# ferdean/lsa-fw

Measured on AMD Instinct MI355X. Metric: converged eigenpairs/sec (k=20, shift-invert), higher is better.
Workload: dtype c128

## Files before the change

### include/lsa_hip.h

```cpp
#ifndef LSA_HIP_H
#define LSA_HIP_H

#include <stdint.h>

#ifdef __cplusplus
extern "C" {
#endif

typedef enum { LSA_F64 = 0, LSA_C128 = 1 } lsa_dtype;

typedef enum {
    LSA_OK = 0,
    LSA_ERR_ARG = -1,
    LSA_ERR_HIP = -2,
    LSA_ERR_ZERO_PIVOT = -3,
    LSA_ERR_DIVERGED = -4,
    LSA_ERR_NONFINITE = -5,
    LSA_ERR_TIMEOUT = -6,
    LSA_ERR_COMM = -7,
    LSA_ERR_OOM = -8
} lsa_status;

typedef struct lsa_ctx lsa_ctx;
typedef struct lsa_mat lsa_mat;
typedef struct lsa_vec lsa_vec;
typedef struct lsa_ilu lsa_ilu;
typedef struct lsa_op lsa_op;
typedef struct lsa_krylov lsa_krylov;

typedef struct {
    int64_t op_applies;
    int64_t gmres_iters;
    int64_t spmv_calls;
    int64_t sptrsv_calls;
    double last_rel_res;
    double max_rel_res;
    double seconds_factor;
    double seconds_solve;
    int32_t stagnated_solves;
    int32_t pc_fallback;
    int32_t backward_accepted;
    int32_t analysis_reused;
    int32_t refined_solves;
    int32_t reserved0;
} lsa_stats;

int lsa_ctx_create(int device, lsa_ctx **out);
void lsa_ctx_destroy(lsa_ctx *ctx);
const char *lsa_last_error(const lsa_ctx *ctx);
int lsa_ctx_synchronize(lsa_ctx *ctx);
const char *lsa_ctx_arch(const lsa_ctx *ctx);

int lsa_vec_create(lsa_ctx *ctx, int64_t n, int dtype, lsa_vec **out);
void lsa_vec_destroy(lsa_vec *v);
int lsa_vec_upload(lsa_ctx *ctx, lsa_vec *v, const void *host);
int lsa_vec_download(lsa_ctx *ctx, const lsa_vec *v, void *host);

int lsa_csr_upload(lsa_ctx *ctx, int32_t n, int64_t nnz, const int32_t *rowptr, const int32_t *col,
                   const void *val, int dtype, lsa_mat **out);
void lsa_mat_destroy(lsa_mat *m);
int lsa_mat_download_values(lsa_ctx *ctx, const lsa_mat *m, void *host_val);
int lsa_csr_axpby(lsa_ctx *ctx, const lsa_mat *A, const lsa_mat *B, const double alpha[2], const double beta[2],
                  int out_dtype, lsa_mat **out);
int lsa_spmv(lsa_ctx *ctx, const lsa_mat *A, const lsa_vec *x, lsa_vec *y);
int lsa_spmv_transpose(lsa_ctx *ctx, const lsa_mat *A, int conj, const lsa_vec *x, lsa_vec *y);
int lsa_spmv_info(lsa_ctx *ctx, const lsa_mat *A, int xdtype, char *kernel, int32_t kernel_len, int64_t *bytes_moved);
int lsa_spmv_time(lsa_ctx *ctx, const lsa_mat *A, const lsa_vec *x, lsa_vec *y, int iters, double *avg_ms);

int lsa_ilu_create(lsa_ctx *ctx, const lsa_mat *C, int levels, double shift_tol, lsa_ilu **out);
void lsa_ilu_destroy(lsa_ilu *pc);
int lsa_ilu_set_algorithm(lsa_ctx *ctx, lsa_ilu *pc, int algo, int32_t block_size);
int lsa_ilu_solve(lsa_ctx *ctx, lsa_ilu *pc, int which, const lsa_vec *b, lsa_vec *x);
int lsa_ilu_solve_time(lsa_ctx *ctx, lsa_ilu *pc, int which, const lsa_vec *b, lsa_vec *x, int iters, double *avg_ms);
int lsa_ilu_info(const lsa_ilu *pc, int64_t *nnz, int32_t *levels_lower, int32_t *levels_upper, int32_t *nshift);
int lsa_ilu_download(lsa_ctx *ctx, const lsa_ilu *pc, int32_t *rowptr, int32_t *col, void *val);

typedef struct lsa_nd_sym lsa_nd_sym;
typedef struct lsa_ndlu lsa_ndlu;
int lsa_nd_analyse(int32_t n, const int32_t *rowptr, const int32_t *col, int32_t leaf_size, const int8_t *constraint, lsa_nd_sym **out);
int lsa_nd_order(int32_t n, const int32_t *rowptr, const int32_t *col, int32_t leaf_size, const int8_t *constraint, lsa_nd_sym **out);
int lsa_nd_analyse_tree(int32_t n, const int32_t *rowptr, const int32_t *col, int32_t ntree, const int32_t *first, const int32_t *size,
                        const int32_t *parent, const int32_t *owner, int32_t rank, int32_t nranks, lsa_nd_sym **out);
const char *lsa_nd_sym_error(const lsa_nd_sym *h);
void lsa_nd_sym_destroy(lsa_nd_sym *h);
int lsa_nd_sym_info(const lsa_nd_sym *h, int32_t *ntree, int32_t *nlevels, int32_t *max_front, int64_t *index_entries,
                    int64_t *factor_entries, int64_t *front_entries, double *flops);
int lsa_nd_sym_memory(const lsa_nd_sym *h, int32_t scalar_bytes, int64_t work_budget_bytes, int64_t *out, int64_t *upd_off, int64_t *work_off,
                      int32_t *chunk_of);
int lsa_nd_sym_export(const lsa_nd_sym *h, int32_t *perm, int32_t *node_start, int32_t *parent, int32_t *level, int32_t *front_size,
                      int32_t *idx);
int lsa_nd_sym_export_tables(const lsa_nd_sym *h, int32_t *cmap, int32_t *gptr, int32_t *gidx, int64_t *asm_dst, int32_t *lvl_ptr,
                             int32_t *lvl_nodes);
int lsa_nd_sym_export_dist(const lsa_nd_sym *h, int32_t *kind, int64_t *front_off, int64_t *u_off, int32_t *asm_src, int32_t *children_ptr,
                           int32_t *children_idx, int64_t *scalars);
int lsa_nd_sym_export_top(const lsa_nd_sym *h, int32_t *owner, int32_t *rows, int64_t *exch, int64_t *totals);
int lsa_ndlu_create(lsa_ctx *ctx, const lsa_mat *C, int32_t leaf_size, lsa_ndlu **out);
int lsa_ndlu_prepare(lsa_ctx *ctx, const lsa_mat *P, int dtype, int32_t leaf_size, const int8_t *constraint);
int lsa_ndlu_prepare_tree(lsa_ctx *ctx, const lsa_mat *P, int dtype, int32_t ntree, const int32_t *first, const int32_t *size,
                          const int32_t *parent);
int lsa_ndlu_create_tree(lsa_ctx *ctx, const lsa_mat *C, int32_t ntree, const int32_t *first, const int32_t *size, const int32_t *parent,
                         const int32_t *owner, lsa_ndlu **out);
int lsa_ndlu_refactor(lsa_ctx *ctx, lsa_ndlu *f, const lsa_mat *C);
void lsa_ndlu_destroy(lsa_ndlu *f);
int lsa_ndlu_solve(lsa_ctx *ctx, lsa_ndlu *f, const lsa_vec *b, lsa_vec *x);
int lsa_ndlu_solve_batch(lsa_ctx *ctx, int32_t J, lsa_ndlu *const *f, const lsa_vec *const *b, lsa_vec *const *x);
int lsa_ndlu_solve_adjoint(lsa_ctx *ctx, lsa_ndlu *f, int conj, const lsa_vec *b, lsa_vec *x);
int lsa_ndlu_solve_time(lsa_ctx *ctx, lsa_ndlu *f, const lsa_vec *b, lsa_vec *x, int iters, double *avg_ms);
int lsa_ndlu_inertia(lsa_ctx *ctx, lsa_ndlu *f, int64_t *negative, int64_t *zero, int64_t *positive);
int lsa_ndlu_info(const lsa_ndlu *f, int32_t *ntree, int32_t *nlevels, int32_t *max_front, int64_t *factor_entries,
                  int64_t *front_entries, int64_t *apply_bytes, int32_t *apply_launches, double *seconds_analyse,
                  double *seconds_numeric);

int lsa_gmres(lsa_ctx *ctx, const lsa_mat *C, lsa_ilu *pc, const lsa_vec *b, lsa_vec *x, int use_x0, double rtol,
              int restart, int maxit, int32_t *iters, double *rel_res);

typedef struct {
    int32_t ilu_levels;
    double ilu_shift;
    double ksp_rtol;
    int32_t ksp_restart;
    int32_t ksp_maxit;
    int32_t pc_type;
    double antishift[2];
} lsa_op_options;

int lsa_op_create(lsa_ctx *ctx, const lsa_mat *A, const lsa_mat *M, const double sigma[2], int mode,
                  const lsa_op_options *opts, lsa_op **out);
void lsa_op_destroy(lsa_op *op);
int lsa_op_apply(lsa_ctx *ctx, lsa_op *op, const lsa_vec *x, lsa_vec *y);
int lsa_op_stats(const lsa_op *op, lsa_stats *out);
int lsa_op_set_adjoint(lsa_ctx *ctx, lsa_op *op, int on);
int lsa_op_set_projection(lsa_ctx *ctx, lsa_op *op, const double *keep);

int lsa_krylov_create(lsa_ctx *ctx, lsa_op *op, int32_t ncv, lsa_krylov **out);
// ... 94 lines not shown
```

### lsa-fw_amd/csrc/core.hip

```cpp
#include "lsa_internal.h"

int lsa_set_error(lsa_ctx* ctx, int code, const char* fmt, ...) {
    char buf[1024];
    va_list ap;
    va_start(ap, fmt);
    vsnprintf(buf, sizeof buf, fmt, ap);
    va_end(ap);
    if (ctx) ctx->err = buf;
    return code;
}

int lsa_ensure_scratch(lsa_ctx* ctx, size_t dbytes, size_t hbytes) {
    if (dbytes > ctx->dscratch_bytes) {
        LSA_HIP_CHECK(ctx, hipStreamSynchronize(ctx->stream));
        if (ctx->dscratch) (void)hipFree(ctx->dscratch);
        ctx->dscratch = nullptr;
        ctx->dscratch_bytes = 0;
        size_t want = dbytes * 2;
        LSA_HIP_CHECK(ctx, hipMalloc(&ctx->dscratch, want));
        ctx->dscratch_bytes = want;
    }
    if (hbytes > ctx->pinned_bytes) {
        LSA_HIP_CHECK(ctx, hipStreamSynchronize(ctx->stream));
        if (ctx->pinned) (void)hipHostFree(ctx->pinned);
        ctx->pinned = nullptr;
        ctx->pinned_bytes = 0;
        size_t want = hbytes * 2;
        LSA_HIP_CHECK(ctx, hipHostMalloc(&ctx->pinned, want, hipHostMallocDefault));
        ctx->pinned_bytes = want;
    }
    return LSA_OK;
}

lsa_mat* mat_row_view(const lsa_mat* full, int32_t r0, int32_t r1) {
    lsa_mat* v = new lsa_mat();
    v->ctx = full->ctx;
    v->n = r1 - r0;
    v->ncols = full->ncols;
    v->row0 = r0;
    v->nnz = (int64_t)full->h_rp[(size_t)r1] - full->h_rp[(size_t)r0];
    v->dtype = full->dtype;
    v->rp = full->rp + r0;
    v->ci = full->ci;
    v->val = full->val;
    v->owns_index = false;
    v->owns_values = false;
    v->ci16_state = -1;
    return v;
}

extern "C" {

int lsa_ctx_create(int device, lsa_ctx** out) {
    if (!out) return LSA_ERR_ARG;
    *out = nullptr;
    int ndev = 0;
    if (hipGetDeviceCount(&ndev) != hipSuccess || ndev <= 0) return LSA_ERR_HIP;
    if (device < 0 || device >= ndev) return LSA_ERR_ARG;
    if (hipSetDevice(device) != hipSuccess) return LSA_ERR_HIP;
    lsa_ctx* ctx = new lsa_ctx();
    ctx->device = device;
    hipDeviceProp_t prop;
    if (hipGetDeviceProperties(&prop, device) != hipSuccess) {
        delete ctx;
        return LSA_ERR_HIP;
    }
    ctx->arch = prop.gcnArchName;
    ctx->num_cu = prop.multiProcessorCount > 0 ? prop.multiProcessorCount : 256;
    if (hipStreamCreateWithFlags(&ctx->stream, hipStreamNonBlocking) != hipSuccess ||
        hipEventCreate(&ctx->ev0) != hipSuccess || hipEventCreate(&ctx->ev1) != hipSuccess) {
        delete ctx;
        return LSA_ERR_HIP;
    }
    if (lsa_ensure_scratch(ctx, 1 << 20, 1 << 16) != LSA_OK) {
        delete ctx;
        return LSA_ERR_HIP;
    }
    *out = ctx;
    return LSA_OK;
}

void lsa_ctx_destroy(lsa_ctx* ctx) {
    if (!ctx) return;
    (void)hipSetDevice(ctx->device);
    if (ctx->stream) (void)hipStreamSynchronize(ctx->stream);
    lsa_ndlu_drop_cache(ctx);
    lsa_krylov_drop_cache(ctx);
    comm_release(ctx);
    if (ctx->dscratch) (void)hipFree(ctx->dscratch);
    if (ctx->pinned) (void)hipHostFree(ctx->pinned);
    if (ctx->ev0) (void)hipEventDestroy(ctx->ev0);
    if (ctx->ev1) (void)hipEventDestroy(ctx->ev1);
    if (ctx->stream) (void)hipStreamDestroy(ctx->stream);
    delete ctx;
}

const char* lsa_last_error(const lsa_ctx* ctx) { return ctx ? ctx->err.c_str() : "null context"; }
const char* lsa_ctx_arch(const lsa_ctx* ctx) { return ctx ? ctx->arch.c_str() : ""; }

int lsa_ctx_synchronize(lsa_ctx* ctx) {
    if (!ctx) return LSA_ERR_ARG;
    LSA_HIP_CHECK(ctx, hipStreamSynchronize(ctx->stream));
    return LSA_OK;
}

static size_t dtype_size(int dtype) { return dtype == LSA_C128 ? 16 : 8; }

int lsa_vec_create(lsa_ctx* ctx, int64_t n, int dtype, lsa_vec** out) {
    if (!ctx || !out || n < 0 || (dtype != LSA_F64 && dtype != LSA_C128))
        return lsa_set_error(ctx, LSA_ERR_ARG, "lsa_vec_create: bad argument");
    lsa_vec* v = new lsa_vec{ctx, n, dtype, nullptr};
    hipError_t e = hipMalloc(&v->d, (size_t)(n > 0 ? n : 1) * dtype_size(dtype));
    if (e != hipSuccess) {
        delete v;
        return lsa_set_error(ctx, LSA_ERR_HIP, "hipMalloc(vector of %lld) failed: %s", (long long)n, hipGetErrorString(e));
    }
    e = hipMemsetAsync(v->d, 0, (size_t)(n > 0 ? n : 1) * dtype_size(dtype), ctx->stream);
    if (e != hipSuccess) {
        (void)hipFree(v->d);
        delete v;
        return lsa_set_error(ctx, LSA_ERR_HIP, "hipMemsetAsync failed: %s", hipGetErrorString(e));
    }
    *out = v;
    return LSA_OK;
}

void lsa_vec_destroy(lsa_vec* v) {
    if (!v) return;
    if (v->ctx && v->ctx->stream) (void)hipStreamSynchronize(v->ctx->stream);
    if (v->d) (void)hipFree(v->d);
    delete v;
}

int lsa_vec_upload(lsa_ctx* ctx, lsa_vec* v, const void* host) {
    if (!ctx || !v || !host) return lsa_set_error(ctx, LSA_ERR_ARG, "lsa_vec_upload: null argument");
    LSA_HIP_CHECK(ctx, hipMemcpyAsync(v->d, host, (size_t)v->n * dtype_size(v->dtype), hipMemcpyHostToDevice, ctx->stream));
    LSA_HIP_CHECK(ctx, hipStreamSynchronize(ctx->stream));
    return LSA_OK;
}

int lsa_vec_download(lsa_ctx* ctx, const lsa_vec* v, void* host) {
    if (!ctx || !v || !host) return lsa_set_error(ctx, LSA_ERR_ARG, "lsa_vec_download: null argument");
    LSA_HIP_CHECK(ctx, hipMemcpyAsync(host, v->d, (size_t)v->n * dtype_size(v->dtype), hipMemcpyDeviceToHost, ctx->stream));
    LSA_HIP_CHECK(ctx, hipStreamSynchronize(ctx->stream));
    return LSA_OK;
}

static int validate_csr(lsa_ctx* ctx, int32_t n, int32_t ncols, int64_t nnz, const int32_t* rp, const int32_t* ci) {
    if (rp[0] != 0 || rp[n] != nnz) return lsa_set_error(ctx, LSA_ERR_ARG, "CSR: rowptr[0] must be 0 and rowptr[n] == nnz");
    for (int32_t i = 0; i < n; ++i) {
        if (rp[i + 1] < rp[i]) return lsa_set_error(ctx, LSA_ERR_ARG, "CSR: rowptr not monotone at row %d", i);
        for (int32_t p = rp[i]; p < rp[i + 1]; ++p) {
            if (ci[p] < 0 || ci[p] >= ncols) return lsa_set_error(ctx, LSA_ERR_ARG, "CSR: column %d out of range in row %d", ci[p], i);
            if (p > rp[i] && ci[p] <= ci[p - 1]) return lsa_set_error(ctx, LSA_ERR_ARG, "CSR: columns of row %d are not strictly increasing", i);
        }
    }
    return LSA_OK;
}

static int csr_upload_impl(lsa_ctx* ctx, int32_t n_local, int32_t ncols, int32_t row0, int64_t nnz, const int32_t* rowptr,
                           const int32_t* col, const void* val, int dtype, lsa_mat** out) {
    if (!ctx || !out || !rowptr || (nnz > 0 && (!col || !val)) || n_local < 0 || nnz < 0 ||
        (dtype != LSA_F64 && dtype != LSA_C128))
        return lsa_set_error(ctx, LSA_ERR_ARG, "lsa_csr_upload: bad argument");
    if (nnz >= (int64_t)INT32_MAX) return lsa_set_error(ctx, LSA_ERR_ARG, "lsa_csr_upload: nnz >= 2^31 needs 64-bit row pointers");
    LSA_CHECK(validate_csr(ctx, n_local, ncols, nnz, rowptr, col));
    lsa_mat* m = new lsa_mat();
    m->ctx = ctx;
    m->n = n_local;
    m->ncols = ncols;
    m->row0 = row0;
    m->nnz = nnz;
    m->dtype = dtype;
// ... 3 lines not shown
    m->val = nullptr;
    m->h_rp.assign(rowptr, rowptr + n_local + 1);
    m->h_ci.assign(col, col + nnz);
    size_t vb = (size_t)(nnz > 0 ? nnz : 1) * dtype_size(dtype);
    hipError_t e1 = hipMalloc(&m->rp, sizeof(int32_t) * (size_t)(n_local + 1));
    hipError_t e2 = hipMalloc(&m->ci, sizeof(int32_t) * (size_t)(nnz > 0 ? nnz : 1));
    hipError_t e3 = hipMalloc(&m->val, vb);
    if (e1 != hipSuccess || e2 != hipSuccess || e3 != hipSuccess) {
        lsa_mat_destroy(m);
        return lsa_set_error(ctx, LSA_ERR_HIP, "hipMalloc(CSR n=%d nnz=%lld) failed", n_local, (long long)nnz);
    }
    hipError_t e = hipMemcpyAsync(m->rp, rowptr, sizeof(int32_t) * (size_t)(n_local + 1), hipMemcpyHostToDevice, ctx->stream);
    if (e == hipSuccess && nnz > 0) e = hipMemcpyAsync(m->ci, col, sizeof(int32_t) * (size_t)nnz, hipMemcpyHostToDevice, ctx->stream);
    if (e == hipSuccess && nnz > 0) e = hipMemcpyAsync(m->val, val, (size_t)nnz * dtype_size(dtype), hipMemcpyHostToDevice, ctx->stream);
    if (e == hipSuccess) e = hipStreamSynchronize(ctx->stream);
    if (e != hipSuccess) {
        lsa_mat_destroy(m);
        return lsa_set_error(ctx, LSA_ERR_HIP, "CSR upload failed: %s", hipGetErrorString(e));
    }
    *out = m;
    return LSA_OK;
}

int lsa_csr_upload(lsa_ctx* ctx, int32_t n, int64_t nnz, const int32_t* rowptr, const int32_t* col, const void* val,
                   int dtype, lsa_mat** out) {
    return csr_upload_impl(ctx, n, n, 0, nnz, rowptr, col, val, dtype, out);
}

int lsa_csr_upload_shard(lsa_ctx* ctx, int32_t n_global, int32_t row0, int32_t row1, int64_t nnz_local,
                         const int32_t* rowptr_local, const int32_t* col, const void* val, int dtype, lsa_mat** out) {
    if (row0 < 0 || row1 < row0 || row1 > n_global) return lsa_set_error(ctx, LSA_ERR_ARG, "lsa_csr_upload_shard: bad row range");
    return csr_upload_impl(ctx, row1 - row0, n_global, row0, nnz_local, rowptr_local, col, val, dtype, out);
}

int64_t lsa_mat_rows(const lsa_mat* m) { return m ? (int64_t)m->n : 0; }

void lsa_mat_destroy(lsa_mat* m) {
    if (!m) return;
    if (m->ctx && m->ctx->stream) (void)hipStreamSynchronize(m->ctx->stream);
    if (m->owns_index) {
        if (m->rp) (void)hipFree(m->rp);
        if (m->ci) (void)hipFree(m->ci);
    }
    if (m->val && m->owns_values) (void)hipFree(m->val);
    if (!m->owns_extras) m->ci16 = nullptr, m->cbase = nullptr, m->grp_start = nullptr;
    if (m->grp_start) (void)hipFree(m->grp_start);
    if (m->ci16) (void)hipFree(m->ci16);
    if (m->cbase) (void)hipFree(m->cbase);
    delete m;
}

int lsa_mat_download_values(lsa_ctx* ctx, const lsa_mat* m, void* host_val) {
    if (!ctx || !m || !host_val) return lsa_set_error(ctx, LSA_ERR_ARG, "lsa_mat_download_values: null argument");
    LSA_HIP_CHECK(ctx, hipMemcpyAsync(host_val, m->val, (size_t)m->nnz * dtype_size(m->dtype), hipMemcpyDeviceToHost, ctx->stream));
    LSA_HIP_CHECK(ctx, hipStreamSynchronize(ctx->stream));
    return LSA_OK;
}

}

template <typename TA, typename TB, typename TC>
__global__ void axpby_kernel(int64_t nnz, const TA* __restrict__ a, const TB* __restrict__ b, cplx alpha, cplx beta,
                             TC* __restrict__ c) {
    int64_t stride = (int64_t)gridDim.x * blockDim.x;
    for (int64_t p = (int64_t)blockIdx.x * blockDim.x + threadIdx.x; p < nnz; p += stride) {
        cplx acc{0.0, 0.0};
        fma_acc(acc, alpha, to_cplx(a[p]));
        fma_acc(acc, beta, to_cplx(b[p]));
        s_from(c[p], acc.re, acc.im);
    }
}

template <typename TA, typename TB, typename TC>
static void launch_axpby(lsa_ctx* ctx, int64_t nnz, const void* a, const void* b, cplx alpha, cplx beta, void* c) {
    int threads = 256;
    int64_t want = (nnz + threads - 1) / threads;
    int blocks = (int)(want < 1 ? 1 : (want > 4096 ? 4096 : want));
    hipLaunchKernelGGL((axpby_kernel<TA, TB, TC>), dim3(blocks), dim3(threads), 0, ctx->stream, nnz, (const TA*)a, (const TB*)b,
                       alpha, beta, (TC*)c);
}

extern "C" int lsa_csr_axpby(lsa_ctx* ctx, const lsa_mat* A, const lsa_mat* B, const double alpha[2], const double beta[2],
                             int out_dtype, lsa_mat** out) {
    if (!ctx || !A || !B || !alpha || !beta || !out) return lsa_set_error(ctx, LSA_ERR_ARG, "lsa_csr_axpby: null argument");
    if (A->n != B->n || A->nnz != B->nnz || A->ncols != B->ncols || A->row0 != B->row0)
        return lsa_set_error(ctx, LSA_ERR_ARG, "lsa_csr_axpby: operands must share one sparsity pattern (n %d vs %d, nnz %lld vs %lld)",
                             A->n, B->n, (long long)A->nnz, (long long)B->nnz);
    if (!A->h_rp.same_object(B->h_rp) || !A->h_ci.same_object(B->h_ci)) {
        if (A->h_rp != B->h_rp || A->h_ci != B->h_ci)
            return lsa_set_error(ctx, LSA_ERR_ARG, "lsa_csr_axpby: operands must share one sparsity pattern (index arrays differ)");
        B->h_rp = A->h_rp;
        B->h_ci = A->h_ci;
        if (!A->h_hash) A->h_hash = B->h_hash ? B->h_hash : std::make_shared<uint64_t>(0);
        B->h_hash = A->h_hash;
        if (!A->h_shared) A->h_shared = B->h_shared ? B->h_shared : std::make_shared<PatternShared>();
        B->h_shared = A->h_shared;
    }
    if (out_dtype == LSA_F64 && (A->dtype != LSA_F64 || B->dtype != LSA_F64 || alpha[1] != 0.0 || beta[1] != 0.0))
        return lsa_set_error(ctx, LSA_ERR_ARG, "lsa_csr_axpby: a real result needs real operands and real coefficients");
    lsa_mat* C = new lsa_mat();
    C->ctx = ctx;
    C->n = A->n;
    C->ncols = A->ncols;
    C->row0 = A->row0;
    C->nnz = A->nnz;
    C->dtype = out_dtype;
    C->rp = A->rp;
    C->ci = A->ci;
    C->owns_index = false;
    C->h_rp = A->h_rp;
    C->h_ci = A->h_ci;
    if (!A->h_hash) A->h_hash = std::make_shared<uint64_t>(0);
    C->h_hash = A->h_hash;
    if (!A->h_shared) A->h_shared = std::make_shared<PatternShared>();
    C->h_shared = A->h_shared;
    C->val = nullptr;
    hipError_t e = hipMalloc(&C->val, (size_t)(C->nnz > 0 ? C->nnz : 1) * dtype_size(out_dtype));
    if (e != hipSuccess) {
        delete C;
        return lsa_set_error(ctx, LSA_ERR_HIP, "hipMalloc(axpby result) failed: %s", hipGetErrorString(e));
    }
    cplx al{alpha[0], alpha[1]}, be{beta[0], beta[1]};
    const bool ca = A->dtype == LSA_C128, cb = B->dtype == LSA_C128;
    if (out_dtype == LSA_F64) launch_axpby<double, double, double>(ctx, C->nnz, A->val, B->val, al, be, C->val);
    else if (!ca && !cb) launch_axpby<double, double, cplx>(ctx, C->nnz, A->val, B->val, al, be, C->val);
    else if (ca && !cb) launch_axpby<cplx, double, cplx>(ctx, C->nnz, A->val, B->val, al, be, C->val);
    else if (!ca && cb) launch_axpby<double, cplx, cplx>(ctx, C->nnz, A->val, B->val, al, be, C->val);
    else launch_axpby<cplx, cplx, cplx>(ctx, C->nnz, A->val, B->val, al, be, C->val);
    hipError_t le = hipGetLastError();
    if (le != hipSuccess) {
        lsa_mat_destroy(C);
        return lsa_set_error(ctx, LSA_ERR_HIP, "axpby launch failed: %s", hipGetErrorString(le));
    }
    *out = C;
    return LSA_OK;
}
```

### lsa-fw_amd/csrc/dense.hip

```cpp
#include <algorithm>
#include <chrono>
#include <cmath>
#include <cstdint>
#include <cstring>
#include <vector>

#include "lsa_internal.h"

namespace {

struct Z {
    double re, im;
};
inline Z operator+(Z a, Z b) { return {a.re + b.re, a.im + b.im}; }
inline Z operator-(Z a, Z b) { return {a.re - b.re, a.im - b.im}; }
inline Z operator-(Z a) { return {-a.re, -a.im}; }
inline Z operator*(Z a, Z b) { return {a.re * b.re - a.im * b.im, a.re * b.im + a.im * b.re}; }
inline Z operator*(double a, Z b) { return {a * b.re, a * b.im}; }
inline Z conj(Z a) { return {a.re, -a.im}; }
inline double abs1(Z a) { return std::fabs(a.re) + std::fabs(a.im); }
inline double abs2(Z a) { return a.re * a.re + a.im * a.im; }
inline double zabs(Z a) { return std::hypot(a.re, a.im); }
inline Z zdiv(Z a, Z b) {
    if (std::fabs(b.re) >= std::fabs(b.im)) {
// ... 667 lines not shown
        }
    auto W = [&](int i, int j) -> double& { return w[(size_t)j * n + i]; };
    auto swap_sym = [&](int p, int q) {
        if (p == q) return;
        for (int j = 0; j < n; ++j) std::swap(W(p, j), W(q, j));
        for (int i = 0; i < n; ++i) std::swap(W(i, p), W(i, q));
    };
    const double alpha = (1.0 + std::sqrt(17.0)) / 8.0, tiny = std::max(tol_rel, 0.0) * amax;
    int k = 0;
    while (k < n) {
        const double absakk = std::fabs(W(k, k));
        int imax = k;
        double colmax = 0.0;
        for (int i = k + 1; i < n; ++i)
            if (std::fabs(W(i, k)) > colmax) colmax = std::fabs(W(i, k)), imax = i;
        int step = 1;
        if (std::max(absakk, colmax) <= tiny) {
            ++*zero;
            ++k;
            continue;
        }
        if (absakk < alpha * colmax) {
            double rowmax = 0.0;
            for (int j = k; j < n; ++j)
                if (j != imax) rowmax = std::max(rowmax, std::fabs(W(imax, j)));
            if (absakk >= alpha * colmax * (colmax / rowmax)) {
            } else if (std::fabs(W(imax, imax)) >= alpha * rowmax) {
                swap_sym(k, imax);
            } else {
                swap_sym(k + 1, imax);
                step = 2;
            }
        }
        if (step == 1) {
            const double d = W(k, k);
            if (std::fabs(d) <= tiny) ++*zero;
            else if (d < 0.0) ++*negative;
            else ++*positive;
            if (std::fabs(d) > tiny) {
                const double dinv = 1.0 / d;
                for (int j = k + 1; j < n; ++j) {
                    const double f = W(k, j) * dinv;
                    if (f == 0.0) continue;
                    for (int i = k + 1; i < n; ++i) W(i, j) -= W(i, k) * f;
                }
            }
        } else {
            const double a = W(k, k), b = W(k + 1, k), c = W(k + 1, k + 1), det = a * c - b * b;
            if (std::fabs(det) <= tiny * tiny) {
                *zero += 2;
            } else {
                if (det < 0.0) {
                    ++*negative;
                    ++*positive;
                } else if (a + c < 0.0) *negative += 2;
                else *positive += 2;
                for (int j = k + 2; j < n; ++j) {
                    const double u = W(k, j), v = W(k + 1, j);
                    const double f0 = (c * u - b * v) / det, f1 = (a * v - b * u) / det;
                    if (f0 == 0.0 && f1 == 0.0) continue;
                    for (int i = k + 2; i < n; ++i) W(i, j) -= W(i, k) * f0 + W(i, k + 1) * f1;
                }
            }
        }
        k += step;
    }
    return LSA_OK;
}

static_assert(sizeof(lsa_ks_result) == 56 && sizeof(lsa_ks_options) == 88, "lsa_ks_options layout is part of the C-ABI (tests/test_abi.py)");

int lsa_krylov_solve(lsa_ctx* ctx, lsa_krylov* k, const lsa_ks_options* o, const void* v0, const double* mask, int32_t max_out, void* theta_out,
                     void* lambda_out, void* X_out, double* est_out, lsa_ks_result* result) {
    if (!ctx || !k || !o || !result) return lsa_set_error(ctx, LSA_ERR_ARG, "lsa_krylov_solve: null argument");
    int32_t m = 0;
    int64_t n = 0;
    LSA_CHECK(lsa_krylov_shape(k, &n, &m));
    if (m > n) return lsa_set_error(ctx, LSA_ERR_ARG, "ncv = %d exceeds the problem size %lld", m, (long long)n);
    LSA_CHECK(ks_check_options(ctx, "lsa_krylov_solve", o, max_out, theta_out, lambda_out));
    const int nev = std::min<int>(o->nev, m);
    const double keep_fraction = ks_keep_fraction(o);
    const Selector sel{o->which, o->transform, {o->sigma[0], o->sigma[1]}, {o->antishift[0], o->antishift[1]}, {o->target[0], o->target[1]}};
    Rng rng = ks_rng(o);
    std::vector<Z> vec((size_t)n);
    auto random_vector = [&]() {
        for (int64_t i = 0; i < n; ++i) {
            rng.normal_pair(vec[(size_t)i].re, vec[(size_t)i].im);
            if (mask && mask[i] == 0.0) vec[(size_t)i] = {0.0, 0.0};
        }
    };
    if (v0) {
        memcpy(vec.data(), v0, (size_t)n * sizeof(Z));
        if (mask)
            for (int64_t i = 0; i < n; ++i)
                if (mask[i] == 0.0) vec[(size_t)i] = {0.0, 0.0};
    } else {
        random_vector();
    }
    LSA_CHECK(lsa_krylov_inject(ctx, k, 0, vec.data()));
    const int ldh = m + 1;
    std::vector<Z> H((size_t)ldh * m, Z{0.0, 0.0}), T((size_t)m * m), Q((size_t)m * m), S((size_t)m * m), b((size_t)m), bq((size_t)m), w((size_t)m);
    std::vector<double> est((size_t)m), rel((size_t)m), keys((size_t)m);
    std::vector<int> rank((size_t)m);
    std::vector<char> select((size_t)m);
    const Mat Hm{H.data(), ldh}, Tm{T.data(), m}, Qm{Q.data(), m}, Sm{S.data(), m};
    int kept = 0, restarts = 0;
    int64_t applies = 0;
    memset(result, 0, sizeof *result);
    KsClock clk;
    auto extend = [&](int j, int32_t* bd) {
        LSA_CHECK(lsa_krylov_extend(ctx, k, j, m, H.data(), ldh, bd));
        if (*bd >= 0) Hm(*bd + 1, *bd) = {0.0, 0.0};
        return (int)LSA_OK;
    };
    auto inject_random = [&](int j) {
        random_vector();
        return lsa_krylov_inject(ctx, k, j, vec.data());
    };
    while (true) {
        clk.start();
        LSA_CHECK(ks_expand(kept, m, &applies, extend, inject_random));
        clk.lap(clk.expand);
        for (int c = 0; c < m; ++c) {
            b[(size_t)c] = Hm(m, c);
            for (int r = 0; r < m; ++r) Tm(r, c) = Hm(r, c);
        }
        if (!schur(m, Tm, Qm)) return lsa_set_error(ctx, LSA_ERR_DIVERGED, "Krylov-Schur: the QR algorithm on the projected matrix did not converge");
        tri_eigenvectors(m, Tm, Sm);
        for (int c = 0; c < m; ++c) {
            Z acc = {0.0, 0.0};
            for (int r = 0; r < m; ++r) acc = acc + b[(size_t)r] * Qm(r, c);
            bq[(size_t)c] = acc;
        }
        for (int c = 0; c < m; ++c) {
            Z acc = {0.0, 0.0};
            for (int r = 0; r <= c; ++r) acc = acc + bq[(size_t)r] * Sm(r, c);
            est[(size_t)c] = zabs(acc);
            w[(size_t)c] = Tm(c, c);
            keys[(size_t)c] = sel.key(w[(size_t)c]);
            rel[(size_t)c] = est[(size_t)c] / std::max(zabs(w[(size_t)c]), 2.2250738585072014e-308);
        }
        const int nconv = ks_rank_converged(m, keys, rel, o->tol, rank);
        if (nconv >= nev || nconv >= m || restarts >= o->max_restarts) {
            const int nout = std::min<int>(nconv, max_out);
            if (nout > 0) {
                std::vector<Z> Y((size_t)m * nout);
                for (int c = 0; c < nout; ++c) {
                    const int src = rank[(size_t)c];
                    for (int r = 0; r < m; ++r) {
                        Z acc = {0.0, 0.0};
                        for (int q = 0; q <= src; ++q) acc = acc + Qm(r, q) * Sm(q, src);
                        Y[(size_t)c * m + r] = acc;
                    }
                    ((Z*)theta_out)[c] = w[(size_t)src];
                    ((Z*)lambda_out)[c] = sel.back(w[(size_t)src]);
                    if (est_out) est_out[c] = rel[(size_t)src];
                }
                clk.lap(clk.dense);
                if (X_out) LSA_CHECK(lsa_krylov_ritz_vectors(ctx, k, m, nout, Y.data(), m, 3, X_out));
                clk.lap(clk.restart);
            }
            clk.lap(clk.dense);
            ks_fill_result(result, clk, nconv, nout, restarts, applies, nconv < m ? rel[(size_t)rank[(size_t)nconv]] : 0.0);
            return k_agree_in_step(ctx, "lsa_krylov_solve");
        }
        int knew = ks_keep_count(m, nconv, keep_fraction);
        {
            std::vector<double> sorted(keys);
            std::sort(sorted.begin(), sorted.end());
            const double thr = sorted[(size_t)knew] > sorted[(size_t)knew - 1] ? 0.5 * (sorted[(size_t)knew - 1] + sorted[(size_t)knew]) : sorted[(size_t)knew - 1];
            for (int c = 0; c < m; ++c) select[(size_t)c] = keys[(size_t)c] <= thr;
            const int sdim = schur_reorder(m, Tm, Qm, select);
            knew = std::max(std::min(sdim, m - 1), 1);
        }
        clk.lap(clk.dense);
        LSA_CHECK(lsa_krylov_restart(ctx, k, m, knew, Q.data(), m));
        clk.lap(clk.restart);
        std::fill(H.begin(), H.end(), Z{0.0, 0.0});
        for (int c = 0; c < knew; ++c) {
            for (int r = 0; r <= c; ++r) Hm(r, c) = Tm(r, c);
            Z acc = {0.0, 0.0};
            for (int r = 0; r < m; ++r) acc = acc + b[(size_t)r] * Qm(r, c);
            Hm(knew, c) = acc;
        }
        kept = knew;
        ++restarts;
    }
}

int lsa_eigs_sinvert(lsa_ctx* ctx, const lsa_mat* A, const lsa_mat* M, const double sigma[2], int32_t nev, int32_t ncv, double tol, int32_t max_restarts,
                     const lsa_op_options* opts, const void* v0, const int32_t* row_perm, int32_t max_out, void* lambda_out, void* X_out, double* est_out,
                     lsa_ks_result* result, lsa_stats* stats) {
    if (!ctx || !A || !sigma || !opts || !result) return lsa_set_error(ctx, LSA_ERR_ARG, "lsa_eigs_sinvert: null argument");
    if (ncv <= 0) ncv = std::max(2 * nev, nev + 15);
    ncv = (int32_t)std::min<int64_t>(ncv, lsa_mat_rows(A));
    lsa_op* op = nullptr;
    lsa_krylov* kr = nullptr;
    int rc = lsa_op_create(ctx, A, M, sigma, 0, opts, &op);
    if (rc == LSA_OK) rc = lsa_krylov_create(ctx, op, ncv, &kr);
    if (rc == LSA_OK && row_perm) rc = lsa_krylov_set_row_permutation(ctx, kr, row_perm);
    if (rc == LSA_OK) {
        lsa_ks_options o;
        memset(&o, 0, sizeof o);
        o.nev = nev;
        o.max_restarts = max_restarts;
        o.tol = tol;
        o.which = LSA_WHICH_TARGET_MAGNITUDE;
        o.transform = 0;
        o.sigma[0] = o.target[0] = sigma[0];
// ... 114 lines not shown
```

### lsa-fw_amd/csrc/lsa_internal.h

```cpp
#pragma once

#include <hip/hip_runtime.h>

#include <cstdarg>
#include <cstdint>
#include <cstdio>
#include <cstdlib>
#include <cstring>
#include <memory>
#include <string>
#include <vector>

#include "../../include/lsa_hip.h"

struct cplx {
    double re, im;
};
static_assert(sizeof(cplx) == 16, "complex128 layout");

__host__ __device__ inline cplx make_cplx(double r, double i) { return cplx{r, i}; }

template <typename T>
struct scalar_traits;
template <>
struct scalar_traits<double> {
    static constexpr int dtype = LSA_F64;
    __host__ __device__ static double zero() { return 0.0; }
};
template <>
struct scalar_traits<cplx> {
    static constexpr int dtype = LSA_C128;
    __host__ __device__ static cplx zero() { return cplx{0.0, 0.0}; }
};

__host__ __device__ inline void fma_acc(double& acc, double a, double b) { acc = fma(a, b, acc); }
__host__ __device__ inline void fma_acc(cplx& acc, double a, cplx b) {
    acc.re = fma(a, b.re, acc.re);
    acc.im = fma(a, b.im, acc.im);
}
__host__ __device__ inline void fma_acc(cplx& acc, cplx a, cplx b) {
    acc.re = fma(a.re, b.re, acc.re);
    acc.re = fma(-a.im, b.im, acc.re);
    acc.im = fma(a.re, b.im, acc.im);
    acc.im = fma(a.im, b.re, acc.im);
}
__host__ __device__ inline void fma_conj_acc(double& acc, double a, double b) { acc = fma(a, b, acc); }
__host__ __device__ inline void fma_conj_acc(cplx& acc, cplx a, cplx b) {
    acc.re = fma(a.re, b.re, acc.re);
    acc.re = fma(a.im, b.im, acc.re);
    acc.im = fma(a.re, b.im, acc.im);
    acc.im = fma(-a.im, b.re, acc.im);
}
__host__ __device__ inline double s_mul(double a, double b) { return a * b; }
__host__ __device__ inline cplx s_mul(double a, cplx b) { return cplx{a * b.re, a * b.im}; }
__host__ __device__ inline cplx s_mul(cplx a, cplx b) { return cplx{a.re * b.re - a.im * b.im, a.re * b.im + a.im * b.re}; }
__host__ __device__ inline double s_add(double a, double b) { return a + b; }
__host__ __device__ inline cplx s_add(cplx a, cplx b) { return cplx{a.re + b.re, a.im + b.im}; }
__host__ __device__ inline double s_sub(double a, double b) { return a - b; }
__host__ __device__ inline cplx s_sub(cplx a, cplx b) { return cplx{a.re - b.re, a.im - b.im}; }
__host__ __device__ inline double s_conj(double a) { return a; }
__host__ __device__ inline cplx s_conj(cplx a) { return cplx{a.re, -a.im}; }
__host__ __device__ inline double s_abs2(double a) { return a * a; }
__host__ __device__ inline double s_abs2(cplx a) { return a.re * a.re + a.im * a.im; }
__host__ __device__ inline double s_inv(double a) { return 1.0 / a; }
__host__ __device__ inline cplx s_inv(cplx a) {
    if (fabs(a.re) >= fabs(a.im)) {
        double r = a.im / a.re, d = a.re + a.im * r;
        return cplx{1.0 / d, -r / d};
    }
    double r = a.re / a.im, d = a.re * r + a.im;
    return cplx{r / d, -1.0 / d};
}
__host__ __device__ inline cplx to_cplx(double a) { return cplx{a, 0.0}; }
__host__ __device__ inline cplx to_cplx(cplx a) { return a; }
__host__ __device__ inline void s_from(double& out, double re, double) { out = re; }
__host__ __device__ inline void s_from(cplx& out, double re, double im) { out = cplx{re, im}; }

struct lsa_ctx {
    int device = 0;
    hipStream_t stream = nullptr;
    hipEvent_t ev0 = nullptr, ev1 = nullptr;
    std::string err;
    std::string arch;
    int num_cu = 256;
    void* pinned = nullptr;
    size_t pinned_bytes = 0;
    void* dscratch = nullptr;
    size_t dscratch_bytes = 0;
    void* comm = nullptr;
    int nranks = 1, rank = 0;
    lsa_host_allgather_fn host_gather = nullptr;
    void* host_gather_user = nullptr;
    void* comm_stage = nullptr;
    size_t comm_stage_bytes = 0;
    int64_t comm_calls = 0, comm_bytes = 0;
    struct lsa_ndlu* nd_cache = nullptr;
    struct lsa_krylov* krylov_cache = nullptr;
};
extern "C" void lsa_ndlu_drop_cache(lsa_ctx* ctx);
extern "C" void lsa_krylov_drop_cache(lsa_ctx* ctx);

struct lsa_vec {
    lsa_ctx* ctx;
    int64_t n;
    int dtype;
    void* d;
};

struct SharedInts {
    std::shared_ptr<const std::vector<int32_t>> p;
    const int32_t* data() const { return p ? p->data() : nullptr; }
    size_t size() const { return p ? p->size() : 0; }
    const int32_t& operator[](size_t i) const { return (*p)[i]; }
    const std::vector<int32_t>& vec() const {
        static const std::vector<int32_t> none;
        return p ? *p : none;
    }
    void assign(const int32_t* b, const int32_t* e) { p = std::make_shared<const std::vector<int32_t>>(b, e); }
    bool same_object(const SharedInts& o) const { return p == o.p; }
    bool operator==(const SharedInts& o) const { return p == o.p || vec() == o.vec(); }
    bool operator!=(const SharedInts& o) const { return !(*this == o); }
};

struct TransposeIndex {
    int32_t *rp = nullptr, *ci = nullptr, *src = nullptr;
    int32_t ncols = 0;
    int64_t nnz = 0;
    ~TransposeIndex() {
        for (void* p : {(void*)rp, (void*)ci, (void*)src})
            if (p) (void)hipFree(p);
    }
};

struct PatternShared {
    std::shared_ptr<TransposeIndex> tr;
};

struct lsa_mat {
    lsa_ctx* ctx;
    int32_t n;
    int32_t ncols;
    int32_t row0;
    int64_t nnz;
    int dtype;
    int32_t* rp;
    int32_t* ci;
    void* val;
    bool owns_index;
    bool owns_values = true;
    mutable SharedInts h_rp, h_ci;
    mutable std::shared_ptr<uint64_t> h_hash;
    mutable std::shared_ptr<PatternShared> h_shared;
    mutable uint16_t* ci16 = nullptr;
    mutable int32_t* cbase = nullptr;
    mutable int ci16_state = 0;
    mutable int32_t* grp_start = nullptr;
    mutable int32_t ngroups = 0;
    mutable int grp_state = 0;
    bool owns_extras = true;
};

int lsa_set_error(lsa_ctx* ctx, int code, const char* fmt, ...);
lsa_mat* mat_row_view(const lsa_mat* full, int32_t r0, int32_t r1);
void comm_release(lsa_ctx* ctx);
int k_agree_status(lsa_ctx* ctx, int rc);
int k_agree_min_i64(lsa_ctx* ctx, int64_t* value);
int k_agree_in_step(lsa_ctx* ctx, const char* where);
int lsa_ensure_scratch(lsa_ctx* ctx, size_t dbytes, size_t hbytes);
inline bool env_flag(const char* name, bool dflt) {
    const char* e = getenv(name);
    return e ? atoi(e) != 0 : dflt;
}

#define LSA_HIP_CHECK(ctx, expr)                                                                         \
    do {                                                                                                 \
        hipError_t _e = (expr);                                                                          \
        if (_e != hipSuccess)                                                                            \
            return lsa_set_error((ctx), LSA_ERR_HIP, "%s failed: %s (%s:%d)", #expr, hipGetErrorString(_e), \
                                 __FILE__, __LINE__);                                                    \
    } while (0)

#define LSA_HIP_ALLOC(ctx, expr)                                                                                    \
    do {                                                                                                            \
        hipError_t _e = (expr);                                                                                     \
        if (_e != hipSuccess) {                                                                                     \
            (void)hipGetLastError();                                                                                \
            return lsa_set_error((ctx), _e == hipErrorOutOfMemory ? LSA_ERR_OOM : LSA_ERR_HIP, "%s failed: %s (%s:%d)", #expr, \
                                 hipGetErrorString(_e), __FILE__, __LINE__);                                        \
        }                                                                                                           \
    } while (0)

#define LSA_CHECK(expr)            \
    do {                           \
        int _rc = (expr);          \
        if (_rc != LSA_OK) return _rc; \
    } while (0)


int k_spmv(lsa_ctx* ctx, const lsa_mat* A, int xdtype, const void* x, void* y);
int k_spmv_transpose(lsa_ctx* ctx, const lsa_mat* A, int conj, int xdtype, const void* x, void* y);

int k_copy(lsa_ctx* ctx, int dtype, int64_t n, const void* x, void* y);
int k_set_zero(lsa_ctx* ctx, int dtype, int64_t n, void* x);
int k_axpy(lsa_ctx* ctx, int dtype, int64_t n, const double alpha[2], const void* x, void* y);
int k_multi_dot(lsa_ctx* ctx, int dtype, int64_t n, int j, const void* V, int64_t ldv, const void* w, void* h_dev);
int k_multi_axpy_dot(lsa_ctx* ctx, int dtype, int64_t n, int j, const void* V, int64_t ldv, const void* h1_dev, void* w, void* h2_dev);
int k_multi_axpy(lsa_ctx* ctx, int dtype, int64_t n, int j, const void* V, int64_t ldv, const void* h_dev, void* w,
                 double* nrm2_dev);
int k_columns_canonical(lsa_ctx* ctx, int64_t n, int ncols, void* X, int64_t ldx, int unit, double* imag2_dev);
int k_nrm2(lsa_ctx* ctx, int dtype, int64_t n, const void* x, double* nrm2_dev);
int k_mask(lsa_ctx* ctx, int dtype, int64_t n, const double* keep_dev, void* y);
int k_residual_norms(lsa_ctx* ctx, int dtype, int64_t n, const void* b, const void* z, void* w, double* nrm2_dev);
int k_scale_by_inv_norm(lsa_ctx* ctx, int dtype, int64_t n, const void* x, const double* nrm2_dev, void* y);
int k_hess_column(lsa_ctx* ctx, int dtype, int j, const void* h1, const void* h2, const double* nrm2_dev, void* hout);
size_t k_cgs2_fused_work_bytes(lsa_ctx* ctx, int64_t n, int jmax);
int k_cgs2_fused(lsa_ctx* ctx, int dtype, int64_t n, int j, const void* V, int64_t ldv, void* w, void* vnext, void* hcol_dev, void* work,
                 const void* chk_b, const void* chk_z, double* chk_out);
bool k_cgs2_tail_fits(lsa_ctx* ctx, int64_t n, int jmax, const lsa_mat* M, const lsa_mat* C);
int k_cgs2_tail_parts(int64_t n);
int k_cgs2_fused_tail(lsa_ctx* ctx, int64_t n, int j, const void* V, int64_t ldv, const void* y, void* w, void* vnext, void* hcol_dev, void* work,
                      const lsa_mat* M, const lsa_mat* C, void* t, double* tail_part);
int k_cgs2_tail_checks(lsa_ctx* ctx, int nslots, int nparts, const double* tail_parts, double* checks);
bool k_dcgs2_fits(int64_t n, int ncv);
int k_dcgs2_step(lsa_ctx* ctx, int64_t n, int j, void* V, int64_t ldv, const void* y, int first, void* slot, int lds, void* work,
                 const void* chk_b, const void* chk_z, double* chk_out);
int k_dcgs2_norm(lsa_ctx* ctx, int64_t n, void* work, void* slot, int lds);
int k_dcgs2_tail(lsa_ctx* ctx, int64_t n, int j, const void* V, int64_t ldv, const void* y, void* work, const lsa_mat* M, const lsa_mat* C, void* t,
                 double* tail_part, void* slot, int lds);
int k_spmv_plain_subwave_lanes(const lsa_mat* A);
int k_basis_gemm(lsa_ctx* ctx, int dtype, int64_t n, int m, int k, const void* V, int64_t ldv, const void* Q, int ldq,
                 void* Out, int64_t ldo);
int k_scatter_rows(lsa_ctx* ctx, int dtype, int64_t n, int ncols, const int32_t* perm, const void* In, void* Out);

int basis_upload_row_permutation(lsa_ctx* ctx, const char* who, int64_t n, const int32_t* perm, int32_t** row_perm);
int basis_times_host_matrix(lsa_ctx* ctx, int dtype, int64_t n, int m, int k, const void* V, const void* Q, int ldq, void* qdev, void* Out,
                            size_t pinned_extra);
int direct_solve_enqueue(lsa_ctx* ctx, lsa_op* op, int dtype, const void* rhs, void* y, void* z, void* r, bool refine, double* norms);
void stats_book_direct_solve(lsa_stats* st, int products, bool refine, double res, double bnorm);

struct lsa_ndlu;
struct lsa_op_parts {
    int64_t n;
    const lsa_mat *Kmul, *Kfac;
    lsa_ndlu* nd;
    bool plain;
    double ksp_rtol;
    double normF;
    bool* refine;
    lsa_stats* st;
};
int lsa_op_get_parts(lsa_op* op, lsa_op_parts* out);
int lanczos_shape(const lsa_lanczos* l, int64_t* n, int32_t* ncv);
int lanczos_inject(lsa_ctx* ctx, lsa_lanczos* l, int32_t j, const double* host_v);
int lanczos_restart(lsa_ctx* ctx, lsa_lanczos* l, int32_t m, int32_t knew, const double* Y, int32_t ldy);
int lanczos_ritz_vectors(lsa_ctx* ctx, lsa_lanczos* l, int32_t m, int32_t nvec, const double* Y, int32_t ldy, double* X);

struct lsa_ilu {
    lsa_ctx* ctx;
    int32_t n;
    int64_t nnz;
    int dtype;
    int32_t *rp, *ci, *diag;
    void* val;
    void* dinv;
    int32_t *order_l, *order_u;
    std::vector<int32_t> lvl_ptr_l, lvl_ptr_u;
    std::vector<int32_t> h_rp, h_ci, h_diag;
    int32_t nshift;
    int32_t* flag;
    int sptrsv_blocks_l, sptrsv_blocks_u;
    int algo;
    void* tmp;
    int tmp_dtype;
    int32_t blk_B = 0, blk_nb = 0;
    int32_t *lsplit = nullptr, *usplit = nullptr;
    void *linv = nullptr, *uinv = nullptr;
    void *blk_t[2] = {nullptr, nullptr}, *blk_y[2] = {nullptr, nullptr};
    void *blk_in[2] = {nullptr, nullptr}, *blk_out[2] = {nullptr, nullptr};
    void* blk_graph[2] = {nullptr, nullptr};
};

int ilu_solve_dev(lsa_ctx* ctx, lsa_ilu* pc, int which, int vdtype, const void* b, void* x);
int blk_setup(lsa_ctx* ctx, lsa_ilu* pc, int32_t B);
int blk_solve(lsa_ctx* ctx, lsa_ilu* pc, int which, int vdtype, const void* b, void* x);
void blk_release(lsa_ilu* pc);

struct lsa_ndlu;
int ndlu_solve_dev(lsa_ctx* ctx, lsa_ndlu* f, int vdtype, const void* b, void* x);
int ndlu_solve_adjoint_dev(lsa_ctx* ctx, lsa_ndlu* f, int conj, int vdtype, const void* b, void* x);
```

### lsa-fw_amd/csrc/ndlu.hip

```cpp
#include <algorithm>
#include <chrono>
#include <cmath>
#include <cstdlib>
#include <functional>
#include <new>
#include <string>

#include "lsa_internal.h"
#include "nd_internal.h"

int k_allgather_inplace(lsa_ctx* ctx, void* vec, size_t bytes_per_rank);

namespace {

constexpr int kRT = 32;
constexpr int kCH = 1024;
constexpr int kGT = 64;

inline double now_s() { return std::chrono::duration<double>(std::chrono::steady_clock::now().time_since_epoch()).count(); }
inline size_t esize(int dtype) { return dtype == LSA_C128 ? 16 : 8; }

struct NdNodeDev {
    int64_t front_off;
    int64_t lfac_off;
// ... 2067 lines not shown
        if (L.exchange_before && f->xupd_slot > 0) {
            LSA_CHECK(k_allgather_inplace(ctx, f->d_upd, (size_t)f->xupd_slot * sizeof(T)));
            exchanged = true;
        }
        LSA_HIP_CHECK(ctx, hipMemsetAsync(f->d_work, 0, (size_t)L.work_entries * sizeof(T), st));
        if (L.asm_count > 0) {
            const int blocks = (int)std::min<int64_t>((L.asm_count + 255) / 256, (int64_t)ctx->num_cu * 16);
            hipLaunchKernelGGL((nd_assemble_kernel<T>), dim3(blocks), dim3(256), 0, st, L.asm_count, (const T*)C->val, f->d_asm_src + L.asm_begin,
                               f->d_asm_dst + L.asm_begin, front);
        }
        for (const TileList& e : L.ext)
            if (e.count > 0)
                hipLaunchKernelGGL((nd_extend_add_kernel<T>), dim3(e.count), dim3(256), 0, st, tl + 2 * e.off, f->d_nodes, f->d_cmap, front, (const T*)upd);
        for (const auto& step : L.xsteps) {
            T* stage = (T*)f->d_xstage;
            int64_t stride = 0;
            for (int r = 0; r < S.nranks; ++r) {
                const NdChunk::XPiece& pc = step[(size_t)r];
                if (pc.nrows > 0) stride = std::max(stride, (int64_t)pc.nrows * (S.f[(size_t)pc.child] - S.m[(size_t)pc.child]));
            }
            if (stride == 0) continue;
            const NdChunk::XPiece& mine = step[(size_t)S.rank];
            if (mine.nrows > 0) {
                const int32_t bc = S.f[(size_t)mine.child] - S.m[(size_t)mine.child];
                const int64_t src_off = f->chunk_node_upd_off(mine.child) + (int64_t)(mine.row0 - S.brow0[(size_t)mine.child]) * bc;
                LSA_HIP_CHECK(ctx, hipMemcpyAsync(stage + (size_t)S.rank * (size_t)stride, upd + src_off, (size_t)mine.nrows * (size_t)bc * sizeof(T),
                                                  hipMemcpyDeviceToDevice, st));
            }
            LSA_CHECK(k_allgather_inplace(ctx, stage, (size_t)stride * sizeof(T)));
            for (int r = 0; r < S.nranks; ++r) {
                const NdChunk::XPiece& pc = step[(size_t)r];
                if (pc.nrows <= 0) continue;
                hipLaunchKernelGGL((nd_extend_add_staged_kernel<T>), dim3((pc.nrows + 15) / 16), dim3(256), 0, st, f->d_nodes, f->d_cmap, front,
                                   (const T*)(stage + (size_t)r * (size_t)stride), pc.child, pc.row0, pc.nrows);
            }
        }
        if (L.max_m >= f->tp_min) LSA_CHECK(launch_level_tp<T>(ctx, f, L, tiny2));
        for (int32_t kb = 0; kb < L.max_m && L.max_m < f->tp_min; kb += kNB) {
            if (L.max_m <= 64) launch_block<T, 64, 1, 8>(ctx, f, L, kb, tiny2);
            else if (L.max_m <= 128) launch_block<T, 128, 1, 8>(ctx, f, L, kb, tiny2);
            else if (L.max_m <= 256) launch_block<T, 256, 1, 8>(ctx, f, L, kb, tiny2);
            else if (L.max_m <= 512) launch_block<T, 512, 1, 8>(ctx, f, L, kb, tiny2);
            else if (L.max_m <= 1024) launch_block<T, 1024, 1, 8>(ctx, f, L, kb, tiny2);
            else if (L.max_m <= 2048) launch_block<T, 1024, 2, 8>(ctx, f, L, kb, tiny2);
            else if (L.max_m <= 4096) launch_block<T, 1024, 4, 4>(ctx, f, L, kb, tiny2);
            else if (L.max_m <= 8192) launch_block<T, 1024, 8, 2>(ctx, f, L, kb, tiny2);
            else launch_block<T, 1024, 16, 1>(ctx, f, L, kb, tiny2);
        }
        if (L.unperm.count > 0)
            hipLaunchKernelGGL((nd_unperm_kernel<T>), dim3(L.unperm.count), dim3(256), 0, st, tl + 2 * L.unperm.off, f->d_nodes, front, f->d_ipiv,
                               f->d_rowq, lfac);
        auto product = [&](auto kind) {
            constexpr int KIND = decltype(kind)::value;
            if (L.gemm[KIND].count == 0) return;
            hipLaunchKernelGGL((nd_gemm_mfma_kernel<T, KIND>), dim3(L.gemm[KIND].count), dim3(256), 0, st, tl + 2 * L.gemm[KIND].off, f->d_nodes, front, lfac, ufac);
        };
        product(std::integral_constant<int, 0>{});
        product(std::integral_constant<int, 1>{});
        product(std::integral_constant<int, 2>{});
        if (L.save.count > 0)
            hipLaunchKernelGGL((nd_save_update_kernel<T>), dim3(L.save.count), dim3(256), 0, st, tl + 2 * L.save.off, f->d_nodes, (const T*)front, upd);
    }
    if (f->top.s > 0)
        for (int q = 0, t0 = 0; q < 2; t0 += f->top_tiles[q++])
            if (f->top_tiles[q] > 0)
                hipLaunchKernelGGL((nd_top_gemm_kernel<T>), dim3(f->top_tiles[q]), dim3(256), 0, st, f->d_top_tiles + 2 * t0, f->d_top_jobs, f->d_cmap,
                                   (const T*)lfac, (const T*)ufac, (T*)f->d_top, f->top.s);
    if (!exchanged && S.nranks > 1 && f->xupd_slot > 0)
        LSA_CHECK(k_allgather_inplace(ctx, f->d_upd, (size_t)f->xupd_slot * sizeof(T)));
    int32_t hflag[4] = {0, 0, 0, 0};
    if (S.nranks > 1) {
        LSA_HIP_CHECK(ctx, hipMemcpyAsync(f->d_xflag + 4 * S.rank, f->d_flag, 4 * sizeof(int32_t), hipMemcpyDeviceToDevice, st));
        LSA_CHECK(k_allgather_inplace(ctx, f->d_xflag, 4 * sizeof(int32_t)));
        std::vector<int32_t> all((size_t)4 * S.nranks, 0);
        LSA_HIP_CHECK(ctx, hipMemcpyAsync(all.data(), f->d_xflag, all.size() * sizeof(int32_t), hipMemcpyDeviceToHost, st));
        LSA_HIP_CHECK(ctx, hipStreamSynchronize(st));
        for (int r = 0; r < S.nranks; ++r)
            if (all[(size_t)4 * r + 1] != 0) {
                memcpy(hflag, &all[(size_t)4 * r], sizeof hflag);
                if (r != S.rank) hflag[1] = -(r + 1);
                break;
            }
    } else {
        LSA_HIP_CHECK(ctx, hipMemcpyAsync(hflag, f->d_flag, sizeof hflag, hipMemcpyDeviceToHost, st));
        LSA_HIP_CHECK(ctx, hipStreamSynchronize(st));
    }
    LSA_HIP_CHECK(ctx, hipGetLastError());
    if (hflag[1] < 0)
        return lsa_set_error(ctx, LSA_ERR_ZERO_PIVOT, "lsa_ndlu: a pivot block on rank %d is singular to 1e-15 * max|C| (column %d of its node)", -hflag[1] - 1,
                             hflag[2]);
    if (hflag[1] != 0) {
        const int32_t t = hflag[1] - 1;
        const unsigned long long hi = (unsigned long long)(uint32_t)hflag[3] << 32;
        double mag2;
        memcpy(&mag2, &hi, sizeof mag2);
        return lsa_set_error(ctx, LSA_ERR_ZERO_PIVOT,
                             "lsa_ndlu: the pivot block of tree node %d (%d unknowns, front %d, level %d) is singular at its column %d: largest "
                             "candidate pivot %.3e against max|C| = %.3e (threshold 1e-15 max|C|); the matrix is singular, or needs pivoting "
                             "across fronts",
                             t, S.m[(size_t)t], S.f[(size_t)t], S.level[(size_t)t], hflag[2], std::sqrt(mag2), std::sqrt(max2));
    }
    if (const char* pe = getenv("LSA_ND_TEST_PERTURB")) {
        const double eps = atof(pe);
        if (eps != 0.0 && f->ufac_entries > 0) {
            const int blocks = (int)std::min<int64_t>((f->ufac_entries + 255) / 256, (int64_t)ctx->num_cu * 16);
            hipLaunchKernelGGL((nd_scale_kernel<T>), dim3(blocks), dim3(256), 0, st, f->ufac_entries, ufac, 1.0 + eps);
            LSA_HIP_CHECK(ctx, hipStreamSynchronize(st));
        }
    }
    return LSA_OK;
}

template <typename MT, typename VT, bool ORDERED>
int nd_apply_ordered(lsa_ctx* ctx, lsa_ndlu* f, const VT* b, VT* x) {
    hipStream_t st = ctx->stream;
    const MT* lfac = (const MT*)f->d_lfac;
    const MT* ufac = (const MT*)f->d_ufac;
    const NdSymbolic& S = f->S;
    VT *ubuf = (VT*)f->d_ubuf, *acc = (VT*)f->d_acc, *xb = (VT*)f->d_xb;
    const bool top = f->top.s > 0;
    if (f->acc_vbytes != (int)sizeof(VT)) {
        LSA_HIP_CHECK(ctx, hipMemsetAsync(f->d_acc, 0, (size_t)std::max<int64_t>(f->acc_entries, 1) * 16, st));
        f->acc_vbytes = (int)sizeof(VT);
    }
    for (size_t li = 0; li <= f->levels.size(); ++li) {
        if ((int32_t)li == S.phase_b_level && S.nranks > 1 && S.xu_slot > 0) LSA_CHECK(k_allgather_inplace(ctx, f->d_ubuf, (size_t)S.xu_slot * sizeof(VT)));
        if (li == f->levels.size()) break;
        const NdLevel& L = f->levels[li];
        if (ORDERED && top && (int32_t)li + 1 == f->top_level) continue;
        if (ORDERED && top && (int32_t)li == f->top_level) {
            hipLaunchKernelGGL((nd_top_kernel<MT, VT>), dim3((f->top.s + 7) / 8), dim3(256), 0, st, f->top, (const MT*)f->d_top, f->d_top_icmap, f->d_gell, b, x,
                               (const VT*)acc, xb);
        } else if (L.fwd_tiles > 0) {
            const dim3 grid(L.node_count, L.fwd_tiles);
            const NdSweepNode* ln = f->d_lnodes + L.node_begin;
            if (L.sweep_rows == 8)
                hipLaunchKernelGGL((nd_fwd_kernel<MT, VT, 64, ORDERED>), grid, dim3(256), 0, st, ln, lfac, f->d_idx, f->d_gell, f->d_cmap, b, x, ubuf, acc, xb);
            else if (L.sweep_rows == 128)
                hipLaunchKernelGGL((nd_fwd_kernel<MT, VT, 4, ORDERED>), grid, dim3(256), 0, st, ln, lfac, f->d_idx, f->d_gell, f->d_cmap, b, x, ubuf, acc, xb);
            else
                hipLaunchKernelGGL((nd_fwd_kernel<MT, VT, 16, ORDERED>), grid, dim3(256), 0, st, ln, lfac, f->d_idx, f->d_gell, f->d_cmap, b, x, ubuf, acc, xb);
        }
        if (L.dist_count > 0 && L.ux_slot > 0) LSA_CHECK(k_allgather_inplace(ctx, ubuf + L.ux_base, (size_t)L.ux_slot * sizeof(VT)));
    }
    for (size_t l = f->levels.size(); l-- > 0;) {
        const NdLevel& L = f->levels[l];
        if (L.bwd_tiles > 0 && !(ORDERED && top && (int32_t)l + 1 == f->top_level)) {
            const dim3 grid(L.node_count, L.bwd_tiles);
            const NdSweepNode* ln = f->d_lnodes_bwd + L.node_begin;
            if (L.sweep_rows == 8) hipLaunchKernelGGL((nd_bwd_kernel<MT, VT, 64, ORDERED>), grid, dim3(256), 0, st, ln, ufac, f->d_idx, f->d_gell, x, xb);
            else hipLaunchKernelGGL((nd_bwd_kernel<MT, VT, 16, ORDERED>), grid, dim3(256), 0, st, ln, ufac, f->d_idx, f->d_gell, x, xb);
        }
        if (L.dist_count > 0) {
            const int32_t* dn = f->d_dist_nodes + L.dist_begin;
            VT* xg = (VT*)f->d_xg;
            if (L.xg_slot > 0) {
                hipLaunchKernelGGL((nd_dist_pack_kernel<VT, ORDERED>), dim3(L.dist_count, (L.dist_rows + 255) / 256), dim3(256), 0, st, dn, f->d_nodes, f->d_idx, S.rank,
                                   (const VT*)x, xg);
                LSA_CHECK(k_allgather_inplace(ctx, xg + L.xg_base, (size_t)L.xg_slot * sizeof(VT)));
            }
            hipLaunchKernelGGL((nd_dist_unpack_kernel<VT, ORDERED>), dim3(L.dist_count, 1 + L.dist_children, (L.dist_rows + 255) / 256), dim3(256), 0, st, dn, f->d_nodes,
                               f->d_child_ptr, f->d_child_idx, f->d_cmap, f->d_idx, S.nranks, x, (const VT*)xg, xb);
        }
    }
    LSA_HIP_CHECK(ctx, hipGetLastError());
    return LSA_OK;
// ... 544 lines not shown
```

### lsa-fw_amd/csrc/solver.hip

```cpp
#include <algorithm>
#include <chrono>
#include <cmath>
#include <complex>

#include "lsa_internal.h"

int ilu_check_abort(lsa_ctx* ctx, lsa_ilu* pc);
int k_allgather_inplace(lsa_ctx* ctx, void* vec, size_t bytes_per_rank);

namespace {

using zc = std::complex<double>;
inline size_t esize(int dtype) { return dtype == LSA_C128 ? 16 : 8; }
inline double now_s() {
    return std::chrono::duration<double>(std::chrono::steady_clock::now().time_since_epoch()).count();
}

struct KrylovSwitches {
    bool fused;
    bool four_passes;
    bool tail;
    bool delayed;
    bool timing;
};
const KrylovSwitches& krylov_switches() {
    static const KrylovSwitches sw = [] {
        const char* passes = getenv("LSA_KRYLOV_PASSES");
        return KrylovSwitches{env_flag("LSA_KRYLOV_FUSED", true), passes && atoi(passes) == 4, env_flag("LSA_KRYLOV_TAIL", true),
                              env_flag("LSA_KRYLOV_DELAYED", true), getenv("LSA_KRYLOV_TIMING") != nullptr};
    }();
    return sw;
}

struct OrthWork {
    void *h1 = nullptr, *h2 = nullptr, *hcol = nullptr;
    double* nrm2 = nullptr;
    void* fused = nullptr;
    int cap = 0;
    int ensure_fused(lsa_ctx* ctx, int64_t n) {
        if (fused) return LSA_OK;
        LSA_HIP_ALLOC(ctx, hipMalloc(&fused, k_cgs2_fused_work_bytes(ctx, n, cap)));
        return LSA_OK;
    }
    int alloc(lsa_ctx* ctx, int cap_, int dtype) {
        cap = cap_;
        const size_t b = (size_t)(cap + 2) * esize(dtype);
        LSA_HIP_CHECK(ctx, hipMalloc(&h1, b));
        LSA_HIP_CHECK(ctx, hipMalloc(&h2, b));
        LSA_HIP_CHECK(ctx, hipMalloc(&hcol, b));
        LSA_HIP_CHECK(ctx, hipMalloc((void**)&nrm2, 4 * sizeof(double)));
        return LSA_OK;
    }
    void release() {
        for (void* p : {h1, h2, hcol, (void*)nrm2, fused})
            if (p) (void)hipFree(p);
        h1 = h2 = hcol = fused = nullptr;
        nrm2 = nullptr;
    }
};

struct SolveCheck {
    const void *b, *z;
    void* r;
    double* out;
};

int orthonormalize_enqueue(lsa_ctx* ctx, int dtype, int64_t n, const void* V, int64_t ldv, int j, void* w, void* vnext, OrthWork& ow,
                           void* hcol_dev, const SolveCheck* chk = nullptr) {
    const KrylovSwitches& sw = krylov_switches();
    if (sw.fused) {
        LSA_CHECK(ow.ensure_fused(ctx, n));
        const int frc = k_cgs2_fused(ctx, dtype, n, j, V, ldv, w, vnext, hcol_dev, ow.fused, chk ? chk->b : nullptr, chk ? chk->z : nullptr,
                                     chk ? chk->out : nullptr);
        if (frc <= 0) return frc;
    }
    if (chk) LSA_CHECK(k_residual_norms(ctx, dtype, n, chk->b, chk->z, chk->r, chk->out));
    LSA_CHECK(k_multi_dot(ctx, dtype, n, j, V, ldv, w, ow.h1));
    const int arc = sw.four_passes ? 1 : k_multi_axpy_dot(ctx, dtype, n, j, V, ldv, ow.h1, w, ow.h2);
    if (arc < 0) return arc;
    if (arc > 0) {
        LSA_CHECK(k_multi_axpy(ctx, dtype, n, j, V, ldv, ow.h1, w, nullptr));
        LSA_CHECK(k_multi_dot(ctx, dtype, n, j, V, ldv, w, ow.h2));
    }
    LSA_CHECK(k_multi_axpy(ctx, dtype, n, j, V, ldv, ow.h2, w, ow.nrm2));
    LSA_CHECK(k_hess_column(ctx, dtype, j, ow.h1, ow.h2, ow.nrm2, hcol_dev));
    LSA_CHECK(k_scale_by_inv_norm(ctx, dtype, n, w, ow.nrm2, vnext));
    return LSA_OK;
}

int orthonormalize(lsa_ctx* ctx, int dtype, int64_t n, const void* V, int64_t ldv, int j, void* w, void* vnext,
                   OrthWork& ow, zc* h_host) {
    LSA_CHECK(orthonormalize_enqueue(ctx, dtype, n, V, ldv, j, w, vnext, ow, ow.hcol));
    const size_t bytes = (size_t)(j + 1) * esize(dtype);
    LSA_CHECK(lsa_ensure_scratch(ctx, 0, bytes));
    LSA_HIP_CHECK(ctx, hipMemcpyAsync(ctx->pinned, ow.hcol, bytes, hipMemcpyDeviceToHost, ctx->stream));
    LSA_HIP_CHECK(ctx, hipStreamSynchronize(ctx->stream));
    if (dtype == LSA_C128) {
        const cplx* p = (const cplx*)ctx->pinned;
        for (int c = 0; c <= j; ++c) h_host[c] = zc(p[c].re, p[c].im);
    } else {
        const double* p = (const double*)ctx->pinned;
        for (int c = 0; c <= j; ++c) h_host[c] = zc(p[c], 0.0);
    }
    return LSA_OK;
}

int device_norm(lsa_ctx* ctx, int dtype, int64_t n, const void* x, double* nrm2_dev, double* out) {
    LSA_CHECK(k_nrm2(ctx, dtype, n, x, nrm2_dev));
    LSA_CHECK(lsa_ensure_scratch(ctx, 0, sizeof(double)));
    LSA_HIP_CHECK(ctx, hipMemcpyAsync(ctx->pinned, nrm2_dev, sizeof(double), hipMemcpyDeviceToHost, ctx->stream));
    LSA_HIP_CHECK(ctx, hipStreamSynchronize(ctx->stream));
    *out = std::sqrt(*(const double*)ctx->pinned);
    return LSA_OK;
}

int upload_small(lsa_ctx* ctx, int dtype, const zc* src, size_t count, void* dst) {
    LSA_CHECK(lsa_ensure_scratch(ctx, 0, count * 16));
    if (dtype == LSA_C128) {
        cplx* p = (cplx*)ctx->pinned;
        for (size_t i = 0; i < count; ++i) p[i] = cplx{src[i].real(), src[i].imag()};
    } else {
        double* p = (double*)ctx->pinned;
        for (size_t i = 0; i < count; ++i) p[i] = src[i].real();
    }
    LSA_HIP_CHECK(ctx, hipMemcpyAsync(dst, ctx->pinned, count * esize(dtype), hipMemcpyHostToDevice, ctx->stream));
    LSA_HIP_CHECK(ctx, hipStreamSynchronize(ctx->stream));
    return LSA_OK;
}

int spmv_global(lsa_ctx* ctx, const lsa_mat* A, int dtype, const void* x, void* y, bool adjoint = false) {
    if (adjoint) return k_spmv_transpose(ctx, A, 1, dtype, x, y);
    const size_t es = esize(dtype);
    LSA_CHECK(k_spmv(ctx, A, dtype, x, (char*)y + (size_t)A->row0 * es));
    if (ctx->nranks > 1 && A->n != A->ncols) LSA_CHECK(k_allgather_inplace(ctx, y, (size_t)(A->ncols / ctx->nranks) * es));
    return LSA_OK;
}

struct PcRef {
    lsa_ilu* ilu = nullptr;
    lsa_ndlu* nd = nullptr;
    bool nd_dist = false;
    bool adjoint = false;
    double normF = 0.0;
    explicit operator bool() const { return ilu || nd; }
    bool exact() const { return nd != nullptr; }
};

int pc_global(lsa_ctx* ctx, PcRef pc, int32_t row0, int64_t nglobal, int dtype, const void* b, void* x) {
    const size_t es = esize(dtype);
    const char* bl = (const char*)b + (size_t)row0 * es;
    char* xl = (char*)x + (size_t)row0 * es;
    if (pc.nd && pc.adjoint) LSA_CHECK(ndlu_solve_adjoint_dev(ctx, pc.nd, 1, dtype, pc.nd_dist ? b : bl, pc.nd_dist ? x : xl));
    else if (pc.nd && pc.nd_dist) LSA_CHECK(ndlu_solve_dev(ctx, pc.nd, dtype, b, x));
    else if (pc.nd) LSA_CHECK(ndlu_solve_dev(ctx, pc.nd, dtype, bl, xl));
    else LSA_CHECK(ilu_solve_dev(ctx, pc.ilu, 2, dtype, bl, xl));
    if (ctx->nranks > 1) LSA_CHECK(k_allgather_inplace(ctx, x, (size_t)(nglobal / ctx->nranks) * es));
    return LSA_OK;
}

struct GmresWork {
    int dtype = LSA_C128;
    int64_t n = 0;
    int restart = 0;
    void *V = nullptr, *w = nullptr, *z = nullptr, *ydev = nullptr;
    OrthWork ow;
    std::vector<zc> H, cs, sn, g, y, hcol;
    int alloc(lsa_ctx* ctx, int64_t n_, int restart_, int dtype_) {
        n = n_;
        restart = restart_;
        dtype = dtype_;
        const size_t vb = (size_t)std::max<int64_t>(n, 1) * esize(dtype);
        LSA_HIP_CHECK(ctx, hipMalloc(&w, vb));
        LSA_HIP_CHECK(ctx, hipMalloc(&z, vb));
        LSA_HIP_CHECK(ctx, hipMemsetAsync(w, 0, vb, ctx->stream));
        LSA_HIP_CHECK(ctx, hipMemsetAsync(z, 0, vb, ctx->stream));
        LSA_HIP_CHECK(ctx, hipMalloc(&ydev, (size_t)(restart + 2) * esize(dtype)));
        LSA_CHECK(ow.alloc(ctx, restart + 1, dtype));
        H.assign((size_t)(restart + 1) * restart, zc(0));
        cs.assign(restart + 1, zc(0));
        sn.assign(restart + 1, zc(0));
        g.assign(restart + 2, zc(0));
        y.assign(restart + 1, zc(0));
        hcol.assign(restart + 2, zc(0));
        return LSA_OK;
    }
    int ensure_basis(lsa_ctx* ctx) {
        if (V) return LSA_OK;
        const size_t vb = (size_t)std::max<int64_t>(n, 1) * esize(dtype);
        LSA_HIP_ALLOC(ctx, hipMalloc(&V, vb * (size_t)(restart + 1)));
        return LSA_OK;
    }
    void release() {
        for (void* p : {V, w, z, ydev})
            if (p) (void)hipFree(p);
        V = w = z = ydev = nullptr;
        ow.release();
    }
};

int gmres_run(lsa_ctx* ctx, const lsa_mat* C, PcRef pc, int dtype, const void* b, void* x, bool use_x0, double rtol,
              int maxit, GmresWork& W, int32_t* iters_out, double* relres_out, lsa_stats* st) {
    const int64_t n = W.n;
    const int m = W.restart;
    const size_t vb = (size_t)n * esize(dtype);
    auto col = [&](int j) { return (void*)((char*)W.V + (size_t)j * vb); };
    double bnorm = 0.0;
    double beta0 = -1.0;
    int total = 0;
    double relres = 0.0;
    if (pc.exact() && !use_x0) {
        LSA_CHECK(pc_global(ctx, pc, C->row0, n, dtype, b, x));
        if (st) st->sptrsv_calls += 2;
        LSA_CHECK(spmv_global(ctx, C, dtype, x, W.z, pc.adjoint));
        if (st) ++st->spmv_calls;
        LSA_CHECK(k_residual_norms(ctx, dtype, n, b, W.z, W.w, W.ow.nrm2));
        LSA_CHECK(lsa_ensure_scratch(ctx, 0, 2 * sizeof(double)));
        LSA_HIP_CHECK(ctx, hipMemcpyAsync(ctx->pinned, W.ow.nrm2, 2 * sizeof(double), hipMemcpyDeviceToHost, ctx->stream));
        LSA_HIP_CHECK(ctx, hipStreamSynchronize(ctx->stream));
        beta0 = std::sqrt(((const double*)ctx->pinned)[0]);
        bnorm = std::sqrt(((const double*)ctx->pinned)[1]);
        use_x0 = true;
        for (int pass = 0; pass < 2 && beta0 > rtol * bnorm && std::isfinite(beta0) && bnorm > 0.0; ++pass) {
            LSA_CHECK(pc_global(ctx, pc, C->row0, n, dtype, W.w, W.z));
            const double one[2] = {1.0, 0.0};
            LSA_CHECK(k_axpy(ctx, dtype, n, one, W.z, x));
            LSA_CHECK(spmv_global(ctx, C, dtype, x, W.z, pc.adjoint));
            LSA_CHECK(k_residual_norms(ctx, dtype, n, b, W.z, W.w, W.ow.nrm2));
            LSA_HIP_CHECK(ctx, hipMemcpyAsync(ctx->pinned, W.ow.nrm2, 2 * sizeof(double), hipMemcpyDeviceToHost, ctx->stream));
            LSA_HIP_CHECK(ctx, hipStreamSynchronize(ctx->stream));
            const double before = beta0;
            beta0 = std::sqrt(((const double*)ctx->pinned)[0]);
            if (st) {
                st->sptrsv_calls += 2;
                ++st->spmv_calls;
                if (pass == 0) ++st->refined_solves;
            }
            if (!(beta0 < 0.5 * before)) break;
        }
        if (beta0 > rtol * bnorm && pc.normF > 0.0 && std::isfinite(beta0)) {
            double xnorm = 0.0;
            LSA_CHECK(device_norm(ctx, dtype, n, x, W.ow.nrm2, &xnorm));
            if (beta0 <= 1e-12 * pc.normF * xnorm) {
                if (st) {
                    ++st->backward_accepted;
                    st->last_rel_res = beta0 / bnorm;
                    st->max_rel_res = std::max(st->max_rel_res, beta0 / bnorm);
                }
                if (iters_out) *iters_out = 0;
                if (relres_out) *relres_out = beta0 / bnorm;
                return LSA_OK;
            }
        }
    } else {
        LSA_CHECK(device_norm(ctx, dtype, n, b, W.ow.nrm2, &bnorm));
    }
    if (!std::isfinite(bnorm)) return lsa_set_error(ctx, LSA_ERR_NONFINITE, "GMRES: right-hand side is not finite");
    if (!use_x0) LSA_CHECK(k_set_zero(ctx, dtype, n, x));
    if (bnorm == 0.0) {
        LSA_CHECK(k_set_zero(ctx, dtype, n, x));
        if (iters_out) *iters_out = 0;
        if (relres_out) *relres_out = 0.0;
        return LSA_OK;
    }
    bool converged = false;
    bool first_cycle = true;
    int verified_cycles = 0;
    bool pending = false;
    double last_verified = 1e300;
    while (!converged && (total < maxit || pending)) {
        if (beta0 >= 0.0) {
        } else if (first_cycle && !use_x0) {
            LSA_CHECK(k_copy(ctx, dtype, n, b, W.w));
        } else {
            LSA_CHECK(spmv_global(ctx, C, dtype, x, W.z, pc.adjoint));
            if (st) ++st->spmv_calls;
            LSA_CHECK(k_copy(ctx, dtype, n, b, W.w));
            const double minus1[2] = {-1.0, 0.0};
            LSA_CHECK(k_axpy(ctx, dtype, n, minus1, W.z, W.w));
        }
        first_cycle = false;
        double beta = beta0;
// ... 84 lines not shown
    if (relres_out) *relres_out = relres;
    if (st) {
        st->gmres_iters += total;
        st->last_rel_res = relres;
        st->max_rel_res = std::max(st->max_rel_res, relres);
    }
    if (!converged)
        return lsa_set_error(ctx, LSA_ERR_DIVERGED, "GMRES did not reach rtol %.1e in %d iterations (relative residual %.3e)", rtol,
                             total, relres);
    return LSA_OK;
}

template <typename T>
__global__ void shift_diag_kernel(int32_t n, int32_t row0, const int32_t* __restrict__ rp, const int32_t* __restrict__ ci,
                                  T* __restrict__ val, cplx shift, int32_t* __restrict__ missing) {
    const int64_t stride = (int64_t)gridDim.x * blockDim.x;
    for (int64_t i = (int64_t)blockIdx.x * blockDim.x + threadIdx.x; i < n; i += stride) {
        const int32_t target = (int32_t)i + row0;
        int32_t lo = rp[i], hi = rp[i + 1];
        while (lo < hi) {
            const int32_t mid = (lo + hi) >> 1;
            if (ci[mid] < target) lo = mid + 1;
            else hi = mid;
        }
        if (lo < rp[i + 1] && ci[lo] == target) {
            cplx v = to_cplx(val[lo]);
            s_from(val[lo], v.re - shift.re, v.im - shift.im);
        } else {
            atomicAdd(missing, 1);
        }
    }
}

}

static_assert(sizeof(lsa_op_options) == 56, "lsa_op_options layout is part of the C-ABI (tests/test_abi.py)");

struct TreeArg {
    int32_t nt;
    const int32_t *first, *size, *parent, *owner;
    int32_t row0, row1;
};

struct lsa_op {
    lsa_ctx* ctx;
    int64_t n;
    const lsa_mat* Kmul;
    const lsa_mat* Kfac;
    lsa_mat* owned;
    lsa_mat* owned_mul = nullptr;
    lsa_mat* owned_diag;
    lsa_ilu* pc;
    lsa_ndlu* nd = nullptr;
    bool nd_dist = false;
    bool adjoint = false;
    double normF = 0.0;
    lsa_mat *view_fac = nullptr, *view_mul = nullptr;
    const lsa_mat* M_whole = nullptr;
    lsa_op_options opts;
    GmresWork gw;
    bool gw_ready;
    void* t;
    double* keep = nullptr;
    bool refine = false;
    lsa_stats st;
};

static PcRef pc_of(const lsa_op* op) {
    PcRef pc;
    pc.ilu = op->pc;
    pc.nd = op->nd;
    pc.nd_dist = op->nd_dist;
    pc.adjoint = op->adjoint;
    pc.normF = op->normF;
    return pc;
}

struct lsa_krylov {
    lsa_ctx* ctx;
    lsa_op* op;
    int64_t n;
    int32_t ncv;
    int32_t* row_perm = nullptr;
    void *V, *V2, *w, *qdev;
    OrthWork ow;
    std::vector<zc> hcol;
    double* imag2 = nullptr;
    void* xtmp = nullptr;
    std::vector<double> imag_norms;
    void* Hdev = nullptr;
    double* checks = nullptr;
    int32_t batch = 0;
    bool pipeline = false;
    void* w2 = nullptr;
    double* tail_parts = nullptr;
    int32_t tail_nparts = 0;
    int32_t t_for = -1;
};

static size_t krylov_slot_bytes(int32_t ncv) { return (size_t)(2 * ncv + 4) * 16; }

static void krylov_free(lsa_krylov* k) {
    for (void* p : {k->V, k->V2, k->w, k->qdev, k->Hdev, (void*)k->checks, (void*)k->imag2, k->xtmp, (void*)k->row_perm, k->w2, (void*)k->tail_parts})
        if (p) (void)hipFree(p);
    k->ow.release();
    delete k;
}

extern "C" {

int lsa_gmres(lsa_ctx* ctx, const lsa_mat* C, lsa_ilu* pc, const lsa_vec* b, lsa_vec* x, int use_x0, double rtol, int restart,
              int maxit, int32_t* iters, double* rel_res) {
    if (!ctx || !C || !b || !x) return lsa_set_error(ctx, LSA_ERR_ARG, "lsa_gmres: null argument");
    if (C->n != C->ncols || b->n != C->n || x->n != C->n || b->dtype != x->dtype)
        return lsa_set_error(ctx, LSA_ERR_ARG, "lsa_gmres: shape/dtype mismatch");
    if (C->dtype == LSA_C128 && b->dtype != LSA_C128) return lsa_set_error(ctx, LSA_ERR_ARG, "lsa_gmres: complex matrix needs complex vectors");
    if (restart < 1 || maxit < 1 || !(rtol > 0.0)) return lsa_set_error(ctx, LSA_ERR_ARG, "lsa_gmres: restart, maxit, rtol must be positive");
    restart = std::min(restart, maxit);
    GmresWork W;
    int rc = W.alloc(ctx, C->n, restart, b->dtype);
    PcRef pcr;
    pcr.ilu = pc;
    if (rc == LSA_OK) rc = gmres_run(ctx, C, pcr, b->dtype, b->d, x->d, use_x0 != 0, rtol, maxit, W, iters, rel_res, nullptr);
    (void)hipStreamSynchronize(ctx->stream);
    W.release();
    return rc;
}

static int build_shifted(lsa_ctx* ctx, const lsa_mat* A, const lsa_mat* M, const double sigma[2], bool cdt, lsa_mat** out) {
    const bool zshift = sigma[0] == 0.0 && sigma[1] == 0.0;
    const double one[2] = {1.0, 0.0}, ms[2] = {-sigma[0], -sigma[1]}, zero[2] = {0.0, 0.0};
    lsa_mat* C = nullptr;
    int rc;
    if (M) rc = lsa_csr_axpby(ctx, A, M, one, ms, cdt ? LSA_C128 : LSA_F64, &C);
    else {
        rc = lsa_csr_axpby(ctx, A, A, one, zero, cdt ? LSA_C128 : LSA_F64, &C);
        if (rc == LSA_OK && !zshift) {
            int32_t* miss = (int32_t*)ctx->dscratch;
            (void)hipMemsetAsync(miss, 0, sizeof(int32_t), ctx->stream);
            const int blocks = std::max(1, std::min((int)((C->n + 255) / 256), ctx->num_cu * 8));
            if (cdt) hipLaunchKernelGGL((shift_diag_kernel<cplx>), dim3(blocks), dim3(256), 0, ctx->stream, C->n, C->row0, C->rp, C->ci, (cplx*)C->val, cplx{sigma[0], sigma[1]}, miss);
            else hipLaunchKernelGGL((shift_diag_kernel<double>), dim3(blocks), dim3(256), 0, ctx->stream, C->n, C->row0, C->rp, C->ci, (double*)C->val, cplx{sigma[0], sigma[1]}, miss);
            int32_t hm = 0;
            (void)hipMemcpyAsync(&hm, miss, sizeof hm, hipMemcpyDeviceToHost, ctx->stream);
            if (hipStreamSynchronize(ctx->stream) != hipSuccess) rc = lsa_set_error(ctx, LSA_ERR_HIP, "diagonal shift failed");
            else if (hm != 0) rc = lsa_set_error(ctx, LSA_ERR_ARG, "A - sigma*I needs a structurally present diagonal (%d rows have none)", hm);
        }
    }
    if (rc != LSA_OK) {
        if (C) lsa_mat_destroy(C);
        return rc;
    }
    *out = C;
    return LSA_OK;
}

static int op_build(lsa_ctx* ctx, const lsa_mat* A, const lsa_mat* M, const lsa_mat* Ad, const lsa_mat* Md, const double sigma[2],
                    int mode, const lsa_op_options* opts, lsa_op** out, const TreeArg* tree = nullptr) {
    if (!ctx || !A || !sigma || !opts || !out) return lsa_set_error(ctx, LSA_ERR_ARG, "lsa_op_create: null argument");
    const bool sharded = Ad != nullptr;
    if (tree) {
        const int nr = std::max(1, ctx->nranks);
        if (sharded || A->n != A->ncols || A->row0 != 0 || (mode != 0 && mode != 2) || opts->pc_type != 2)
            return lsa_set_error(ctx, LSA_ERR_ARG, "lsa_op_create_dist: needs the whole square matrices, a factorising mode (0 or 2) and pc_type 2");
        if (A->ncols % nr != 0 || tree->row0 != (int64_t)ctx->rank * (A->ncols / nr) || tree->row1 < tree->row0 || tree->row1 > tree->row0 + A->ncols / nr)
            return lsa_set_error(ctx, LSA_ERR_ARG, "lsa_op_create_dist: this rank's rows do not sit on its block of the padded layout");
    }
    if (!sharded && A->n != A->ncols) return lsa_set_error(ctx, LSA_ERR_ARG, "lsa_op_create: A must be square (got %d x %d)", A->n, A->ncols);
    if (M && (M->n != A->n || M->ncols != A->ncols || M->row0 != A->row0)) return lsa_set_error(ctx, LSA_ERR_ARG, "lsa_op_create: M does not match A's shape");
    if (mode < 0 || mode > 2) return lsa_set_error(ctx, LSA_ERR_ARG, "lsa_op_create: mode must be 0 (sinvert), 1 (shift) or 2 (Cayley)");
    if (sharded) {
        if (Ad->n != Ad->ncols || Ad->n != A->n || (Md && (Md->n != Ad->n || Md->ncols != Ad->ncols)) || (M != nullptr) != (Md != nullptr))
            return lsa_set_error(ctx, LSA_ERR_ARG, "lsa_op_create_sharded: diagonal blocks must be square with the shard's row count");
        if (A->ncols % std::max(1, ctx->nranks) != 0 || A->row0 != (int64_t)ctx->rank * (A->ncols / std::max(1, ctx->nranks)))
            return lsa_set_error(ctx, LSA_ERR_ARG, "lsa_op_create_sharded: shard does not sit on this rank's block of the padded layout");
        if (A->n > A->ncols / std::max(1, ctx->nranks)) return lsa_set_error(ctx, LSA_ERR_ARG, "lsa_op_create_sharded: shard larger than its padded block");
    }
    const double t0 = now_s();
    lsa_op* op = new lsa_op();
    op->ctx = ctx;
    op->n = A->ncols;
    op->Kmul = op->Kfac = nullptr;
    op->owned = op->owned_diag = nullptr;
    op->pc = nullptr;
    op->opts = *opts;
    op->gw_ready = false;
    op->t = nullptr;
    memset(&op->st, 0, sizeof op->st);
    const bool zshift = sigma[0] == 0.0 && sigma[1] == 0.0;
    const bool cdt = sigma[1] != 0.0 || A->dtype == LSA_C128 || (M && M->dtype == LSA_C128);
    int rc = LSA_OK;
    lsa_mat* C = nullptr;
    if (!(mode == 1 && zshift)) {
        rc = build_shifted(ctx, A, M, sigma, cdt, &C);
        if (rc != LSA_OK) {
            delete op;
            return rc;
        }
        op->owned = C;
    }
    const lsa_mat* fac_src = nullptr;
    if (mode == 0 || mode == 2) {
        op->Kfac = C;
        op->Kmul = M;
        op->M_whole = M;
        bool shard_rows = false;
        if (tree) {
            const char* e = getenv("LSA_DIST_SPMV");
            shard_rows = (e && *e) ? (e[0] == 's') : (C->nnz > 60 * (int64_t)C->n);
        }
        if (tree && shard_rows) {
            op->view_fac = mat_row_view(C, tree->row0, tree->row1);
            op->Kfac = op->view_fac;
            if (M) {
                op->view_mul = mat_row_view(M, tree->row0, tree->row1);
                op->Kmul = op->view_mul;
            }
        }
        if (mode == 2) {
            const double mnu[2] = {-opts->antishift[0], -opts->antishift[1]};
            const bool cmul = cdt || opts->antishift[1] != 0.0;
            rc = build_shifted(ctx, A, M, mnu, cmul, &op->owned_mul);
            if (rc != LSA_OK) {
                lsa_op_destroy(op);
                return rc;
            }
            if (tree && shard_rows) {
                if (op->view_mul) lsa_mat_destroy(op->view_mul);
                op->view_mul = mat_row_view(op->owned_mul, tree->row0, tree->row1);
                op->Kmul = op->view_mul;
            } else op->Kmul = op->owned_mul;
        }
        if (sharded) {
            rc = build_shifted(ctx, Ad, Md, sigma, cdt, &op->owned_diag);
            if (rc != LSA_OK) {
                lsa_op_destroy(op);
                return rc;
            }
            fac_src = op->owned_diag;
        } else fac_src = C;
    } else {
        op->Kmul = C ? C : A;
        op->Kfac = M;
        fac_src = sharded ? Md : M;
    }
    bool lu_fell_back = false;
    if (opts->pc_type == 3) {
        lsa_op_destroy(op);
        return lsa_set_error(ctx, LSA_ERR_ARG, "lsa_op_create: pc_type 3 (the banded block LU of round 1) left the product library; it lives on as a "
                                               "cross-check library for the tests (tests/xcheck).  Use pc_type 2, the nested-dissection LU");
    }
    if (op->Kfac && fac_src && opts->pc_type == 2) {
        if (tree) {
            rc = lsa_ndlu_create_tree(ctx, fac_src, tree->nt, tree->first, tree->size, tree->parent, tree->owner, &op->nd);
            op->nd_dist = rc == LSA_OK;
            if (rc == LSA_ERR_OOM) {
                lsa_op_destroy(op);
                return rc;
            }
        } else
            rc = lsa_ndlu_create(ctx, fac_src, 0, &op->nd);
        if (rc == LSA_OK && op->nd) {
            double sa = 1.0;
            (void)lsa_ndlu_info(op->nd, nullptr, nullptr, nullptr, nullptr, nullptr, nullptr, nullptr, &sa, nullptr);
            op->st.analysis_reused = sa == 0.0 ? 1 : 0;
        }
        if (rc == LSA_ERR_OOM) {
            fprintf(stderr, "[lsa_hip] exact LU does not fit the device memory (%s): falling back to ILU(%d) + GMRES\n", ctx->err.c_str(),
                    opts->ilu_levels);
            lu_fell_back = true;
            op->st.pc_fallback = 1;
        } else if (rc != LSA_OK) {
            lsa_op_destroy(op);
            return rc;
        }
    }
    if (op->Kfac && fac_src && (opts->pc_type == 1 || lu_fell_back)) {
        rc = lsa_ilu_create(ctx, fac_src, opts->ilu_levels, opts->ilu_shift, &op->pc);
        if (rc != LSA_OK) {
            lsa_op_destroy(op);
            return rc;
        }
    }
    const size_t tb = (size_t)std::max<int64_t>(op->n, 1) * 16;
    if (hipMalloc(&op->t, tb) != hipSuccess || hipMemsetAsync(op->t, 0, tb, ctx->stream) != hipSuccess) {
        lsa_op_destroy(op);
        return lsa_set_error(ctx, LSA_ERR_HIP, "lsa_op_create: out of device memory");
    }
    if (op->Kfac && op->nd && fac_src && fac_src->nnz > 0) {
        double* nr = (double*)op->t;
        double v2 = 0.0;
        if (k_nrm2(ctx, fac_src->dtype, fac_src->nnz, fac_src->val, nr) == LSA_OK &&
            hipMemcpyAsync(&v2, nr, sizeof v2, hipMemcpyDeviceToHost, ctx->stream) == hipSuccess && hipStreamSynchronize(ctx->stream) == hipSuccess &&
            std::isfinite(v2))
            op->normF = std::sqrt(v2);
        (void)hipMemsetAsync(op->t, 0, sizeof(double), ctx->stream);
    }
    op->st.seconds_factor = now_s() - t0;
    *out = op;
    return LSA_OK;
}

int lsa_op_create(lsa_ctx* ctx, const lsa_mat* A, const lsa_mat* M, const double sigma[2], int mode, const lsa_op_options* opts,
                  lsa_op** out) {
    return op_build(ctx, A, M, nullptr, nullptr, sigma, mode, opts, out);
}

int lsa_op_create_sharded(lsa_ctx* ctx, const lsa_mat* A_rows, const lsa_mat* M_rows, const lsa_mat* A_diag, const lsa_mat* M_diag,
                          const double sigma[2], int mode, const lsa_op_options* opts, lsa_op** out) {
    if (!A_diag) return lsa_set_error(ctx, LSA_ERR_ARG, "lsa_op_create_sharded: the diagonal block of A is required");
    return op_build(ctx, A_rows, M_rows, A_diag, M_diag, sigma, mode, opts, out);
}

int lsa_op_create_dist(lsa_ctx* ctx, const lsa_mat* A, const lsa_mat* M, int32_t row0, int32_t row1, int32_t ntree, const int32_t* first,
                       const int32_t* size, const int32_t* parent, const int32_t* owner, const double sigma[2], int mode, const lsa_op_options* opts,
                       lsa_op** out) {
    if (!first || !size || !parent || !owner || ntree < 1) return lsa_set_error(ctx, LSA_ERR_ARG, "lsa_op_create_dist: the forest is required");
    const TreeArg tree{ntree, first, size, parent, owner, row0, row1};
    return op_build(ctx, A, M, nullptr, nullptr, sigma, mode, opts, out, &tree);
}

void lsa_op_destroy(lsa_op* op) {
    if (!op) return;
    if (op->ctx && op->ctx->stream) (void)hipStreamSynchronize(op->ctx->stream);
    if (op->pc) lsa_ilu_destroy(op->pc);
    if (op->nd) lsa_ndlu_destroy(op->nd);
    if (op->view_fac) lsa_mat_destroy(op->view_fac);
    if (op->view_mul) lsa_mat_destroy(op->view_mul);
    if (op->owned) lsa_mat_destroy(op->owned);
    if (op->owned_mul) lsa_mat_destroy(op->owned_mul);
    if (op->owned_diag) lsa_mat_destroy(op->owned_diag);
    if (op->gw_ready) op->gw.release();
    if (op->t) (void)hipFree(op->t);
    if (op->keep) (void)hipFree(op->keep);
    delete op;
}

static int op_apply_dev(lsa_ctx* ctx, lsa_op* op, const void* x, void* y) {
    const int dtype = LSA_C128;
    ++op->st.op_applies;
    const void* rhs = x;
    if (op->Kmul) {
        void* dst = op->Kfac ? op->t : y;
        LSA_CHECK(spmv_global(ctx, op->Kmul, dtype, x, dst, op->adjoint));
        ++op->st.spmv_calls;
        rhs = dst;
    }
    if (!op->Kfac) {
        if (!op->Kmul) LSA_CHECK(k_copy(ctx, dtype, op->n, x, y));
        if (op->keep) LSA_CHECK(k_mask(ctx, dtype, op->n, op->keep, y));
        return LSA_OK;
    }
    if (!op->gw_ready) {
        int restart = std::max(1, std::min(op->opts.ksp_restart, op->opts.ksp_maxit));
        if (op->nd && (ctx->nranks == 1 || op->nd_dist)) restart = std::min(restart, 40);
        LSA_CHECK(op->gw.alloc(ctx, op->n, restart, dtype));
        op->gw_ready = true;
    }
    LSA_CHECK(gmres_run(ctx, op->Kfac, pc_of(op), dtype, rhs, y, false, op->opts.ksp_rtol, op->opts.ksp_maxit, op->gw, nullptr, nullptr, &op->st));
    if (op->keep) LSA_CHECK(k_mask(ctx, dtype, op->n, op->keep, y));
    return LSA_OK;
}

int lsa_op_set_adjoint(lsa_ctx* ctx, lsa_op* op, int on) {
    if (!ctx || !op) return lsa_set_error(ctx, LSA_ERR_ARG, "lsa_op_set_adjoint: null argument");
    if (on && (!op->nd || !op->Kfac || (ctx->nranks != 1 && !op->nd_dist)))
        return lsa_set_error(ctx, LSA_ERR_ARG, "lsa_op_set_adjoint: needs the nested-dissection LU (pc_type 2) of a factorising mode, on one rank or in the "
                                                "subtree-parallel layout");
    if (op->nd_dist) {
        op->Kfac = (on || !op->view_fac) ? op->owned : op->view_fac;
        op->Kmul = (on || !op->view_mul) ? (op->owned_mul ? op->owned_mul : op->M_whole) : op->view_mul;
    }
    op->adjoint = on != 0;
    return LSA_OK;
}

int lsa_op_set_projection(lsa_ctx* ctx, lsa_op* op, const double* keep) {
    if (!ctx || !op) return lsa_set_error(ctx, LSA_ERR_ARG, "lsa_op_set_projection: null argument");
    LSA_HIP_CHECK(ctx, hipStreamSynchronize(ctx->stream));
    if (!keep) {
        if (op->keep) (void)hipFree(op->keep);
        op->keep = nullptr;
        return LSA_OK;
    }
    for (int64_t i = 0; i < op->n; ++i)
        if (keep[i] != 0.0 && keep[i] != 1.0) return lsa_set_error(ctx, LSA_ERR_ARG, "lsa_op_set_projection: keep[%lld] is neither 0 nor 1", (long long)i);
    const size_t bytes = sizeof(double) * (size_t)std::max<int64_t>(op->n, 1);
    if (!op->keep) LSA_HIP_CHECK(ctx, hipMalloc((void**)&op->keep, bytes));
    LSA_HIP_CHECK(ctx, hipMemcpy(op->keep, keep, sizeof(double) * (size_t)op->n, hipMemcpyHostToDevice));
    return LSA_OK;
}

int lsa_op_apply(lsa_ctx* ctx, lsa_op* op, const lsa_vec* x, lsa_vec* y) {
    if (!ctx || !op || !x || !y) return lsa_set_error(ctx, LSA_ERR_ARG, "lsa_op_apply: null argument");
    if (x->n != op->n || y->n != op->n || x->dtype != LSA_C128 || y->dtype != LSA_C128 || x->d == y->d)
        return lsa_set_error(ctx, LSA_ERR_ARG, "lsa_op_apply: x and y must be distinct complex vectors of length n");
    const double t0 = now_s();
    int rc = op_apply_dev(ctx, op, x->d, y->d);
    if (rc == LSA_OK) LSA_HIP_CHECK(ctx, hipStreamSynchronize(ctx->stream));
    op->st.seconds_solve += now_s() - t0;
    return rc;
}

}

int lsa_op_get_parts(lsa_op* op, lsa_op_parts* out) {
    if (!op || !out) return LSA_ERR_ARG;
    out->n = op->n;
    out->Kmul = op->Kmul;
    out->Kfac = op->Kfac;
    out->nd = op->nd;
    out->plain = op->Kfac && op->Kfac == op->owned && op->Kmul == op->M_whole && !op->owned_mul && !op->adjoint && !op->keep && !op->nd_dist &&
                 op->ctx->nranks == 1;
    out->ksp_rtol = op->opts.ksp_rtol;
    out->normF = op->normF;
    out->refine = &op->refine;
    out->st = &op->st;
    return LSA_OK;
}

int direct_solve_enqueue(lsa_ctx* ctx, lsa_op* op, int dtype, const void* rhs, void* y, void* z, void* r, bool refine, double* norms) {
    const PcRef pc = pc_of(op);
    const lsa_mat* C = op->Kfac;
    LSA_CHECK(pc_global(ctx, pc, C->row0, op->n, dtype, rhs, y));
    LSA_CHECK(spmv_global(ctx, C, dtype, y, z, op->adjoint));
    if (refine) {
        LSA_CHECK(k_residual_norms(ctx, dtype, op->n, rhs, z, r, norms));
        LSA_CHECK(pc_global(ctx, pc, C->row0, op->n, dtype, r, z));
        const double one[2] = {1.0, 0.0};
        LSA_CHECK(k_axpy(ctx, dtype, op->n, one, z, y));
        LSA_CHECK(spmv_global(ctx, C, dtype, y, z, op->adjoint));
    }
    return LSA_OK;
}

void stats_book_direct_solve(lsa_stats* st, int products, bool refine, double res, double bnorm) {
    ++st->op_applies;
    st->spmv_calls += products + (refine ? 1 : 0);
    st->sptrsv_calls += refine ? 4 : 2;
    if (refine) ++st->refined_solves;
    st->last_rel_res = bnorm > 0.0 ? res / bnorm : 0.0;
    st->max_rel_res = std::max(st->max_rel_res, st->last_rel_res);
}

int basis_upload_row_permutation(lsa_ctx* ctx, const char* who, int64_t n, const int32_t* perm, int32_t** row_perm) {
    LSA_HIP_CHECK(ctx, hipStreamSynchronize(ctx->stream));
    if (*row_perm) (void)hipFree(*row_perm);
    *row_perm = nullptr;
    if (!perm) return LSA_OK;
    std::vector<char> seen((size_t)n, 0);
    for (int64_t i = 0; i < n; ++i) {
        if (perm[i] < 0 || perm[i] >= n || seen[(size_t)perm[i]]) return lsa_set_error(ctx, LSA_ERR_ARG, "%s: not a permutation of 0..n-1", who);
        seen[(size_t)perm[i]] = 1;
    }
    LSA_HIP_ALLOC(ctx, hipMalloc((void**)row_perm, sizeof(int32_t) * (size_t)std::max<int64_t>(n, 1)));
    LSA_HIP_CHECK(ctx, hipMemcpy(*row_perm, perm, sizeof(int32_t) * (size_t)n, hipMemcpyHostToDevice));
    return LSA_OK;
}

int basis_times_host_matrix(lsa_ctx* ctx, int dtype, int64_t n, int m, int k, const void* V, const void* Q, int ldq, void* qdev, void* Out,
                            size_t pinned_extra) {
    const size_t es = esize(dtype), qbytes = (size_t)m * k * es;
    LSA_CHECK(lsa_ensure_scratch(ctx, 0, qbytes + pinned_extra));
    for (int c = 0; c < k; ++c) memcpy((char*)ctx->pinned + (size_t)c * m * es, (const char*)Q + (size_t)c * ldq * es, (size_t)m * es);
    LSA_HIP_CHECK(ctx, hipMemcpyAsync(qdev, ctx->pinned, qbytes, hipMemcpyHostToDevice, ctx->stream));
    return k_basis_gemm(ctx, dtype, n, m, k, V, n, qdev, m, Out, n);
}

extern "C" {

int lsa_op_stats(const lsa_op* op, lsa_stats* out) {
    if (!op || !out) return LSA_ERR_ARG;
    *out = op->st;
    return LSA_OK;
}

int lsa_krylov_create(lsa_ctx* ctx, lsa_op* op, int32_t ncv, lsa_krylov** out) {
    if (!ctx || !op || !out || ncv < 1) return lsa_set_error(ctx, LSA_ERR_ARG, "lsa_krylov_create: bad argument");
    const size_t vb = (size_t)std::max<int64_t>(op->n, 1) * 16;
    const char* be = getenv("LSA_KRYLOV_BATCH");
    const int32_t batch = be && *be ? std::max(0, std::min(atoi(be), 256)) : 16;
    if (lsa_krylov* c = ctx->krylov_cache) {
        ctx->krylov_cache = nullptr;
        if (c->n == op->n && c->ncv == ncv && c->batch == batch) {
            c->op = op;
            c->pipeline = true;
            c->imag_norms.clear();
            (void)hipMemsetAsync(c->w, 0, vb, ctx->stream);
            *out = c;
            return LSA_OK;
        }
        krylov_free(c);
    }
    lsa_krylov* k = new lsa_krylov();
    k->ctx = ctx;
    k->op = op;
    k->n = op->n;
    k->ncv = ncv;
    k->V = k->V2 = k->w = k->qdev = nullptr;
    bool ok = hipMalloc(&k->V, vb * (size_t)(ncv + 1)) == hipSuccess && hipMalloc(&k->V2, vb * (size_t)(ncv + 1)) == hipSuccess &&
              hipMalloc(&k->w, vb) == hipSuccess && hipMalloc(&k->qdev, (size_t)(ncv + 1) * (size_t)(ncv + 1) * 16) == hipSuccess;
    if (!ok || k->ow.alloc(ctx, ncv + 1, LSA_C128) != LSA_OK) {
        lsa_krylov_destroy(k);
        return lsa_set_error(ctx, LSA_ERR_HIP, "lsa_krylov_create: out of device memory (n=%lld, ncv=%d)", (long long)op->n, ncv);
    }
    (void)hipMemsetAsync(k->w, 0, vb, ctx->stream);
    k->hcol.assign((size_t)ncv + 2, zc(0));
    k->batch = batch;
    const size_t slots = (size_t)std::max(batch, 1);
    if (hipMalloc(&k->Hdev, slots * krylov_slot_bytes(ncv)) != hipSuccess || hipMalloc((void**)&k->checks, slots * 2 * sizeof(double)) != hipSuccess) {
        lsa_krylov_destroy(k);
        return lsa_set_error(ctx, LSA_ERR_HIP, "lsa_krylov_create: out of device memory (pipeline buffers)");
    }
    k->pipeline = true;
    *out = k;
    return LSA_OK;
}

void lsa_krylov_destroy(lsa_krylov* k) {
    if (!k) return;
    lsa_ctx* ctx = k->ctx;
    if (ctx && ctx->stream) (void)hipStreamSynchronize(ctx->stream);
    if (k->row_perm) (void)hipFree(k->row_perm);
    k->row_perm = nullptr;
    k->op = nullptr;
    if (ctx && k->V && k->V2 && k->w && k->qdev && k->ow.h1 && !getenv("LSA_KRYLOV_NO_CACHE")) {
        if (ctx->krylov_cache) krylov_free(ctx->krylov_cache);
        ctx->krylov_cache = k;
        return;
    }
    krylov_free(k);
}

void lsa_krylov_drop_cache(lsa_ctx* ctx) {
    if (ctx && ctx->krylov_cache) {
        krylov_free(ctx->krylov_cache);
        ctx->krylov_cache = nullptr;
    }
}

int lsa_krylov_shape(const lsa_krylov* k, int64_t* n, int32_t* ncv) {
    if (!k) return LSA_ERR_ARG;
    if (n) *n = k->n;
    if (ncv) *ncv = k->ncv;
    return LSA_OK;
}

int lsa_krylov_set_row_permutation(lsa_ctx* ctx, lsa_krylov* k, const int32_t* perm) {
    if (!ctx || !k) return lsa_set_error(ctx, LSA_ERR_ARG, "lsa_krylov_set_row_permutation: null argument");
    return basis_upload_row_permutation(ctx, "lsa_krylov_set_row_permutation", k->n, perm, &k->row_perm);
}

int lsa_krylov_set_start(lsa_ctx* ctx, lsa_krylov* k, const void* host_v) {
    if (!ctx || !k || !host_v) return lsa_set_error(ctx, LSA_ERR_ARG, "lsa_krylov_set_start: null argument");
    LSA_HIP_CHECK(ctx, hipMemcpyAsync(k->w, host_v, (size_t)k->n * 16, hipMemcpyHostToDevice, ctx->stream));
    double nrm = 0.0;
    LSA_CHECK(device_norm(ctx, LSA_C128, k->n, k->w, k->ow.nrm2, &nrm));
    if (!(nrm > 0.0) || !std::isfinite(nrm)) return lsa_set_error(ctx, LSA_ERR_ARG, "lsa_krylov_set_start: start vector is zero or not finite");
    LSA_CHECK(k_scale_by_inv_norm(ctx, LSA_C128, k->n, k->w, k->ow.nrm2, k->V));
    LSA_HIP_CHECK(ctx, hipStreamSynchronize(ctx->stream));
    return LSA_OK;
}

int lsa_krylov_inject(lsa_ctx* ctx, lsa_krylov* k, int32_t j, const void* host_v) {
    if (!ctx || !k || !host_v) return lsa_set_error(ctx, LSA_ERR_ARG, "lsa_krylov_inject: null argument");
    if (j < 0 || j > k->ncv) return lsa_set_error(ctx, LSA_ERR_ARG, "lsa_krylov_inject: index %d out of range", j);
    if (j == 0) return lsa_krylov_set_start(ctx, k, host_v);
    const size_t vb = (size_t)k->n * 16;
    LSA_HIP_CHECK(ctx, hipMemcpyAsync(k->w, host_v, vb, hipMemcpyHostToDevice, ctx->stream));
    LSA_CHECK(orthonormalize(ctx, LSA_C128, k->n, k->V, k->n, j, k->w, (char*)k->V + (size_t)j * vb, k->ow, k->hcol.data()));
    const double beta = k->hcol[j].real();
    if (!(beta > 0.0) || !std::isfinite(beta)) return lsa_set_error(ctx, LSA_ERR_ARG, "lsa_krylov_inject: vector lies in the span of the basis");
    return LSA_OK;
}

enum class Orth {
    cgs2_fused,
    cgs2_staged,
    dcgs2,
};
struct StepPlan {
    bool pipelined = false;
    Orth orth = Orth::cgs2_fused;
    bool tail = false;
};

static StepPlan step_plan(lsa_ctx* ctx, const lsa_krylov* k) {
    const KrylovSwitches& sw = krylov_switches();
    const lsa_op* op = k->op;
    StepPlan p;
    if (!sw.fused) p.orth = Orth::cgs2_staged;
    else if (sw.delayed && ctx->nranks == 1 && !op->adjoint && op->n == k->n && k_dcgs2_fits(k->n, k->ncv)) p.orth = Orth::dcgs2;
    p.pipelined = k->pipeline && (k->batch > 1 || p.orth == Orth::dcgs2) && op->Kfac && op->nd && !op->pc &&
                  !(ctx->nranks > 1 && (!op->nd_dist || ctx->host_gather));
    p.tail = p.pipelined && sw.tail && sw.fused && op->Kmul && !op->adjoint && !op->keep && !op->refine && op->n == k->n &&
             k_cgs2_tail_fits(ctx, k->n, k->ncv, op->Kmul, op->Kfac);
    return p;
}

static int krylov_enqueue_step(lsa_ctx* ctx, lsa_krylov* k, const StepPlan& plan, int32_t j, int32_t slot, bool first) {
    lsa_op* op = k->op;
    const int dtype = LSA_C128;
    const size_t vb = (size_t)k->n * 16;
    const void* vj = (char*)k->V + (size_t)j * vb;
    void* vn = (char*)k->V + (size_t)(j + 1) * vb;
    void* sl = (char*)k->Hdev + (size_t)slot * krylov_slot_bytes(k->ncv);
    double* chk = k->checks + 2 * (size_t)slot;
    const bool dcgs2 = plan.orth == Orth::dcgs2;
    if (plan.orth != Orth::cgs2_staged) LSA_CHECK(k->ow.ensure_fused(ctx, k->n));
    if (plan.tail) {
        if (k->t_for != j) LSA_CHECK(spmv_global(ctx, op->Kmul, dtype, vj, op->t, false));
        k->t_for = -1;
        LSA_CHECK(pc_global(ctx, pc_of(op), op->Kfac->row0, op->n, dtype, op->t, k->w));
        double* parts = k->tail_parts + (size_t)slot * 2 * (size_t)k->tail_nparts;
        if (dcgs2) {
            LSA_CHECK(k_dcgs2_step(ctx, k->n, j, k->V, k->n, k->w, first ? 1 : 0, sl, k->ncv, k->ow.fused, nullptr, nullptr, nullptr));
            LSA_CHECK(k_dcgs2_tail(ctx, k->n, j, k->V, k->n, k->w, k->ow.fused, op->Kmul, op->Kfac, op->t, parts, sl, k->ncv));
        } else {
            LSA_CHECK(k_cgs2_fused_tail(ctx, k->n, j + 1, k->V, k->n, k->w, k->w2, vn, sl, k->ow.fused, op->Kmul, op->Kfac, op->t, parts));
        }
        k->t_for = j + 1;
        return LSA_OK;
    }
    k->t_for = -1;
    const void* rhs = vj;
    if (op->Kmul) {
        LSA_CHECK(spmv_global(ctx, op->Kmul, dtype, vj, op->t, op->adjoint));
        rhs = op->t;
    }
    LSA_CHECK(direct_solve_enqueue(ctx, op, dtype, rhs, k->w, op->gw.z, op->gw.w, op->refine, chk));
    const SolveCheck check{rhs, op->gw.z, op->gw.w, chk};
    const bool rides = plan.orth != Orth::cgs2_staged;
    if (!rides) LSA_CHECK(k_residual_norms(ctx, dtype, op->n, check.b, check.z, check.r, check.out));
    if (op->keep) LSA_CHECK(k_mask(ctx, dtype, op->n, op->keep, k->w));
    if (dcgs2) {
        LSA_CHECK(k_dcgs2_step(ctx, k->n, j, k->V, k->n, k->w, first ? 1 : 0, sl, k->ncv, k->ow.fused, check.b, check.z, check.out));
        return k_dcgs2_norm(ctx, k->n, k->ow.fused, sl, k->ncv);
    }
    return orthonormalize_enqueue(ctx, dtype, k->n, k->V, k->n, j + 1, k->w, vn, k->ow, sl, rides ? &check : nullptr);
}

struct HessView {
    cplx* Hh;
    int32_t ldh, j0, ncv;
    cplx* col(int32_t j) const { return Hh + (size_t)j * ldh; }
};

static int judge_norm(double beta, const cplx* col, int32_t rows) {
    if (!std::isfinite(beta)) return -1;
    double colmax = 0.0;
    for (int32_t i = 0; i < rows; ++i) colmax = std::max(colmax, std::hypot(col[i].re, col[i].im));
    return beta <= 1e-14 * std::max(colmax, 1e-300) ? 1 : 0;
}

static int take_column(const HessView& H, int32_t j, const cplx* h) {
    cplx* Hj = H.col(j);
    for (int32_t i = 0; i < H.ldh; ++i) Hj[i] = i <= j + 1 ? h[i] : cplx{0.0, 0.0};
    return judge_norm(h[j + 1].re, h, j + 1);
}

static int finish_column(const HessView& H, int32_t jc, const cplx* sl) {
    cplx* Hp = H.col(jc - 1);
    const double nu = sl[2 * H.ncv].re;
    for (int32_t i = 0; i < jc; ++i) Hp[i] = cplx{Hp[i].re + sl[i].re, Hp[i].im + sl[i].im};
    Hp[jc] = cplx{nu, 0.0};
    return judge_norm(nu, Hp, jc);
}

static int provisional_column(const HessView& H, int32_t jc, const cplx* sl, bool first, cplx* h) {
    const int32_t ncv = H.ncv;
    const double inv = 1.0 / sl[2 * ncv].re;
    for (int32_t i = 0; i < jc; ++i) h[i] = sl[ncv + i];
    h[jc] = sl[2 * ncv + 1];
    if (!first) {
        for (int32_t c = 0; c < jc; ++c) {
            const cplx a = sl[c];
            const cplx* Hc = H.col(c);
            const int32_t rows = std::min(jc, std::max(H.j0, c + 1));
            for (int32_t i = 0; i <= rows; ++i) {
                h[i].re -= Hc[i].re * a.re - Hc[i].im * a.im;
                h[i].im -= Hc[i].re * a.im + Hc[i].im * a.re;
            }
        }
        for (int32_t i = 0; i <= jc; ++i) h[i] = cplx{h[i].re * inv, h[i].im * inv};
    }
    h[jc + 1] = cplx{sl[2 * ncv + 2].re, 0.0};
    return take_column(H, jc, h);
}

static int arnoldi_nonfinite(lsa_ctx* ctx, int32_t j) { return lsa_set_error(ctx, LSA_ERR_NONFINITE, "Arnoldi: non-finite norm at step %d", j); }

static int extend_pipelined(lsa_ctx* ctx, lsa_krylov* k, const HessView& H, int32_t* jp, int32_t j1, int32_t* breakdown) {
    lsa_op* op = k->op;
    StepPlan plan = step_plan(ctx, k);
    if (!op->gw_ready) {
        LSA_CHECK(op->gw.alloc(ctx, op->n, std::max(1, std::min({op->opts.ksp_restart, op->opts.ksp_maxit, 40})), LSA_C128));
        op->gw_ready = true;
    }
    const int32_t slots = std::max(k->batch, 1);
    const size_t colb = krylov_slot_bytes(k->ncv);
    LSA_CHECK(lsa_ensure_scratch(ctx, 0, (size_t)slots * (colb + 2 * sizeof(double))));
    if (plan.tail && !k->tail_parts) {
        k->tail_nparts = k_cgs2_tail_parts(k->n);
        LSA_HIP_ALLOC(ctx, hipMalloc(&k->w2, (size_t)k->n * 16));
        LSA_HIP_ALLOC(ctx, hipMalloc((void**)&k->tail_parts, (size_t)slots * 2 * (size_t)k->tail_nparts * sizeof(double)));
    }
    const bool delayed = plan.orth == Orth::dcgs2;
    const double rtol = op->opts.ksp_rtol;
    char* host = (char*)ctx->pinned;
    cplx* hwork = (cplx*)k->hcol.data();
    k->t_for = -1;
    bool pending = false;
    int32_t j = *jp;
    for (; j < j1 && plan.pipelined; plan = step_plan(ctx, k)) {
        const int32_t nb = std::min<int32_t>(slots, j1 - j);
        const double tq = now_s();
        for (int32_t s = 0; s < nb; ++s) {
            const int rc = krylov_enqueue_step(ctx, k, plan, j + s, s, s == 0 && !pending);
            if (rc != LSA_OK) {
                (void)hipStreamSynchronize(ctx->stream);
                return rc;
            }
        }
        if (plan.tail) LSA_CHECK(k_cgs2_tail_checks(ctx, nb, k->tail_nparts, k->tail_parts, k->checks));
        LSA_HIP_CHECK(ctx, hipMemcpyAsync(host, k->Hdev, (size_t)nb * colb, hipMemcpyDeviceToHost, ctx->stream));
        LSA_HIP_CHECK(ctx, hipMemcpyAsync(host + (size_t)slots * colb, k->checks, (size_t)nb * 2 * sizeof(double), hipMemcpyDeviceToHost, ctx->stream));
        const double tw = now_s();
        LSA_HIP_CHECK(ctx, hipStreamSynchronize(ctx->stream));
        if (krylov_switches().timing) fprintf(stderr, "[lsa_krylov] %d steps queued in %.3f ms, waited %.3f ms\n", nb, 1e3 * (tw - tq), 1e3 * (now_s() - tw));
        const double* chk = (const double*)(host + (size_t)slots * colb);
        int32_t accepted = 0;
        for (int32_t s = 0; s < nb; ++s, ++accepted) {
            const cplx* hc = (const cplx*)(host + (size_t)s * colb);
            const bool first = s == 0 && !pending;
            if (delayed && !first) {
                pending = false;
                const int what = finish_column(H, j + s, hc);
                if (what < 0) return arnoldi_nonfinite(ctx, j + s - 1);
                if (what > 0) {
                    *breakdown = j + s - 1;
                    return LSA_OK;
                }
            }
            const double beta0 = std::sqrt(chk[2 * s]), bnorm = std::sqrt(chk[2 * s + 1]);
            if (!(beta0 <= rtol * bnorm)) {
                if (!op->refine && std::isfinite(beta0)) op->refine = true;
                else k->pipeline = false;
                break;
            }
            stats_book_direct_solve(&op->st, op->Kmul ? 2 : 1, op->refine, beta0, bnorm);
            const int what = delayed ? provisional_column(H, j + s, hc, first, hwork) : take_column(H, j + s, hc);
            pending = delayed;
            if (what < 0) return arnoldi_nonfinite(ctx, j + s);
            if (what > 0) {
                *breakdown = j + s;
                return LSA_OK;
            }
        }
        j += accepted;
        if (accepted < nb) k->t_for = -1;
    }
    *jp = j;
    if (pending) {
        LSA_CHECK(k_dcgs2_step(ctx, k->n, j, k->V, k->n, nullptr, 0, k->Hdev, k->ncv, k->ow.fused, nullptr, nullptr, nullptr));
        LSA_HIP_CHECK(ctx, hipMemcpyAsync(host, k->Hdev, colb, hipMemcpyDeviceToHost, ctx->stream));
        LSA_HIP_CHECK(ctx, hipStreamSynchronize(ctx->stream));
        const int what = finish_column(H, j, (const cplx*)host);
        if (what < 0) return arnoldi_nonfinite(ctx, j - 1);
        if (what > 0) *breakdown = j - 1;
    }
    return LSA_OK;
}

static int extend_one_step(lsa_ctx* ctx, lsa_krylov* k, const HessView& H, int32_t j, int32_t j1, int32_t* breakdown) {
    const size_t vb = (size_t)k->n * 16;
    k->t_for = -1;
    for (; j < j1; ++j) {
        const void* vj = (char*)k->V + (size_t)j * vb;
        void* vn = (char*)k->V + (size_t)(j + 1) * vb;
        LSA_CHECK(op_apply_dev(ctx, k->op, vj, k->w));
        LSA_CHECK(orthonormalize(ctx, LSA_C128, k->n, k->V, k->n, j + 1, k->w, vn, k->ow, k->hcol.data()));
        const int what = take_column(H, j, (const cplx*)k->hcol.data());
        if (what < 0) return arnoldi_nonfinite(ctx, j);
        if (what > 0) {
            *breakdown = j;
            break;
        }
    }
    return LSA_OK;
}

int lsa_krylov_extend(lsa_ctx* ctx, lsa_krylov* k, int32_t j0, int32_t j1, void* H, int32_t ldh, int32_t* breakdown) {
    if (!ctx || !k || !H) return lsa_set_error(ctx, LSA_ERR_ARG, "lsa_krylov_extend: null argument");
    if (j0 < 0 || j1 < j0 || j1 > k->ncv || ldh < j1 + 1) return lsa_set_error(ctx, LSA_ERR_ARG, "lsa_krylov_extend: bad step range [%d, %d) for ncv %d", j0, j1, k->ncv);
    const double t0 = now_s();
    const HessView Hv{(cplx*)H, ldh, j0, k->ncv};
    int32_t j = j0, bd = -1;
    int rc = LSA_OK;
    if (step_plan(ctx, k).pipelined) rc = extend_pipelined(ctx, k, Hv, &j, j1, &bd);
    if (rc == LSA_OK && bd < 0) rc = extend_one_step(ctx, k, Hv, j, j1, &bd);
    if (breakdown) *breakdown = bd;
    k->op->st.seconds_solve += now_s() - t0;
    return rc;
}

int lsa_krylov_restart(lsa_ctx* ctx, lsa_krylov* k, int32_t m, int32_t knew, const void* Q, int32_t ldq) {
    if (!ctx || !k || !Q) return lsa_set_error(ctx, LSA_ERR_ARG, "lsa_krylov_restart: null argument");
    if (m < 1 || m > k->ncv || knew < 0 || knew > m || ldq < m) return lsa_set_error(ctx, LSA_ERR_ARG, "lsa_krylov_restart: bad sizes m=%d knew=%d", m, knew);
    const size_t vb = (size_t)k->n * 16;
    if (knew > 0) LSA_CHECK(basis_times_host_matrix(ctx, LSA_C128, k->n, m, knew, k->V, Q, ldq, k->qdev, k->V2, 0));
    LSA_CHECK(k_copy(ctx, LSA_C128, k->n, (char*)k->V + (size_t)m * vb, (char*)k->V2 + (size_t)knew * vb));
    LSA_HIP_CHECK(ctx, hipStreamSynchronize(ctx->stream));
    std::swap(k->V, k->V2);
    return LSA_OK;
}

int lsa_krylov_ritz_vectors(lsa_ctx* ctx, lsa_krylov* k, int32_t m, int32_t nvec, const void* Y, int32_t ldy, int normalise,
                            void* X) {
    if (!ctx || !k || !Y || !X) return lsa_set_error(ctx, LSA_ERR_ARG, "lsa_krylov_ritz_vectors: null argument");
    if (m < 1 || m > k->ncv + 1 || nvec < 0 || nvec > k->ncv + 1 || ldy < m) return lsa_set_error(ctx, LSA_ERR_ARG, "lsa_krylov_ritz_vectors: bad sizes");
    if (nvec == 0) return LSA_OK;
    const size_t vb = (size_t)k->n * 16;
    LSA_CHECK(basis_times_host_matrix(ctx, LSA_C128, k->n, m, nvec, k->V, Y, ldy, k->qdev, k->V2, (size_t)nvec * sizeof(double)));
    k->imag_norms.clear();
    if (normalise & 2) {
        if (!k->imag2) LSA_HIP_ALLOC(ctx, hipMalloc((void**)&k->imag2, (size_t)(k->ncv + 2) * sizeof(double)));
        LSA_CHECK(k_columns_canonical(ctx, k->n, nvec, k->V2, k->n, normalise & 1, k->imag2));
        k->imag_norms.assign((size_t)nvec, 0.0);
        LSA_HIP_CHECK(ctx, hipMemcpyAsync((char*)ctx->pinned + (size_t)m * nvec * 16, k->imag2, (size_t)nvec * sizeof(double), hipMemcpyDeviceToHost, ctx->stream));
    } else if (normalise) {
        for (int32_t c = 0; c < nvec; ++c) {
            void* col = (char*)k->V2 + (size_t)c * vb;
            LSA_CHECK(k_nrm2(ctx, LSA_C128, k->n, col, k->ow.nrm2));
            LSA_CHECK(k_copy(ctx, LSA_C128, k->n, col, k->w));
            LSA_CHECK(k_scale_by_inv_norm(ctx, LSA_C128, k->n, k->w, k->ow.nrm2, col));
        }
    }
    const void* src = k->V2;
    void* tmp = nullptr;
    if (k->row_perm) {
        if (!k->xtmp) LSA_HIP_ALLOC(ctx, hipMalloc(&k->xtmp, vb * (size_t)(k->ncv + 1)));
        tmp = k->xtmp;
        LSA_CHECK(k_scatter_rows(ctx, LSA_C128, k->n, nvec, k->row_perm, k->V2, tmp));
        src = tmp;
    }
    hipError_t e = hipMemcpyAsync(X, src, vb * (size_t)nvec, hipMemcpyDeviceToHost, ctx->stream);
    if (e == hipSuccess) e = hipStreamSynchronize(ctx->stream);
    if (e != hipSuccess) return lsa_set_error(ctx, LSA_ERR_HIP, "lsa_krylov_ritz_vectors: download failed: %s", hipGetErrorString(e));
    for (size_t c = 0; c < k->imag_norms.size(); ++c) k->imag_norms[c] = std::sqrt(((const double*)((const char*)ctx->pinned + (size_t)m * nvec * 16))[c]);
    return LSA_OK;
}

int lsa_krylov_imag_norms(const lsa_krylov* k, int32_t nvec, double* out) {
    if (!k || !out || nvec < 0 || (size_t)nvec > k->imag_norms.size()) return LSA_ERR_ARG;
    for (int32_t c = 0; c < nvec; ++c) out[c] = k->imag_norms[(size_t)c];
    return LSA_OK;
}

int lsa_eig_residuals(lsa_ctx* ctx, const lsa_mat* A, const lsa_mat* M, int32_t nvec, const void* lam, const void* X, double* res) {
    if (!ctx || !A || !lam || !X || !res || nvec < 0) return lsa_set_error(ctx, LSA_ERR_ARG, "lsa_eig_residuals: bad argument");
    const int64_t n = A->n;
    const size_t vb = (size_t)std::max<int64_t>(n, 1) * 16;
    void *x = nullptr, *ax = nullptr, *mx = nullptr;
    double* nr = nullptr;
    int rc = LSA_OK;
    if (hipMalloc(&x, vb) != hipSuccess || hipMalloc(&ax, vb) != hipSuccess || hipMalloc(&mx, vb) != hipSuccess ||
        hipMalloc((void**)&nr, 4 * sizeof(double)) != hipSuccess)
        rc = lsa_set_error(ctx, LSA_ERR_HIP, "lsa_eig_residuals: out of device memory");
    const cplx* lamh = (const cplx*)lam;
    for (int32_t c = 0; c < nvec && rc == LSA_OK; ++c) {
        double nax = 0, nmx = 0, nrr = 0;
        if (hipMemcpyAsync(x, (const char*)X + (size_t)c * (size_t)n * 16, (size_t)n * 16, hipMemcpyHostToDevice, ctx->stream) != hipSuccess) {
            rc = lsa_set_error(ctx, LSA_ERR_HIP, "lsa_eig_residuals: upload failed");
            break;
        }
        rc = k_spmv(ctx, A, LSA_C128, x, ax);
        if (rc == LSA_OK) rc = M ? k_spmv(ctx, M, LSA_C128, x, mx) : k_copy(ctx, LSA_C128, n, x, mx);
        if (rc == LSA_OK) rc = device_norm(ctx, LSA_C128, n, ax, nr, &nax);
        if (rc == LSA_OK) rc = device_norm(ctx, LSA_C128, n, mx, nr, &nmx);
        const double ml[2] = {-lamh[c].re, -lamh[c].im};
        if (rc == LSA_OK) rc = k_axpy(ctx, LSA_C128, n, ml, mx, ax);
        if (rc == LSA_OK) rc = device_norm(ctx, LSA_C128, n, ax, nr, &nrr);
        const double lmag = std::hypot(lamh[c].re, lamh[c].im);
        res[c] = nrr / (nax + lmag * nmx + 1e-16);
    }
    (void)hipStreamSynchronize(ctx->stream);
    for (void* p : {x, ax, mx, (void*)nr})
        if (p) (void)hipFree(p);
    return rc;
}

}
```

### lsa-fw_amd/lsa_hip/__init__.py

```python

from __future__ import annotations

import ctypes
import os
from pathlib import Path

import numpy as np

LSA_F64, LSA_C128 = 0, 1

_STATUS_NAMES = {
    0: "LSA_OK",
    -1: "LSA_ERR_ARG",
    -2: "LSA_ERR_HIP",
    -3: "LSA_ERR_ZERO_PIVOT",
    -4: "LSA_ERR_DIVERGED",
    -5: "LSA_ERR_NONFINITE",
    -6: "LSA_ERR_TIMEOUT",
    -7: "LSA_ERR_COMM",
    -8: "LSA_ERR_OOM",
}

globals().update({name: code for code, name in _STATUS_NAMES.items()})

LIB_PATH = Path(os.environ.get("LSA_HIP_LIB", Path(__file__).resolve().parent / "liblsa_hip.so"))


class LsaError(RuntimeError):

    def __init__(self, status: int, message: str):
        super().__init__(f"{_STATUS_NAMES.get(status, status)}: {message}")
        self.status = status


class lsa_stats(ctypes.Structure):
    _fields_ = [
        ("op_applies", ctypes.c_int64),
        ("gmres_iters", ctypes.c_int64),
        ("spmv_calls", ctypes.c_int64),
        ("sptrsv_calls", ctypes.c_int64),
        ("last_rel_res", ctypes.c_double),
        ("max_rel_res", ctypes.c_double),
        ("seconds_factor", ctypes.c_double),
        ("seconds_solve", ctypes.c_double),
        ("stagnated_solves", ctypes.c_int32),
        ("pc_fallback", ctypes.c_int32),
        ("backward_accepted", ctypes.c_int32),
        ("analysis_reused", ctypes.c_int32),
        ("refined_solves", ctypes.c_int32),
        ("reserved0", ctypes.c_int32),
    ]


class lsa_op_options(ctypes.Structure):
    _fields_ = [
        ("ilu_levels", ctypes.c_int32),
        ("ilu_shift", ctypes.c_double),
        ("ksp_rtol", ctypes.c_double),
        ("ksp_restart", ctypes.c_int32),
        ("ksp_maxit", ctypes.c_int32),
        ("pc_type", ctypes.c_int32),
        ("antishift", ctypes.c_double * 2),
    ]


class lsa_ks_options(ctypes.Structure):
    _fields_ = [
        ("nev", ctypes.c_int32),
        ("max_restarts", ctypes.c_int32),
        ("tol", ctypes.c_double),
        ("which", ctypes.c_int32),
        ("transform", ctypes.c_int32),
        ("sigma", ctypes.c_double * 2),
        ("antishift", ctypes.c_double * 2),
        ("target", ctypes.c_double * 2),
        ("seed", ctypes.c_uint64),
        ("keep_fraction", ctypes.c_double),
    ]


class lsa_ks_result(ctypes.Structure):
    _fields_ = [
        ("nconv", ctypes.c_int32),
        ("nout", ctypes.c_int32),
        ("restarts", ctypes.c_int32),
        ("pad", ctypes.c_int32),
        ("op_applies", ctypes.c_int64),
        ("next_unconverged", ctypes.c_double),
        ("seconds_expand", ctypes.c_double),
        ("seconds_dense", ctypes.c_double),
        ("seconds_restart", ctypes.c_double),
    ]


_P = ctypes.c_void_p
_I32, _I64, _DBL = ctypes.c_int32, ctypes.c_int64, ctypes.c_double
_PP = ctypes.POINTER(ctypes.c_void_p)

SIGNATURES = {
    "lsa_ctx_create": (ctypes.c_int, [ctypes.c_int, _PP]),
    "lsa_ctx_destroy": (None, [_P]),
    "lsa_last_error": (ctypes.c_char_p, [_P]),
    "lsa_ctx_synchronize": (ctypes.c_int, [_P]),
    "lsa_ctx_arch": (ctypes.c_char_p, [_P]),
    "lsa_vec_create": (ctypes.c_int, [_P, _I64, ctypes.c_int, _PP]),
    "lsa_vec_destroy": (None, [_P]),
    "lsa_vec_upload": (ctypes.c_int, [_P, _P, _P]),
    "lsa_vec_download": (ctypes.c_int, [_P, _P, _P]),
    "lsa_csr_upload": (ctypes.c_int, [_P, _I32, _I64, _P, _P, _P, ctypes.c_int, _PP]),
    "lsa_mat_destroy": (None, [_P]),
    "lsa_mat_download_values": (ctypes.c_int, [_P, _P, _P]),
    "lsa_csr_axpby": (ctypes.c_int, [_P, _P, _P, _DBL * 2, _DBL * 2, ctypes.c_int, _PP]),
    "lsa_spmv": (ctypes.c_int, [_P, _P, _P, _P]),
    "lsa_spmv_transpose": (ctypes.c_int, [_P, _P, ctypes.c_int, _P, _P]),
    "lsa_spmv_info": (ctypes.c_int, [_P, _P, ctypes.c_int, ctypes.c_char_p, _I32, ctypes.POINTER(_I64)]),
    "lsa_spmv_time": (ctypes.c_int, [_P, _P, _P, _P, ctypes.c_int, ctypes.POINTER(_DBL)]),
    "lsa_ilu_create": (ctypes.c_int, [_P, _P, ctypes.c_int, _DBL, _PP]),
    "lsa_ilu_destroy": (None, [_P]),
    "lsa_ilu_set_algorithm": (ctypes.c_int, [_P, _P, ctypes.c_int, _I32]),
    "lsa_ilu_solve": (ctypes.c_int, [_P, _P, ctypes.c_int, _P, _P]),
    "lsa_ilu_solve_time": (ctypes.c_int, [_P, _P, ctypes.c_int, _P, _P, ctypes.c_int, ctypes.POINTER(_DBL)]),
    "lsa_ilu_info": (ctypes.c_int, [_P, ctypes.POINTER(_I64), ctypes.POINTER(_I32), ctypes.POINTER(_I32), ctypes.POINTER(_I32)]),
    "lsa_ilu_download": (ctypes.c_int, [_P, _P, _P, _P, _P]),
    "lsa_nd_analyse": (ctypes.c_int, [_I32, _P, _P, _I32, _P, _PP]),
    "lsa_nd_order": (ctypes.c_int, [_I32, _P, _P, _I32, _P, _PP]),
    "lsa_nd_analyse_tree": (ctypes.c_int, [_I32, _P, _P, _I32, _P, _P, _P, _P, _I32, _I32, _PP]),
    "lsa_nd_sym_export_dist": (ctypes.c_int, [_P, _P, _P, _P, _P, _P, _P, _P]),
    "lsa_nd_sym_export_top": (ctypes.c_int, [_P, _P, _P, _P, _P]),
    "lsa_ndlu_inertia": (ctypes.c_int, [_P, _P, ctypes.POINTER(_I64), ctypes.POINTER(_I64), ctypes.POINTER(_I64)]),
    "lsa_dense_sym_inertia": (ctypes.c_int, [_I32, _P, _I32, _DBL, ctypes.POINTER(_I64), ctypes.POINTER(_I64), ctypes.POINTER(_I64)]),
    "lsa_nd_sym_error": (ctypes.c_char_p, [_P]),
    "lsa_nd_sym_destroy": (None, [_P]),
    "lsa_nd_sym_info": (ctypes.c_int, [_P, ctypes.POINTER(_I32), ctypes.POINTER(_I32), ctypes.POINTER(_I32), ctypes.POINTER(_I64),
                                       ctypes.POINTER(_I64), ctypes.POINTER(_I64), ctypes.POINTER(_DBL)]),
    "lsa_nd_sym_export": (ctypes.c_int, [_P, _P, _P, _P, _P, _P, _P]),
    "lsa_nd_sym_memory": (ctypes.c_int, [_P, _I32, _I64, _P, _P, _P, _P]),
    "lsa_nd_sym_export_tables": (ctypes.c_int, [_P, _P, _P, _P, _P, _P, _P]),
    "lsa_ndlu_create": (ctypes.c_int, [_P, _P, _I32, _PP]),
    "lsa_ndlu_prepare": (ctypes.c_int, [_P, _P, ctypes.c_int, _I32, _P]),
    "lsa_ndlu_prepare_tree": (ctypes.c_int, [_P, _P, ctypes.c_int, _I32, _P, _P, _P]),
    "lsa_ndlu_create_tree": (ctypes.c_int, [_P, _P, _I32, _P, _P, _P, _P, _PP]),
    "lsa_ndlu_refactor": (ctypes.c_int, [_P, _P, _P]),
    "lsa_ndlu_destroy": (None, [_P]),
    "lsa_ndlu_solve": (ctypes.c_int, [_P, _P, _P, _P]),
    "lsa_ndlu_solve_batch": (ctypes.c_int, [_P, _I32, _PP, _PP, _PP]),
    "lsa_ndlu_solve_adjoint": (ctypes.c_int, [_P, _P, ctypes.c_int, _P, _P]),
    "lsa_ndlu_solve_time": (ctypes.c_int, [_P, _P, _P, _P, ctypes.c_int, ctypes.POINTER(_DBL)]),
    "lsa_ndlu_info": (ctypes.c_int, [_P, ctypes.POINTER(_I32), ctypes.POINTER(_I32), ctypes.POINTER(_I32), ctypes.POINTER(_I64),
                                     ctypes.POINTER(_I64), ctypes.POINTER(_I64), ctypes.POINTER(_I32), ctypes.POINTER(_DBL), ctypes.POINTER(_DBL)]),
    "lsa_gmres": (ctypes.c_int, [_P, _P, _P, _P, _P, ctypes.c_int, _DBL, ctypes.c_int, ctypes.c_int, ctypes.POINTER(_I32), ctypes.POINTER(_DBL)]),
    "lsa_op_create": (ctypes.c_int, [_P, _P, _P, _DBL * 2, ctypes.c_int, ctypes.POINTER(lsa_op_options), _PP]),
    "lsa_op_create_sharded": (ctypes.c_int, [_P, _P, _P, _P, _P, _DBL * 2, ctypes.c_int, ctypes.POINTER(lsa_op_options), _PP]),
    "lsa_op_create_dist": (ctypes.c_int, [_P, _P, _P, _I32, _I32, _I32, _P, _P, _P, _P, _DBL * 2, ctypes.c_int, ctypes.POINTER(lsa_op_options), _PP]),
    "lsa_op_destroy": (None, [_P]),
    "lsa_op_apply": (ctypes.c_int, [_P, _P, _P, _P]),
    "lsa_op_stats": (ctypes.c_int, [_P, ctypes.POINTER(lsa_stats)]),
    "lsa_op_set_adjoint": (ctypes.c_int, [_P, _P, ctypes.c_int]),
    "lsa_op_set_projection": (ctypes.c_int, [_P, _P, _P]),
    "lsa_krylov_create": (ctypes.c_int, [_P, _P, _I32, _PP]),
    "lsa_krylov_destroy": (None, [_P]),
    "lsa_krylov_set_row_permutation": (ctypes.c_int, [_P, _P, _P]),
    "lsa_krylov_set_start": (ctypes.c_int, [_P, _P, _P]),
    "lsa_krylov_inject": (ctypes.c_int, [_P, _P, _I32, _P]),
    "lsa_krylov_extend": (ctypes.c_int, [_P, _P, _I32, _I32, _P, _I32, ctypes.POINTER(_I32)]),
    "lsa_krylov_restart": (ctypes.c_int, [_P, _P, _I32, _I32, _P, _I32]),
    "lsa_krylov_ritz_vectors": (ctypes.c_int, [_P, _P, _I32, _I32, _P, _I32, ctypes.c_int, _P]),
    "lsa_krylov_imag_norms": (ctypes.c_int, [_P, _I32, _P]),
    "lsa_krylov_shape": (ctypes.c_int, [_P, ctypes.POINTER(_I64), ctypes.POINTER(_I32)]),
    "lsa_mat_rows": (_I64, [_P]),
    "lsa_krylov_solve": (ctypes.c_int, [_P, _P, _P, _P, _P, _I32, _P, _P, _P, _P, _P]),
    "lsa_eigs_sinvert": (ctypes.c_int, [_P, _P, _P, _DBL * 2, _I32, _I32, _DBL, _I32, ctypes.POINTER(lsa_op_options), _P, _P, _I32, _P, _P, _P, _P, _P]),
    "lsa_dense_schur": (ctypes.c_int, [_I32, _P, _I32, _P, _I32]),
    "lsa_dense_schur_reorder": (ctypes.c_int, [_I32, _P, _I32, _P, _I32, _P, ctypes.POINTER(_I32)]),
    "lsa_dense_tri_eigenvectors": (ctypes.c_int, [_I32, _P, _I32, _P, _I32]),
    "lsa_eig_residuals": (ctypes.c_int, [_P, _P, _P, _I32, _P, _P, _P]),
    "lsa_lanczos_create": (ctypes.c_int, [_P, _P, _I32, _PP]),
    "lsa_lanczos_destroy": (None, [_P]),
    "lsa_lanczos_set_row_permutation": (ctypes.c_int, [_P, _P, _P]),
    "lsa_lanczos_set_start": (ctypes.c_int, [_P, _P, _P]),
    "lsa_lanczos_extend": (ctypes.c_int, [_P, _P, _I32, _I32, _P, _I32, ctypes.POINTER(_I32)]),
    "lsa_lanczos_basis": (ctypes.c_int, [_P, _P, _I32, _P]),
    "lsa_lanczos_solve": (ctypes.c_int, [_P, _P, ctypes.POINTER(lsa_ks_options), _P, _I32, _P, _P, _P, _P, ctypes.POINTER(lsa_ks_result)]),
    "lsa_dense_syev": (ctypes.c_int, [_I32, _P, _I32, _P]),
    "lsa_mm_open": (ctypes.c_int, [ctypes.c_char_p, _PP, ctypes.POINTER(_I32), ctypes.POINTER(_I32), ctypes.POINTER(_I64), ctypes.POINTER(ctypes.c_int)]),
    "lsa_mm_read_csr": (ctypes.c_int, [_P, _P, _P, _P]),
    "lsa_mm_error": (ctypes.c_char_p, [_P]),
    "lsa_mm_close": (None, [_P]),
# ... 15 lines not shown
        return _lib
    if not LIB_PATH.exists():
        raise RuntimeError(
            f"{LIB_PATH} is missing: build it with `make -C lsa-fw_amd/csrc` (or __graft_entry__.build()). "
            "There is no CPU fallback for the eigen path."
        )
    lib = ctypes.CDLL(str(LIB_PATH))
    for name, (restype, argtypes) in SIGNATURES.items():
        fn = getattr(lib, name)
        fn.restype = restype
        fn.argtypes = argtypes
    _lib = lib
    return lib


def _ptr(a: np.ndarray):
    return a.ctypes.data_as(ctypes.c_void_p)


def _dtype_code(dt) -> int:
    dt = np.dtype(dt)
    if dt == np.float64:
        return LSA_F64
    if dt == np.complex128:
        return LSA_C128
    raise ValueError(f"unsupported dtype {dt}: use float64 or complex128")


def _np_dtype(code: int):
    return np.complex128 if code == LSA_C128 else np.float64


_host_blas_limit = None


def _calm_host_blas() -> None:
    global _host_blas_limit
    want = os.environ.get("LSA_HOST_BLAS_THREADS", "keep")
    if _host_blas_limit is not None or want == "keep":
        return
    try:
        from threadpoolctl import threadpool_limits

        _host_blas_limit = threadpool_limits(limits=max(1, int(want)), user_api="blas")
    except Exception:
        _host_blas_limit = False


class Context:

    def __init__(self, device: int = 0):
        self._lib = load_library()
        _calm_host_blas()
        h = ctypes.c_void_p()
        rc = self._lib.lsa_ctx_create(int(device), ctypes.byref(h))
        if rc != 0:
            raise RuntimeError(
                f"lsa_ctx_create(device={device}) failed with {_STATUS_NAMES.get(rc, rc)}: no usable AMD GPU. "
                "The eigen path has no CPU fallback."
            )
        self.handle = h
        self.device = device

    @property
    def arch(self) -> str:
        return self._lib.lsa_ctx_arch(self.handle).decode()

    def check(self, rc: int) -> None:
        if rc == 0:
            return
        msg = self._lib.lsa_last_error(self.handle).decode(errors="replace")
        if rc == -1:
            raise ValueError(msg)
        raise LsaError(rc, msg)

    def synchronize(self) -> None:
        self.check(self._lib.lsa_ctx_synchronize(self.handle))

    def close(self) -> None:
        if getattr(self, "handle", None):
            self._lib.lsa_ctx_destroy(self.handle)
            self.handle = None

    def unique_id(self) -> bytes:
        buf = ctypes.create_string_buffer(128)
        rc = self._lib.lsa_comm_unique_id(buf)
        if rc != 0:
            raise LsaError(rc, "RCCL unavailable")
        return buf.raw

    def comm_init(self, nranks: int, rank: int, uid: bytes) -> None:
        buf = ctypes.create_string_buffer(uid, 128)
        self.check(self._lib.lsa_comm_init(self.handle, nranks, rank, buf))

    def comm_init_host(self, nranks: int, rank: int, exchange) -> None:

        def _cb(host_buf, bytes_per_rank, _user):
            try:
                view = np.ctypeslib.as_array((ctypes.c_uint8 * (int(bytes_per_rank) * nranks)).from_address(host_buf))
                exchange(view.reshape(nranks, int(bytes_per_rank)))
                return 0
            except Exception:
                import traceback

                traceback.print_exc()
                return 1

        self._host_cb = _HOST_GATHER_FN(_cb)
        self.check(self._lib.lsa_comm_init_host(self.handle, nranks, rank, ctypes.cast(self._host_cb, ctypes.c_void_p), None))

    def comm_selftest(self, nbytes: int = 1 << 20) -> None:
        self.check(self._lib.lsa_comm_selftest(self.handle, int(nbytes)))

    def comm_stats(self) -> dict:
        calls, nbytes = _I64(0), _I64(0)
        self._lib.lsa_comm_stats(self.handle, ctypes.byref(calls), ctypes.byref(nbytes))
        return {"allgather_calls": calls.value, "allgather_bytes_received": nbytes.value}


class DeviceVector:
    def __init__(self, ctx: Context, n: int, dtype=np.complex128):
        self.ctx = ctx
        self.n = int(n)
        self.dtype = np.dtype(dtype)
        h = ctypes.c_void_p()
        ctx.check(ctx._lib.lsa_vec_create(ctx.handle, self.n, _dtype_code(dtype), ctypes.byref(h)))
        self.handle = h

    @classmethod
    def from_numpy(cls, ctx: Context, a: np.ndarray) -> "DeviceVector":
        a = np.ascontiguousarray(a)
        if a.dtype not in (np.float64, np.complex128):
            a = a.astype(np.complex128 if a.dtype.kind == "c" else np.float64)
        v = cls(ctx, a.shape[0], a.dtype)
        v.upload(a)
        return v

    def upload(self, a: np.ndarray) -> None:
        a = np.ascontiguousarray(a, dtype=self.dtype)
        if a.shape != (self.n,):
            raise ValueError(f"expected shape ({self.n},), got {a.shape}")
        self.ctx.check(self.ctx._lib.lsa_vec_upload(self.ctx.handle, self.handle, _ptr(a)))

    def numpy(self) -> np.ndarray:
        out = np.empty(self.n, dtype=self.dtype)
        self.ctx.check(self.ctx._lib.lsa_vec_download(self.ctx.handle, self.handle, _ptr(out)))
        return out

    def __del__(self):
        if getattr(self, "handle", None) and getattr(self.ctx, "handle", None):
            self.ctx._lib.lsa_vec_destroy(self.handle)
            self.handle = None


class CsrMatrix:

    def __init__(self, ctx: Context, handle, shape, nnz: int, dtype, keep=()):
        self.ctx, self.handle, self.shape, self.nnz, self.dtype = ctx, handle, shape, int(nnz), np.dtype(dtype)
        self._keep = keep

    @classmethod
    def from_scipy(cls, ctx: Context, A) -> "CsrMatrix":
        import scipy.sparse as sp

        A = sp.csr_matrix(A)
        if A.shape[0] != A.shape[1]:
            raise ValueError("lsa_csr_upload handles square matrices; use from_scipy_shard for row blocks")
        if not A.has_sorted_indices:
            A = A.copy()
            A.sort_indices()
        dt = np.complex128 if A.dtype.kind == "c" else np.float64
        rp = np.ascontiguousarray(A.indptr, dtype=np.int32)
        ci = np.ascontiguousarray(A.indices, dtype=np.int32)
        val = np.ascontiguousarray(A.data, dtype=dt)
        h = ctypes.c_void_p()
        ctx.check(
            ctx._lib.lsa_csr_upload(ctx.handle, A.shape[0], A.nnz, _ptr(rp), _ptr(ci), _ptr(val), _dtype_code(dt), ctypes.byref(h))
        )
        return cls(ctx, h, A.shape, A.nnz, dt)

    @classmethod
    def from_scipy_shard(cls, ctx: Context, A_rows, n_global: int, row0: int) -> "CsrMatrix":
        import scipy.sparse as sp

        A = sp.csr_matrix(A_rows)
        A.sort_indices()
        dt = np.complex128 if A.dtype.kind == "c" else np.float64
        rp = np.ascontiguousarray(A.indptr, dtype=np.int32)
        ci = np.ascontiguousarray(A.indices, dtype=np.int32)
        val = np.ascontiguousarray(A.data, dtype=dt)
        h = ctypes.c_void_p()
        ctx.check(
            ctx._lib.lsa_csr_upload_shard(
                ctx.handle, n_global, row0, row0 + A.shape[0], A.nnz, _ptr(rp), _ptr(ci), _ptr(val), _dtype_code(dt), ctypes.byref(h)
            )
        )
        return cls(ctx, h, (A.shape[0], n_global), A.nnz, dt)

    def prepare_lu(self, complex_factors: bool, leaf_size: int = 0, constraint=None) -> None:
        flags = None if constraint is None else np.ascontiguousarray(constraint, dtype=np.int8)
# ... 541 lines not shown
```

Before: 556.8.

## Pool operator buffers, stage start vector, speculate restart apply, chunk Ritz download

```diff
diff --git a/include/lsa_hip.h b/include/lsa_hip.h
--- a/include/lsa_hip.h
+++ b/include/lsa_hip.h
@@ -50,6 +50,8 @@
 const char *lsa_last_error(const lsa_ctx *ctx);
 int lsa_ctx_synchronize(lsa_ctx *ctx);
 const char *lsa_ctx_arch(const lsa_ctx *ctx);
+void lsa_op_drop_pool(lsa_ctx *ctx);
+int64_t lsa_pool_bytes(const lsa_ctx *ctx);
 
 int lsa_vec_create(lsa_ctx *ctx, int64_t n, int dtype, lsa_vec **out);
 void lsa_vec_destroy(lsa_vec *v);
diff --git a/lsa-fw_amd/csrc/core.hip b/lsa-fw_amd/csrc/core.hip
--- a/lsa-fw_amd/csrc/core.hip
+++ b/lsa-fw_amd/csrc/core.hip
@@ -29,6 +29,17 @@
         LSA_HIP_CHECK(ctx, hipHostMalloc(&ctx->pinned, want, hipHostMallocDefault));
         ctx->pinned_bytes = want;
     }
+    return LSA_OK;
+}
+
+int lsa_ensure_stage(lsa_ctx* ctx, size_t bytes) {
+    if (bytes <= ctx->stage_bytes) return LSA_OK;
+    LSA_HIP_CHECK(ctx, hipStreamSynchronize(ctx->stream));
+    if (ctx->stage) (void)hipHostFree(ctx->stage);
+    ctx->stage = nullptr;
+    ctx->stage_bytes = 0;
+    LSA_HIP_CHECK(ctx, hipHostMalloc(&ctx->stage, bytes, hipHostMallocDefault));
+    ctx->stage_bytes = bytes;
     return LSA_OK;
 }
 
@@ -86,9 +97,11 @@
     if (ctx->stream) (void)hipStreamSynchronize(ctx->stream);
     lsa_ndlu_drop_cache(ctx);
     lsa_krylov_drop_cache(ctx);
+    lsa_op_drop_pool(ctx);
     comm_release(ctx);
     if (ctx->dscratch) (void)hipFree(ctx->dscratch);
     if (ctx->pinned) (void)hipHostFree(ctx->pinned);
+    if (ctx->stage) (void)hipHostFree(ctx->stage);
     if (ctx->ev0) (void)hipEventDestroy(ctx->ev0);
     if (ctx->ev1) (void)hipEventDestroy(ctx->ev1);
     if (ctx->stream) (void)hipStreamDestroy(ctx->stream);
@@ -258,6 +271,10 @@
 
 extern "C" int lsa_csr_axpby(lsa_ctx* ctx, const lsa_mat* A, const lsa_mat* B, const double alpha[2], const double beta[2],
                              int out_dtype, lsa_mat** out) {
+    return csr_axpby_into(ctx, A, B, alpha, beta, out_dtype, nullptr, out);
+}
+
+int csr_axpby_into(lsa_ctx* ctx, const lsa_mat* A, const lsa_mat* B, const double alpha[2], const double beta[2], int out_dtype, void* val, lsa_mat** out) {
     if (!ctx || !A || !B || !alpha || !beta || !out) return lsa_set_error(ctx, LSA_ERR_ARG, "lsa_csr_axpby: null argument");
     if (A->n != B->n || A->nnz != B->nnz || A->ncols != B->ncols || A->row0 != B->row0)
         return lsa_set_error(ctx, LSA_ERR_ARG, "lsa_csr_axpby: operands must share one sparsity pattern (n %d vs %d, nnz %lld vs %lld)",
@@ -290,8 +307,8 @@
     C->h_hash = A->h_hash;
     if (!A->h_shared) A->h_shared = std::make_shared<PatternShared>();
     C->h_shared = A->h_shared;
-    C->val = nullptr;
-    hipError_t e = hipMalloc(&C->val, (size_t)(C->nnz > 0 ? C->nnz : 1) * dtype_size(out_dtype));
+    C->val = val;
+    hipError_t e = val ? hipSuccess : hipMalloc(&C->val, (size_t)(C->nnz > 0 ? C->nnz : 1) * dtype_size(out_dtype));
     if (e != hipSuccess) {
         delete C;
         return lsa_set_error(ctx, LSA_ERR_HIP, "hipMalloc(axpby result) failed: %s", hipGetErrorString(e));
@@ -305,6 +322,7 @@
     else launch_axpby<cplx, cplx, cplx>(ctx, C->nnz, A->val, B->val, al, be, C->val);
     hipError_t le = hipGetLastError();
     if (le != hipSuccess) {
+        if (val) C->owns_values = false;
         lsa_mat_destroy(C);
         return lsa_set_error(ctx, LSA_ERR_HIP, "axpby launch failed: %s", hipGetErrorString(le));
     }
diff --git a/lsa-fw_amd/csrc/dense.hip b/lsa-fw_amd/csrc/dense.hip
--- a/lsa-fw_amd/csrc/dense.hip
+++ b/lsa-fw_amd/csrc/dense.hip
@@ -773,22 +773,30 @@
     const double keep_fraction = ks_keep_fraction(o);
     const Selector sel{o->which, o->transform, {o->sigma[0], o->sigma[1]}, {o->antishift[0], o->antishift[1]}, {o->target[0], o->target[1]}};
     Rng rng = ks_rng(o);
-    std::vector<Z> vec((size_t)n);
-    auto random_vector = [&]() {
+    std::vector<Z> vec;
+    Z* start = nullptr;
+    LSA_CHECK(krylov_stage_start(ctx, k, (void**)&start));
+    const bool staged = start != nullptr;
+    auto random_vector = [&](Z* dst) {
         for (int64_t i = 0; i < n; ++i) {
-            rng.normal_pair(vec[(size_t)i].re, vec[(size_t)i].im);
-            if (mask && mask[i] == 0.0) vec[(size_t)i] = {0.0, 0.0};
+            rng.normal_pair(dst[i].re, dst[i].im);
+            if (mask && mask[i] == 0.0) dst[i] = {0.0, 0.0};
         }
     };
+    if (!staged) {
+        vec.resize((size_t)n);
+        start = vec.data();
+    }
     if (v0) {
-        memcpy(vec.data(), v0, (size_t)n * sizeof(Z));
+        memcpy(start, v0, (size_t)n * sizeof(Z));
         if (mask)
             for (int64_t i = 0; i < n; ++i)
-                if (mask[i] == 0.0) vec[(size_t)i] = {0.0, 0.0};
+                if (mask[i] == 0.0) start[i] = {0.0, 0.0};
     } else {
-        random_vector();
-    }
-    LSA_CHECK(lsa_krylov_inject(ctx, k, 0, vec.data()));
+        random_vector(start);
+    }
+    if (staged) LSA_CHECK(krylov_start_staged(ctx, k));
+    else LSA_CHECK(lsa_krylov_inject(ctx, k, 0, vec.data()));
     const int ldh = m + 1;
     std::vector<Z> H((size_t)ldh * m, Z{0.0, 0.0}), T((size_t)m * m), Q((size_t)m * m), S((size_t)m * m), b((size_t)m), bq((size_t)m), w((size_t)m);
     std::vector<double> est((size_t)m), rel((size_t)m), keys((size_t)m);
@@ -805,7 +813,8 @@
         return (int)LSA_OK;
     };
     auto inject_random = [&](int j) {
-        random_vector();
+        vec.resize((size_t)n);
+        random_vector(vec.data());
         return lsa_krylov_inject(ctx, k, j, vec.data());
     };
     while (true) {
@@ -816,6 +825,7 @@
             b[(size_t)c] = Hm(m, c);
             for (int r = 0; r < m; ++r) Tm(r, c) = Hm(r, c);
         }
+        if (restarts < o->max_restarts) LSA_CHECK(krylov_speculate_apply(ctx, k, m));
         if (!schur(m, Tm, Qm)) return lsa_set_error(ctx, LSA_ERR_DIVERGED, "Krylov-Schur: the QR algorithm on the projected matrix did not converge");
         tri_eigenvectors(m, Tm, Sm);
         for (int c = 0; c < m; ++c) {
diff --git a/lsa-fw_amd/csrc/lsa_internal.h b/lsa-fw_amd/csrc/lsa_internal.h
--- a/lsa-fw_amd/csrc/lsa_internal.h
+++ b/lsa-fw_amd/csrc/lsa_internal.h
@@ -96,9 +96,25 @@
     int64_t comm_calls = 0, comm_bytes = 0;
     struct lsa_ndlu* nd_cache = nullptr;
     struct lsa_krylov* krylov_cache = nullptr;
+    struct OpPool {
+        void* t = nullptr;
+        size_t t_bytes = 0;
+        void* cval = nullptr;
+        size_t cval_bytes = 0;
+        void* gw = nullptr;
+        size_t gw_bytes = 0;
+        size_t bytes() const { return t_bytes + cval_bytes + gw_bytes; }
+    } op_pool;
+    void* stage = nullptr;
+    size_t stage_bytes = 0;
+    const void* rider_src = nullptr;
+    double rider_dst[2] = {0.0, 0.0};
+    size_t rider_bytes = 0;
 };
 extern "C" void lsa_ndlu_drop_cache(lsa_ctx* ctx);
 extern "C" void lsa_krylov_drop_cache(lsa_ctx* ctx);
+int lsa_ensure_stage(lsa_ctx* ctx, size_t bytes);
+int csr_axpby_into(lsa_ctx* ctx, const lsa_mat* A, const lsa_mat* B, const double alpha[2], const double beta[2], int out_dtype, void* val, lsa_mat** out);
 
 struct lsa_vec {
     lsa_ctx* ctx;
@@ -233,6 +249,9 @@
 int k_scatter_rows(lsa_ctx* ctx, int dtype, int64_t n, int ncols, const int32_t* perm, const void* In, void* Out);
 
 int basis_upload_row_permutation(lsa_ctx* ctx, const char* who, int64_t n, const int32_t* perm, int32_t** row_perm);
+int krylov_stage_start(lsa_ctx* ctx, lsa_krylov* k, void** buf);
+int krylov_start_staged(lsa_ctx* ctx, lsa_krylov* k);
+int krylov_speculate_apply(lsa_ctx* ctx, lsa_krylov* k, int32_t m);
 int basis_times_host_matrix(lsa_ctx* ctx, int dtype, int64_t n, int m, int k, const void* V, const void* Q, int ldq, void* qdev, void* Out,
                             size_t pinned_extra);
 int direct_solve_enqueue(lsa_ctx* ctx, lsa_op* op, int dtype, const void* rhs, void* y, void* z, void* r, bool refine, double* norms);
diff --git a/lsa-fw_amd/csrc/ndlu.hip b/lsa-fw_amd/csrc/ndlu.hip
--- a/lsa-fw_amd/csrc/ndlu.hip
+++ b/lsa-fw_amd/csrc/ndlu.hip
@@ -2173,6 +2173,10 @@
                 break;
             }
     } else {
+        if (ctx->rider_src) {
+            LSA_HIP_CHECK(ctx, hipMemcpyAsync(ctx->rider_dst, ctx->rider_src, ctx->rider_bytes, hipMemcpyDeviceToHost, st));
+            ctx->rider_src = nullptr;
+        }
         LSA_HIP_CHECK(ctx, hipMemcpyAsync(hflag, f->d_flag, sizeof hflag, hipMemcpyDeviceToHost, st));
         LSA_HIP_CHECK(ctx, hipStreamSynchronize(st));
     }
diff --git a/lsa-fw_amd/csrc/solver.hip b/lsa-fw_amd/csrc/solver.hip
--- a/lsa-fw_amd/csrc/solver.hip
+++ b/lsa-fw_amd/csrc/solver.hip
@@ -1,4 +1,5 @@
 #include <algorithm>
+#include <atomic>
 #include <chrono>
 #include <cmath>
 #include <complex>
@@ -57,6 +58,9 @@
         h1 = h2 = hcol = fused = nullptr;
         nrm2 = nullptr;
     }
+    size_t bytes(lsa_ctx* ctx, int64_t n, int dtype) const {
+        return (h1 ? 3 * (size_t)(cap + 2) * esize(dtype) + 4 * sizeof(double) : 0) + (fused ? k_cgs2_fused_work_bytes(ctx, n, cap) : 0);
+    }
 };
 
 struct SolveCheck {
@@ -172,10 +176,14 @@
         const size_t vb = (size_t)std::max<int64_t>(n, 1) * esize(dtype);
         LSA_HIP_CHECK(ctx, hipMalloc(&w, vb));
         LSA_HIP_CHECK(ctx, hipMalloc(&z, vb));
+        LSA_HIP_CHECK(ctx, hipMalloc(&ydev, (size_t)(restart + 2) * esize(dtype)));
+        LSA_CHECK(ow.alloc(ctx, restart + 1, dtype));
+        return reset(ctx);
+    }
+    int reset(lsa_ctx* ctx) {
+        const size_t vb = (size_t)std::max<int64_t>(n, 1) * esize(dtype);
         LSA_HIP_CHECK(ctx, hipMemsetAsync(w, 0, vb, ctx->stream));
         LSA_HIP_CHECK(ctx, hipMemsetAsync(z, 0, vb, ctx->stream));
-        LSA_HIP_CHECK(ctx, hipMalloc(&ydev, (size_t)(restart + 2) * esize(dtype)));
-        LSA_CHECK(ow.alloc(ctx, restart + 1, dtype));
         H.assign((size_t)(restart + 1) * restart, zc(0));
         cs.assign(restart + 1, zc(0));
         sn.assign(restart + 1, zc(0));
@@ -196,7 +204,61 @@
         V = w = z = ydev = nullptr;
         ow.release();
     }
+    void release_basis() {
+        if (V) (void)hipFree(V);
+        V = nullptr;
+    }
+    size_t bytes(lsa_ctx* ctx) const {
+        return 2 * (size_t)std::max<int64_t>(n, 1) * esize(dtype) + (size_t)(restart + 2) * esize(dtype) + ow.bytes(ctx, n, dtype);
+    }
 };
+
+std::atomic<int64_t> g_pool_bytes{0};
+
+void* pool_take(void*& slot, size_t& slot_bytes, size_t want) {
+    void* p = nullptr;
+    if (slot && slot_bytes == want) p = slot;
+    else if (slot) (void)hipFree(slot);
+    g_pool_bytes -= (int64_t)slot_bytes;
+    slot = nullptr;
+    slot_bytes = 0;
+    return p;
+}
+void pool_put(void*& slot, size_t& slot_bytes, void* p, size_t bytes) {
+    (void)pool_take(slot, slot_bytes, 0);
+    slot = p;
+    slot_bytes = p ? bytes : 0;
+    g_pool_bytes += (int64_t)slot_bytes;
+}
+void pool_drop_gw(lsa_ctx* ctx) {
+    if (GmresWork* g = (GmresWork*)ctx->op_pool.gw) {
+        g->release();
+        delete g;
+    }
+    g_pool_bytes -= (int64_t)ctx->op_pool.gw_bytes;
+    ctx->op_pool.gw = nullptr;
+    ctx->op_pool.gw_bytes = 0;
+}
+int pool_take_gw(lsa_ctx* ctx, GmresWork& W, int64_t n, int restart, int dtype) {
+    GmresWork* g = (GmresWork*)ctx->op_pool.gw;
+    if (g && g->n == n && g->restart == restart && g->dtype == dtype) {
+        W = std::move(*g);
+        delete g;
+        g_pool_bytes -= (int64_t)ctx->op_pool.gw_bytes;
+        ctx->op_pool.gw = nullptr;
+        ctx->op_pool.gw_bytes = 0;
+        return W.reset(ctx);
+    }
+    pool_drop_gw(ctx);
+    return W.alloc(ctx, n, restart, dtype);
+}
+void pool_put_gw(lsa_ctx* ctx, GmresWork& W) {
+    pool_drop_gw(ctx);
+    W.release_basis();
+    ctx->op_pool.gw = new GmresWork(std::move(W));
+    ctx->op_pool.gw_bytes = ((GmresWork*)ctx->op_pool.gw)->bytes(ctx);
+    g_pool_bytes += (int64_t)ctx->op_pool.gw_bytes;
+}
 
 int gmres_run(lsa_ctx* ctx, const lsa_mat* C, PcRef pc, int dtype, const void* b, void* x, bool use_x0, double rtol,
               int maxit, GmresWork& W, int32_t* iters_out, double* relres_out, lsa_stats* st) {
@@ -447,6 +509,8 @@
     int64_t n;
     int32_t ncv;
     int32_t* row_perm = nullptr;
+    int32_t* row_perm_dev = nullptr;
+    std::vector<int32_t> row_perm_host;
     void *V, *V2, *w, *qdev;
     OrthWork ow;
     std::vector<zc> hcol;
@@ -454,19 +518,28 @@
     void* xtmp = nullptr;
     std::vector<double> imag_norms;
     void* Hdev = nullptr;
+    double* start_nrm2 = nullptr;
     double* checks = nullptr;
+    bool start_pending = false;
     int32_t batch = 0;
     bool pipeline = false;
     void* w2 = nullptr;
     double* tail_parts = nullptr;
     int32_t tail_nparts = 0;
     int32_t t_for = -1;
+    int32_t solved_for = -1;
+    int32_t spec_col = -1;
 };
 
 static size_t krylov_slot_bytes(int32_t ncv) { return (size_t)(2 * ncv + 4) * 16; }
 
+static int krylov_judge_start(lsa_ctx* ctx, double nrm) {
+    if (!(nrm > 0.0) || !std::isfinite(nrm)) return lsa_set_error(ctx, LSA_ERR_ARG, "lsa_krylov_set_start: start vector is zero or not finite");
+    return LSA_OK;
+}
+
 static void krylov_free(lsa_krylov* k) {
-    for (void* p : {k->V, k->V2, k->w, k->qdev, k->Hdev, (void*)k->checks, (void*)k->imag2, k->xtmp, (void*)k->row_perm, k->w2, (void*)k->tail_parts})
+    for (void* p : {k->V, k->V2, k->w, k->qdev, k->Hdev, (void*)k->imag2, k->xtmp, (void*)k->row_perm_dev, k->w2, (void*)k->tail_parts})
         if (p) (void)hipFree(p);
     k->ow.release();
     delete k;
@@ -492,14 +565,16 @@
     return rc;
 }
 
-static int build_shifted(lsa_ctx* ctx, const lsa_mat* A, const lsa_mat* M, const double sigma[2], bool cdt, lsa_mat** out) {
+static int build_shifted(lsa_ctx* ctx, const lsa_mat* A, const lsa_mat* M, const double sigma[2], bool cdt, lsa_mat** out, bool pooled = false) {
     const bool zshift = sigma[0] == 0.0 && sigma[1] == 0.0;
     const double one[2] = {1.0, 0.0}, ms[2] = {-sigma[0], -sigma[1]}, zero[2] = {0.0, 0.0};
     lsa_mat* C = nullptr;
     int rc;
-    if (M) rc = lsa_csr_axpby(ctx, A, M, one, ms, cdt ? LSA_C128 : LSA_F64, &C);
+    const size_t vbytes = (size_t)std::max<int64_t>(A->nnz, 1) * (cdt ? 16 : 8);
+    void* val = pooled ? pool_take(ctx->op_pool.cval, ctx->op_pool.cval_bytes, vbytes) : nullptr;
+    if (M) rc = csr_axpby_into(ctx, A, M, one, ms, cdt ? LSA_C128 : LSA_F64, val, &C);
     else {
-        rc = lsa_csr_axpby(ctx, A, A, one, zero, cdt ? LSA_C128 : LSA_F64, &C);
+        rc = csr_axpby_into(ctx, A, A, one, zero, cdt ? LSA_C128 : LSA_F64, val, &C);
         if (rc == LSA_OK && !zshift) {
             int32_t* miss = (int32_t*)ctx->dscratch;
             (void)hipMemsetAsync(miss, 0, sizeof(int32_t), ctx->stream);
@@ -514,6 +589,7 @@
     }
     if (rc != LSA_OK) {
         if (C) lsa_mat_destroy(C);
+        else if (val) (void)hipFree(val);
         return rc;
     }
     *out = C;
@@ -557,12 +633,18 @@
     int rc = LSA_OK;
     lsa_mat* C = nullptr;
     if (!(mode == 1 && zshift)) {
-        rc = build_shifted(ctx, A, M, sigma, cdt, &C);
+        rc = build_shifted(ctx, A, M, sigma, cdt, &C, true);
         if (rc != LSA_OK) {
             delete op;
             return rc;
         }
         op->owned = C;
+    }
+    const size_t tb = (size_t)std::max<int64_t>(op->n, 1) * 16;
+    op->t = pool_take(ctx->op_pool.t, ctx->op_pool.t_bytes, tb);
+    if ((!op->t && hipMalloc(&op->t, tb) != hipSuccess) || hipMemsetAsync(op->t, 0, tb, ctx->stream) != hipSuccess) {
+        lsa_op_destroy(op);
+        return lsa_set_error(ctx, LSA_ERR_HIP, "lsa_op_create: out of device memory");
     }
     const lsa_mat* fac_src = nullptr;
     if (mode == 0 || mode == 2) {
@@ -615,6 +697,13 @@
         return lsa_set_error(ctx, LSA_ERR_ARG, "lsa_op_create: pc_type 3 (the banded block LU of round 1) left the product library; it lives on as a "
                                                "cross-check library for the tests (tests/xcheck).  Use pc_type 2, the nested-dissection LU");
     }
+    ctx->rider_src = nullptr;
+    if (op->Kfac && fac_src && opts->pc_type == 2 && fac_src->nnz > 0) {
+        if (k_nrm2(ctx, fac_src->dtype, fac_src->nnz, fac_src->val, (double*)op->t) == LSA_OK) {
+            ctx->rider_src = op->t;
+            ctx->rider_bytes = sizeof(double);
+        }
+    }
     if (op->Kfac && fac_src && opts->pc_type == 2) {
         if (tree) {
             rc = lsa_ndlu_create_tree(ctx, fac_src, tree->nt, tree->first, tree->size, tree->parent, tree->owner, &op->nd);
@@ -647,20 +736,16 @@
             return rc;
         }
     }
-    const size_t tb = (size_t)std::max<int64_t>(op->n, 1) * 16;
-    if (hipMalloc(&op->t, tb) != hipSuccess || hipMemsetAsync(op->t, 0, tb, ctx->stream) != hipSuccess) {
-        lsa_op_destroy(op);
-        return lsa_set_error(ctx, LSA_ERR_HIP, "lsa_op_create: out of device memory");
-    }
     if (op->Kfac && op->nd && fac_src && fac_src->nnz > 0) {
-        double* nr = (double*)op->t;
-        double v2 = 0.0;
-        if (k_nrm2(ctx, fac_src->dtype, fac_src->nnz, fac_src->val, nr) == LSA_OK &&
-            hipMemcpyAsync(&v2, nr, sizeof v2, hipMemcpyDeviceToHost, ctx->stream) == hipSuccess && hipStreamSynchronize(ctx->stream) == hipSuccess &&
-            std::isfinite(v2))
-            op->normF = std::sqrt(v2);
-        (void)hipMemsetAsync(op->t, 0, sizeof(double), ctx->stream);
-    }
+        bool have = false;
+        if (!ctx->rider_src) have = true;
+        else
+            have = hipMemcpyAsync(ctx->rider_dst, op->t, sizeof(double), hipMemcpyDeviceToHost, ctx->stream) == hipSuccess &&
+                   hipStreamSynchronize(ctx->stream) == hipSuccess;
+        if (have && std::isfinite(ctx->rider_dst[0])) op->normF = std::sqrt(ctx->rider_dst[0]);
+    }
+    ctx->rider_src = nullptr;
+    (void)hipMemsetAsync(op->t, 0, sizeof(double), ctx->stream);
     op->st.seconds_factor = now_s() - t0;
     *out = op;
     return LSA_OK;
@@ -692,11 +777,18 @@
     if (op->nd) lsa_ndlu_destroy(op->nd);
     if (op->view_fac) lsa_mat_destroy(op->view_fac);
     if (op->view_mul) lsa_mat_destroy(op->view_mul);
+    lsa_ctx* ctx = op->ctx;
+    if (op->owned && ctx && op->owned->val && op->owned->owns_values) {
+        pool_put(ctx->op_pool.cval, ctx->op_pool.cval_bytes, op->owned->val, (size_t)std::max<int64_t>(op->owned->nnz, 1) * esize(op->owned->dtype));
+        op->owned->owns_values = false;
+    }
     if (op->owned) lsa_mat_destroy(op->owned);
     if (op->owned_mul) lsa_mat_destroy(op->owned_mul);
     if (op->owned_diag) lsa_mat_destroy(op->owned_diag);
-    if (op->gw_ready) op->gw.release();
-    if (op->t) (void)hipFree(op->t);
+    if (op->gw_ready && ctx) pool_put_gw(ctx, op->gw);
+    else if (op->gw_ready) op->gw.release();
+    if (op->t && ctx) pool_put(ctx->op_pool.t, ctx->op_pool.t_bytes, op->t, (size_t)std::max<int64_t>(op->n, 1) * 16);
+    else if (op->t) (void)hipFree(op->t);
     if (op->keep) (void)hipFree(op->keep);
     delete op;
 }
@@ -719,7 +811,7 @@
     if (!op->gw_ready) {
         int restart = std::max(1, std::min(op->opts.ksp_restart, op->opts.ksp_maxit));
         if (op->nd && (ctx->nranks == 1 || op->nd_dist)) restart = std::min(restart, 40);
-        LSA_CHECK(op->gw.alloc(ctx, op->n, restart, dtype));
+        LSA_CHECK(pool_take_gw(ctx, op->gw, op->n, restart, dtype));
         op->gw_ready = true;
     }
     LSA_CHECK(gmres_run(ctx, op->Kfac, pc_of(op), dtype, rhs, y, false, op->opts.ksp_rtol, op->opts.ksp_maxit, op->gw, nullptr, nullptr, &op->st));
@@ -850,6 +942,8 @@
         if (c->n == op->n && c->ncv == ncv && c->batch == batch) {
             c->op = op;
             c->pipeline = true;
+            c->start_pending = false;
+            c->spec_col = -1;
             c->imag_norms.clear();
             (void)hipMemsetAsync(c->w, 0, vb, ctx->stream);
             *out = c;
@@ -873,10 +967,12 @@
     k->hcol.assign((size_t)ncv + 2, zc(0));
     k->batch = batch;
     const size_t slots = (size_t)std::max(batch, 1);
-    if (hipMalloc(&k->Hdev, slots * krylov_slot_bytes(ncv)) != hipSuccess || hipMalloc((void**)&k->checks, slots * 2 * sizeof(double)) != hipSuccess) {
+    if (hipMalloc(&k->Hdev, slots * krylov_slot_bytes(ncv) + 2 * sizeof(double) + slots * 2 * sizeof(double)) != hipSuccess) {
         lsa_krylov_destroy(k);
         return lsa_set_error(ctx, LSA_ERR_HIP, "lsa_krylov_create: out of device memory (pipeline buffers)");
     }
+    k->start_nrm2 = (double*)((char*)k->Hdev + slots * krylov_slot_bytes(ncv));
+    k->checks = k->start_nrm2 + 2;
     k->pipeline = true;
     *out = k;
     return LSA_OK;
@@ -886,7 +982,6 @@
     if (!k) return;
     lsa_ctx* ctx = k->ctx;
     if (ctx && ctx->stream) (void)hipStreamSynchronize(ctx->stream);
-    if (k->row_perm) (void)hipFree(k->row_perm);
     k->row_perm = nullptr;
     k->op = nullptr;
     if (ctx && k->V && k->V2 && k->w && k->qdev && k->ow.h1 && !getenv("LSA_KRYLOV_NO_CACHE")) {
@@ -904,6 +999,15 @@
     }
 }
 
+void lsa_op_drop_pool(lsa_ctx* ctx) {
+    if (!ctx) return;
+    (void)pool_take(ctx->op_pool.t, ctx->op_pool.t_bytes, 0);
+    (void)pool_take(ctx->op_pool.cval, ctx->op_pool.cval_bytes, 0);
+    pool_drop_gw(ctx);
+}
+
+int64_t lsa_pool_bytes(const lsa_ctx* ctx) { return ctx ? (int64_t)ctx->op_pool.bytes() : g_pool_bytes.load(); }
+
 int lsa_krylov_shape(const lsa_krylov* k, int64_t* n, int32_t* ncv) {
     if (!k) return LSA_ERR_ARG;
     if (n) *n = k->n;
@@ -913,15 +1017,27 @@
 
 int lsa_krylov_set_row_permutation(lsa_ctx* ctx, lsa_krylov* k, const int32_t* perm) {
     if (!ctx || !k) return lsa_set_error(ctx, LSA_ERR_ARG, "lsa_krylov_set_row_permutation: null argument");
-    return basis_upload_row_permutation(ctx, "lsa_krylov_set_row_permutation", k->n, perm, &k->row_perm);
+    k->row_perm = nullptr;
+    if (!perm) return LSA_OK;
+    if (k->row_perm_dev && (int64_t)k->row_perm_host.size() == k->n && memcmp(k->row_perm_host.data(), perm, sizeof(int32_t) * (size_t)k->n) == 0) {
+        k->row_perm = k->row_perm_dev;
+        return LSA_OK;
+    }
+    k->row_perm_host.clear();
+    LSA_CHECK(basis_upload_row_permutation(ctx, "lsa_krylov_set_row_permutation", k->n, perm, &k->row_perm_dev));
+    k->row_perm_host.assign(perm, perm + k->n);
+    k->row_perm = k->row_perm_dev;
+    return LSA_OK;
 }
 
 int lsa_krylov_set_start(lsa_ctx* ctx, lsa_krylov* k, const void* host_v) {
     if (!ctx || !k || !host_v) return lsa_set_error(ctx, LSA_ERR_ARG, "lsa_krylov_set_start: null argument");
+    k->start_pending = false;
+    k->spec_col = -1;
     LSA_HIP_CHECK(ctx, hipMemcpyAsync(k->w, host_v, (size_t)k->n * 16, hipMemcpyHostToDevice, ctx->stream));
     double nrm = 0.0;
     LSA_CHECK(device_norm(ctx, LSA_C128, k->n, k->w, k->ow.nrm2, &nrm));
-    if (!(nrm > 0.0) || !std::isfinite(nrm)) return lsa_set_error(ctx, LSA_ERR_ARG, "lsa_krylov_set_start: start vector is zero or not finite");
+    LSA_CHECK(krylov_judge_start(ctx, nrm));
     LSA_CHECK(k_scale_by_inv_norm(ctx, LSA_C128, k->n, k->w, k->ow.nrm2, k->V));
     LSA_HIP_CHECK(ctx, hipStreamSynchronize(ctx->stream));
     return LSA_OK;
@@ -931,6 +1047,7 @@
     if (!ctx || !k || !host_v) return lsa_set_error(ctx, LSA_ERR_ARG, "lsa_krylov_inject: null argument");
     if (j < 0 || j > k->ncv) return lsa_set_error(ctx, LSA_ERR_ARG, "lsa_krylov_inject: index %d out of range", j);
     if (j == 0) return lsa_krylov_set_start(ctx, k, host_v);
+    k->spec_col = -1;
     const size_t vb = (size_t)k->n * 16;
     LSA_HIP_CHECK(ctx, hipMemcpyAsync(k->w, host_v, vb, hipMemcpyHostToDevice, ctx->stream));
     LSA_CHECK(orthonormalize(ctx, LSA_C128, k->n, k->V, k->n, j, k->w, (char*)k->V + (size_t)j * vb, k->ow, k->hcol.data()));
@@ -975,8 +1092,8 @@
     if (plan.orth != Orth::cgs2_staged) LSA_CHECK(k->ow.ensure_fused(ctx, k->n));
     if (plan.tail) {
         if (k->t_for != j) LSA_CHECK(spmv_global(ctx, op->Kmul, dtype, vj, op->t, false));
-        k->t_for = -1;
-        LSA_CHECK(pc_global(ctx, pc_of(op), op->Kfac->row0, op->n, dtype, op->t, k->w));
+        if (k->t_for != j || k->solved_for != j) LSA_CHECK(pc_global(ctx, pc_of(op), op->Kfac->row0, op->n, dtype, op->t, k->w));
+        k->t_for = k->solved_for = -1;
         double* parts = k->tail_parts + (size_t)slot * 2 * (size_t)k->tail_nparts;
         if (dcgs2) {
             LSA_CHECK(k_dcgs2_step(ctx, k->n, j, k->V, k->n, k->w, first ? 1 : 0, sl, k->ncv, k->ow.fused, nullptr, nullptr, nullptr));
@@ -987,7 +1104,7 @@
         k->t_for = j + 1;
         return LSA_OK;
     }
-    k->t_for = -1;
+    k->t_for = k->solved_for = -1;
     const void* rhs = vj;
     if (op->Kmul) {
         LSA_CHECK(spmv_global(ctx, op->Kmul, dtype, vj, op->t, op->adjoint));
@@ -1059,12 +1176,12 @@
     lsa_op* op = k->op;
     StepPlan plan = step_plan(ctx, k);
     if (!op->gw_ready) {
-        LSA_CHECK(op->gw.alloc(ctx, op->n, std::max(1, std::min({op->opts.ksp_restart, op->opts.ksp_maxit, 40})), LSA_C128));
+        LSA_CHECK(pool_take_gw(ctx, op->gw, op->n, std::max(1, std::min({op->opts.ksp_restart, op->opts.ksp_maxit, 40})), LSA_C128));
         op->gw_ready = true;
     }
     const int32_t slots = std::max(k->batch, 1);
     const size_t colb = krylov_slot_bytes(k->ncv);
-    LSA_CHECK(lsa_ensure_scratch(ctx, 0, (size_t)slots * (colb + 2 * sizeof(double))));
+    LSA_CHECK(lsa_ensure_scratch(ctx, 0, (size_t)slots * (colb + 2 * sizeof(double)) + 2 * sizeof(double)));
     if (plan.tail && !k->tail_parts) {
         k->tail_nparts = k_cgs2_tail_parts(k->n);
         LSA_HIP_ALLOC(ctx, hipMalloc(&k->w2, (size_t)k->n * 16));
@@ -1074,7 +1191,8 @@
     const double rtol = op->opts.ksp_rtol;
     char* host = (char*)ctx->pinned;
     cplx* hwork = (cplx*)k->hcol.data();
-    k->t_for = -1;
+    k->t_for = k->solved_for = plan.tail && k->spec_col == *jp ? *jp : -1;
+    k->spec_col = -1;
     bool pending = false;
     int32_t j = *jp;
     for (; j < j1 && plan.pipelined; plan = step_plan(ctx, k)) {
@@ -1088,12 +1206,15 @@
             }
         }
         if (plan.tail) LSA_CHECK(k_cgs2_tail_checks(ctx, nb, k->tail_nparts, k->tail_parts, k->checks));
-        LSA_HIP_CHECK(ctx, hipMemcpyAsync(host, k->Hdev, (size_t)nb * colb, hipMemcpyDeviceToHost, ctx->stream));
-        LSA_HIP_CHECK(ctx, hipMemcpyAsync(host + (size_t)slots * colb, k->checks, (size_t)nb * 2 * sizeof(double), hipMemcpyDeviceToHost, ctx->stream));
+        LSA_HIP_CHECK(ctx, hipMemcpyAsync(host, k->Hdev, (size_t)slots * colb + 2 * sizeof(double) + (size_t)nb * 2 * sizeof(double), hipMemcpyDeviceToHost, ctx->stream));
         const double tw = now_s();
         LSA_HIP_CHECK(ctx, hipStreamSynchronize(ctx->stream));
         if (krylov_switches().timing) fprintf(stderr, "[lsa_krylov] %d steps queued in %.3f ms, waited %.3f ms\n", nb, 1e3 * (tw - tq), 1e3 * (now_s() - tw));
-        const double* chk = (const double*)(host + (size_t)slots * colb);
+        if (k->start_pending) {
+            k->start_pending = false;
+            LSA_CHECK(krylov_judge_start(ctx, std::sqrt(*(const double*)(host + (size_t)slots * colb))));
+        }
+        const double* chk = (const double*)(host + (size_t)slots * colb + 2 * sizeof(double));
         int32_t accepted = 0;
         for (int32_t s = 0; s < nb; ++s, ++accepted) {
             const cplx* hc = (const cplx*)(host + (size_t)s * colb);
@@ -1139,7 +1260,7 @@
 
 static int extend_one_step(lsa_ctx* ctx, lsa_krylov* k, const HessView& H, int32_t j, int32_t j1, int32_t* breakdown) {
     const size_t vb = (size_t)k->n * 16;
-    k->t_for = -1;
+    k->t_for = k->solved_for = k->spec_col = -1;
     for (; j < j1; ++j) {
         const void* vj = (char*)k->V + (size_t)j * vb;
         void* vn = (char*)k->V + (size_t)(j + 1) * vb;
@@ -1163,6 +1284,13 @@
     int32_t j = j0, bd = -1;
     int rc = LSA_OK;
     if (step_plan(ctx, k).pipelined) rc = extend_pipelined(ctx, k, Hv, &j, j1, &bd);
+    if (rc == LSA_OK && k->start_pending) {
+        k->start_pending = false;
+        double v2 = 0.0;
+        LSA_HIP_CHECK(ctx, hipMemcpyAsync(&v2, k->start_nrm2, sizeof v2, hipMemcpyDeviceToHost, ctx->stream));
+        LSA_HIP_CHECK(ctx, hipStreamSynchronize(ctx->stream));
+        rc = krylov_judge_start(ctx, std::sqrt(v2));
+    }
     if (rc == LSA_OK && bd < 0) rc = extend_one_step(ctx, k, Hv, j, j1, &bd);
     if (breakdown) *breakdown = bd;
     k->op->st.seconds_solve += now_s() - t0;
@@ -1173,6 +1301,7 @@
     if (!ctx || !k || !Q) return lsa_set_error(ctx, LSA_ERR_ARG, "lsa_krylov_restart: null argument");
     if (m < 1 || m > k->ncv || knew < 0 || knew > m || ldq < m) return lsa_set_error(ctx, LSA_ERR_ARG, "lsa_krylov_restart: bad sizes m=%d knew=%d", m, knew);
     const size_t vb = (size_t)k->n * 16;
+    k->spec_col = k->spec_col == m ? knew : -1;
     if (knew > 0) LSA_CHECK(basis_times_host_matrix(ctx, LSA_C128, k->n, m, knew, k->V, Q, ldq, k->qdev, k->V2, 0));
     LSA_CHECK(k_copy(ctx, LSA_C128, k->n, (char*)k->V + (size_t)m * vb, (char*)k->V2 + (size_t)knew * vb));
     LSA_HIP_CHECK(ctx, hipStreamSynchronize(ctx->stream));
@@ -1185,6 +1314,7 @@
     if (!ctx || !k || !Y || !X) return lsa_set_error(ctx, LSA_ERR_ARG, "lsa_krylov_ritz_vectors: null argument");
     if (m < 1 || m > k->ncv + 1 || nvec < 0 || nvec > k->ncv + 1 || ldy < m) return lsa_set_error(ctx, LSA_ERR_ARG, "lsa_krylov_ritz_vectors: bad sizes");
     if (nvec == 0) return LSA_OK;
+    k->spec_col = -1;
     const size_t vb = (size_t)k->n * 16;
     LSA_CHECK(basis_times_host_matrix(ctx, LSA_C128, k->n, m, nvec, k->V, Y, ldy, k->qdev, k->V2, (size_t)nvec * sizeof(double)));
     k->imag_norms.clear();
@@ -1209,9 +1339,27 @@
         LSA_CHECK(k_scatter_rows(ctx, LSA_C128, k->n, nvec, k->row_perm, k->V2, tmp));
         src = tmp;
     }
-    hipError_t e = hipMemcpyAsync(X, src, vb * (size_t)nvec, hipMemcpyDeviceToHost, ctx->stream);
+    const int32_t cols = (int32_t)std::max<size_t>(1, std::min<size_t>((size_t)nvec, ((size_t)2 << 20) / std::max<size_t>(vb, 1)));
+    const int32_t nchunks = (nvec + cols - 1) / cols;
+    LSA_CHECK(lsa_ensure_stage(ctx, 2 * (size_t)cols * vb));
+    const hipEvent_t done[2] = {ctx->ev0, ctx->ev1};
+    auto chunk_cols = [&](int32_t c) { return std::min<int32_t>(cols, nvec - c * cols); };
+    auto fetch = [&](int32_t c) {
+        hipError_t e = hipMemcpyAsync((char*)ctx->stage + (size_t)(c & 1) * cols * vb, (const char*)src + (size_t)c * cols * vb, (size_t)chunk_cols(c) * vb,
+                                      hipMemcpyDeviceToHost, ctx->stream);
+        return e == hipSuccess ? hipEventRecord(done[c & 1], ctx->stream) : e;
+    };
+    hipError_t e = fetch(0);
+    for (int32_t c = 0; c < nchunks && e == hipSuccess; ++c) {
+        if (c + 1 < nchunks) e = fetch(c + 1);
+        if (e == hipSuccess) e = hipEventSynchronize(done[c & 1]);
+        if (e == hipSuccess) memcpy((char*)X + (size_t)c * cols * vb, (const char*)ctx->stage + (size_t)(c & 1) * cols * vb, (size_t)chunk_cols(c) * vb);
+    }
     if (e == hipSuccess) e = hipStreamSynchronize(ctx->stream);
-    if (e != hipSuccess) return lsa_set_error(ctx, LSA_ERR_HIP, "lsa_krylov_ritz_vectors: download failed: %s", hipGetErrorString(e));
+    if (e != hipSuccess) {
+        (void)hipStreamSynchronize(ctx->stream);
+        return lsa_set_error(ctx, LSA_ERR_HIP, "lsa_krylov_ritz_vectors: download failed: %s", hipGetErrorString(e));
+    }
     for (size_t c = 0; c < k->imag_norms.size(); ++c) k->imag_norms[c] = std::sqrt(((const double*)((const char*)ctx->pinned + (size_t)m * nvec * 16))[c]);
     return LSA_OK;
 }
@@ -1256,3 +1404,30 @@
 }
 
 }
+
+int krylov_stage_start(lsa_ctx* ctx, lsa_krylov* k, void** buf) {
+    *buf = nullptr;
+    if (ctx->nranks != 1 || !step_plan(ctx, k).pipelined) return LSA_OK;
+    LSA_CHECK(lsa_ensure_stage(ctx, (size_t)std::max<int64_t>(k->n, 1) * 16));
+    *buf = ctx->stage;
+    return LSA_OK;
+}
+int krylov_start_staged(lsa_ctx* ctx, lsa_krylov* k) {
+    LSA_HIP_CHECK(ctx, hipMemcpyAsync(k->w, ctx->stage, (size_t)k->n * 16, hipMemcpyHostToDevice, ctx->stream));
+    LSA_CHECK(k_nrm2(ctx, LSA_C128, k->n, k->w, k->start_nrm2));
+    LSA_CHECK(k_scale_by_inv_norm(ctx, LSA_C128, k->n, k->w, k->start_nrm2, k->V));
+    k->start_pending = true;
+    return LSA_OK;
+}
+
+int krylov_speculate_apply(lsa_ctx* ctx, lsa_krylov* k, int32_t m) {
+    k->spec_col = -1;
+    if (m < 1 || m > k->ncv || ctx->nranks != 1) return LSA_OK;
+    const StepPlan plan = step_plan(ctx, k);
+    if (!plan.pipelined || !plan.tail) return LSA_OK;
+    lsa_op* op = k->op;
+    LSA_CHECK(spmv_global(ctx, op->Kmul, LSA_C128, (const char*)k->V + (size_t)m * (size_t)k->n * 16, op->t, false));
+    LSA_CHECK(pc_global(ctx, pc_of(op), op->Kfac->row0, op->n, LSA_C128, op->t, k->w));
+    k->spec_col = m;
+    return LSA_OK;
+}
diff --git a/lsa-fw_amd/lsa_hip/__init__.py b/lsa-fw_amd/lsa_hip/__init__.py
--- a/lsa-fw_amd/lsa_hip/__init__.py
+++ b/lsa-fw_amd/lsa_hip/__init__.py
@@ -103,6 +103,8 @@
     "lsa_last_error": (ctypes.c_char_p, [_P]),
     "lsa_ctx_synchronize": (ctypes.c_int, [_P]),
     "lsa_ctx_arch": (ctypes.c_char_p, [_P]),
+    "lsa_op_drop_pool": (None, [_P]),
+    "lsa_pool_bytes": (_I64, [_P]),
     "lsa_vec_create": (ctypes.c_int, [_P, _I64, ctypes.c_int, _PP]),
     "lsa_vec_destroy": (None, [_P]),
     "lsa_vec_upload": (ctypes.c_int, [_P, _P, _P]),
@@ -284,6 +286,13 @@
             self._lib.lsa_ctx_destroy(self.handle)
             self.handle = None
 
+    def pool_bytes(self) -> int:
+        return int(self._lib.lsa_pool_bytes(self.handle)) if getattr(self, "handle", None) else 0
+
+    def drop_pool(self) -> None:
+        if getattr(self, "handle", None):
+            self._lib.lsa_op_drop_pool(self.handle)
+
     def unique_id(self) -> bytes:
         buf = ctypes.create_string_buffer(128)
         rc = self._lib.lsa_comm_unique_id(buf)
@@ -318,6 +327,10 @@
         calls, nbytes = _I64(0), _I64(0)
         self._lib.lsa_comm_stats(self.handle, ctypes.byref(calls), ctypes.byref(nbytes))
         return {"allgather_calls": calls.value, "allgather_bytes_received": nbytes.value}
+
+
+def pool_bytes_total() -> int:
+    return int(load_library().lsa_pool_bytes(None))
 
 
 class DeviceVector:
```

After: 540.8. 0.971x the previous value.
